# Pi-Star-Lab/RESCO

Measured on AMD Instinct MI355X. Metric: env-steps/sec, higher is better.
Workload: dtype f32; 1 GPU; ingolstadt21 x 4096 lock-step envs per GPU (BASELINE config 3), fixed demand from the map's rou.xml, on-device seeded random policy, Krauss sigma 0.5 + speedFactor dev 0.1; tls_expiry=1, map=ingolstadt21, envs_per_gpu=4096, pipes=2, ticks_per_env_step=10, block_threads=512, lds_bytes_per_env=40896, parallelism=env-batch split x1, no collective on the data path

## Files before the change

include/resco_sim.h:

```cpp
#ifndef RESCO_SIM_H
#define RESCO_SIM_H
#include <stdint.h>

#ifdef __cplusplus
extern "C" {
#endif

#define RS_OK 0
#define RS_EINVAL (-1)
#define RS_EHIP (-2)
#define RS_ENOMEM (-3)
#define RS_ELIMIT (-4)

typedef struct rs_scenario {
    int32_t n_lanes, n_links, n_edges, n_routes, n_trips, n_signals, n_obs, n_vtypes;
    int32_t n_foes, n_route_steps, n_tls_states, n_tls_dur, n_tls_yellow;
    int32_t n_fix_states, n_fix_dur, n_mv_in, n_mv_out, n_pr_out;
    int32_t horizon, capacity, step_length, yellow_length, kmax;
    const float *lane_len, *lane_vmax;
    const int32_t *lane_edge, *lane_left, *lane_right, *lane_link_start, *lane_link_cnt, *lane_obs, *lane_internal;
    const int32_t *link_to_lane, *link_dest_lane, *link_to_edge, *link_tls, *link_tls_pos, *link_minor, *link_cont;
    const int32_t *link_foe_start, *link_foe_cnt;
    const float *link_via_len;
    const int32_t *link_via1, *link_via2, *link_from_lane, *foe_link;
// ... 203 lines not shown
int rs_mplight_dqn_grad(rs_mplight_dqn_handle p, const rs_mplight_ring *ring, const int32_t *idx, int32_t batch, float *loss_out, void *stream);
int rs_mplight_dqn_step(rs_mplight_dqn_handle p, void *stream);
int rs_mplight_dqn_update(rs_mplight_dqn_handle p, const rs_mplight_ring *ring, int32_t batch, uint32_t seed, int32_t n_updates, float *loss_out,
                          void *stream);
int64_t rs_mplight_dqn_steps(rs_mplight_dqn_handle p);
void rs_mplight_dqn_destroy(rs_mplight_dqn_handle p);

typedef struct rs_train {
    int32_t kind;
    int32_t n_envs;
    rs_policy_handle policy;
    void *learner;
    void *obs;
    int16_t *act;
    float *rew;
    uint8_t *done;
    float *ret;
    float *loss_out;
    int64_t t0;
    double eps_start, eps_end;
    int32_t capacity, head, count, done_step;
    int32_t batch, updates_per_step, target_update, decay_steps;
    uint32_t policy_seed, learner_seed;
} rs_train;
int rs_idqn_pack_weights(rs_policy_handle p, const rs_dqn_tensors *params, void *stream);
int rs_dqn_sync_target(rs_dqn_handle p, void *stream);
int rs_mplight_dqn_sync_target(rs_mplight_dqn_handle p, void *stream);
int rs_group_train(const rs_handle *handles, int32_t n_handles, const rs_train *train, int32_t n_steps);

typedef struct rs_ppo_train {
    rs_policy_handle policy;
    rs_ppo_handle learner;
    rs_rollout seg;
    uint8_t *done;
    float *last_value;
    float *adv, *ret;
    void *gae_scratch;
    int32_t *perm;
    float *loss_out;
    int64_t t0;
    int64_t update0;
    int32_t slot0, done_step;
    int32_t epochs, minibatch;
    float gamma, lambda;
    uint32_t policy_seed, learner_seed;
} rs_ppo_train;
int rs_ppo_perm(int32_t n, int32_t epochs, uint32_t seed, uint32_t update_key, int32_t *perm , void *stream);
int rs_ippo_pack_weights(rs_policy_handle p, const rs_ppo_tensors *params, void *stream);
int rs_group_ppo_train(const rs_handle *handles, int32_t n_handles, const rs_ppo_train *tr, int32_t n_steps);

typedef struct rs_fma2c_desc {
    int32_t K, M, S, n_obs, full;
    float norm_wave, clip_wave, norm_wait, clip_wait;
    const int32_t *n_a, *n_s, *n_w, *n_f;
    const int32_t *gather_off, *gather_idx;
    const float *gather_scale;
    const int32_t *fp_off, *fp_src, *mgr_off, *mgr_src;
} rs_fma2c_desc;
int rs_fma2c_create(int32_t device_id, const rs_fma2c_desc *desc, const float *weights, int32_t max_envs, rs_policy_handle *out);
int rs_fma2c_act(rs_policy_handle p, const float *lane_agg, int32_t n_envs, int32_t env_base, uint32_t seed, uint32_t step_key,
                 const void *dyn, int32_t *actions, float *pi_out, float *value_out, float *rows_out, void *stream);
int rs_fma2c_value(rs_policy_handle p, const float *lane_agg, int32_t n_envs, int32_t env_base, float *value_out, void *stream);
int rs_fma2c_reset(rs_policy_handle p, int32_t env_base, int32_t n_envs, int32_t clear_fingerprints, void *stream);
int rs_fma2c_set_device_weights(rs_policy_handle p, const float *weights);
int rs_fma2c_buffer(rs_policy_handle p, int32_t which, void **dev_ptr);
void rs_fma2c_destroy(rs_policy_handle p);

typedef struct rs_fma2c_learn_config {
    double gamma, lr, alpha, eps, max_grad_norm, value_coef, entropy_coef, reward_norm, reward_clip;
    int64_t workspace_bytes;
} rs_fma2c_learn_config;
typedef struct rs_fma2c_learn *rs_fma2c_learn_handle;
int rs_fma2c_learn_create(rs_policy_handle policy, const rs_fma2c_learn_config *config, int32_t n_envs, int32_t t_max, rs_fma2c_learn_handle *out);
int rs_fma2c_learn_grad(rs_fma2c_learn_handle l, const float *rows, const int32_t *acts, const float *rewards, const float *values,
                        const int32_t *dones, const float *R_boot, int32_t T, float *loss_out, void *stream);
int rs_fma2c_learn_step(rs_fma2c_learn_handle l, void *stream);
int rs_fma2c_learn_update(rs_fma2c_learn_handle l, const float *rows, const int32_t *acts, const float *rewards, const float *values,
                          const int32_t *dones, const float *R_boot, int32_t T, float *loss_out, const float *states_fw, void *stream);
int rs_fma2c_learn_reset(rs_fma2c_learn_handle l, void *stream);
int rs_fma2c_learn_buffer(rs_fma2c_learn_handle l, int32_t which, void **dev_ptr);
void rs_fma2c_learn_destroy(rs_fma2c_learn_handle l);

int rs_info(rs_handle h, int32_t *n_envs, int32_t *block_threads, int32_t *lds_bytes, int32_t *max_lanes_per_signal);

#ifdef __cplusplus
}
#endif
#endif
```

resco_amd/build.py:

```python
import os
import subprocess

HERE = os.path.dirname(os.path.abspath(__file__))
ROOT = os.path.dirname(HERE)
SRC = os.path.join(HERE, 'csrc', 'resco_sim.hip')
LIB = os.path.join(HERE, 'csrc', 'libresco_sim.so')
HIPCC = os.environ.get('HIPCC', '/opt/rocm/bin/hipcc')
FLAGS = ['--offload-arch=gfx950', '-O3', '-std=c++17', '-ffp-contract=off', '-fno-honor-nans', '-mllvm', '-disable-machine-licm', '-fPIC', '-shared',
         '-I' + os.path.join(ROOT, 'include'), '-I' + os.path.join(HERE, 'csrc')]
_DEPS = [SRC] + [os.path.join(HERE, 'csrc', f) for f in ('resco_host.h', 'resco_step.h', 'resco_tables.h', 'resco_policy.h', 'resco_frap.h', 'resco_fma2c.h', 'resco_fma2c_train.h', 'resco_ppo.h', 'resco_train.h', 'resco_ppo_train.h', 'resco_dqn_train.h', 'resco_frap_train.h', 'resco_group_train.h', 'resco_ppo_loop.h')] + \
        [os.path.join(ROOT, 'include', f) for f in ('resco_sim.h', 'resco_model.h')]


def build_library(force=False, verbose=False):
    force = force or os.environ.get('GRAFT_FORCE_BUILD') == '1'
    if not force and os.path.exists(LIB) and all(os.path.getmtime(LIB) >= os.path.getmtime(d) for d in _DEPS):
        return LIB
    cmd = [HIPCC] + FLAGS + [SRC, '-o', LIB]
    if verbose:
        print(' '.join(cmd))
    subprocess.check_call(cmd)
    return LIB


CHECK_LIB = os.path.join(HERE, 'csrc', 'libresco_sim_check.so')


def build_check_library(force=False):
    force = force or os.environ.get('GRAFT_FORCE_BUILD') == '1'
    if not force and os.path.exists(CHECK_LIB) and all(os.path.getmtime(CHECK_LIB) >= os.path.getmtime(d) for d in _DEPS):
        return CHECK_LIB
    subprocess.check_call([HIPCC] + FLAGS + ['-DRS_DEVICE_ASSERT', '-DRS_ONE_CAP=256', SRC, '-o', CHECK_LIB])
    return CHECK_LIB


FIELDLOADS_LIB = os.path.join(HERE, 'csrc', 'libresco_sim_fieldloads.so')


def build_fieldloads_library(force=False):
    if not force and os.path.exists(FIELDLOADS_LIB) and all(os.path.getmtime(FIELDLOADS_LIB) >= os.path.getmtime(d) for d in _DEPS):
        return FIELDLOADS_LIB
    subprocess.check_call([HIPCC] + FLAGS + ['-DRS_FIELD_LOADS', '-DRS_ONE_CAP=256', SRC, '-o', FIELDLOADS_LIB])
    return FIELDLOADS_LIB


if __name__ == '__main__':
    print(build_library(force=True, verbose=True))
```

resco_amd/csrc/resco_host.h:

```cpp
#pragma once
#include "resco_step.h"

RS_DEV void rs_reset_env(const KTab &T, const State &G, const KParams &P, int env, int first, unsigned stride) {
    const int C = T.capacity, S = T.n_signals;
    const size_t eo = (size_t)env * C;
    for (int s = first; s < C; s += stride) {
        G.lane()[eo + s] = LANE_NONE; G.trip()[eo + s] = TRIP_NONE; G.owner()[eo + s] = OWNER_NONE;
        G.rwait()[eo + s] = 0; G.swait()[eo + s] = 0; G.cursor()[eo + s] = 0; G.depart()[eo + s] = 0; G.wtot()[eo + s] = 0;
        G.pos()[eo + s] = 0.0f; G.speed()[eo + s] = 0.0f; G.accel()[eo + s] = 0.0f; G.tloss()[eo + s] = 0.0f; G.sf()[eo + s] = 1.0f;
        G.coop(0)[eo + s] = COOP_NONE; G.coop(1)[eo + s] = COOP_NONE; G.cooplead(0)[eo + s] = COOP_NONE; G.cooplead(1)[eo + s] = COOP_NONE;
    }
    for (int s = first; s < S; s += stride) {
        int ph, left;
        if (P.fixed_program) { ph = T.cold.fix_init_phase[s]; left = T.cold.fix_init_left[s]; }
        else { ph = T.cold.tls_init_phase[s]; left = T.cold.tls_dur[T.cold.tls_dur_off[s] + ph]; }
        G.tls[(env * S + s) * TLS_W + 0] = ph; G.tls[(env * S + s) * TLS_W + 1] = left; G.tls[(env * S + s) * TLS_W + 2] = 0; G.tls[(env * S + s) * TLS_W + 3] = 0;
    }
    for (int d = first; d < T.n_dep; d += stride) G.dep_next[(size_t)env * T.n_dep + d] = T.cold.dep_first[d];
    for (int i = first; i < (C + 31) / 32; i += stride) G.mail[(size_t)env * ((C + 31) / 32) + i] = 0u;
    for (int i = first; i < 4; i += stride) G.env[env * 4 + i] = 0;
    for (int i = first; i < ST_N; i += stride) G.stats[(size_t)env * ST_N + i] = 0;
    if (G.trip_log)
        for (int i = first; i < T.n_trips * 4; i += stride) G.trip_log[(size_t)env * T.n_trips * 4 + i] = 0;
}
// ... 57 lines not shown
    X(VEH_POS, G.pos(), F32, 2, n, c, 1, 1)                 X(VEH_SPEED, G.speed(), F32, 2, n, c, 1, 1)                               \
    X(VEH_ACCEL, G.accel(), F32, 2, n, c, 1, 1)             X(VEH_TLOSS, G.tloss(), F32, 2, n, c, 1, 1)                               \
    X(VEH_LANE, G.lane(), U16, 2, n, c, 1, 1)               X(VEH_TRIP, G.trip(), U16, 2, n, c, 1, 1)                                 \
    X(VEH_CURSOR, G.cursor(), U16, 2, n, c, 1, 1)           X(VEH_SWAIT, G.swait(), U16, 2, n, c, 1, 1)                               \
    X(VEH_RWAIT, G.rwait(), U16, 2, n, c, 1, 1)             X(VEH_DEPART, G.depart(), U16, 2, n, c, 1, 1)                             \
    X(VEH_OWNER, G.owner(), U8, 2, n, c, 1, 1)              X(STATS, G.stats, I64, 2, n, ST_N, 1, 1)                                  \
    X(DRQ_NORM_F16, O.drq_f16(), F16, 4, n, s, lmax, 5)     X(VEH_SF, G.sf(), F32, 2, n, c, 1, 1)                                     \
    X(VEH_WTOT, G.wtot(), U16, 2, n, c, 1, 1)               X(TRIP_LOG, G.trip_log, I32, 3, n, n_trips, 4, 1)                         \
    X(DEP_NEXT, G.dep_next, U16, 2, n, n_dep, 1, 1)                                                                                   \
    X(VEH_COOP, G.coop(0), U32, 2, n, c, 1, 1)              X(VEH_COOPLEAD, G.cooplead(0), U32, 2, n, c, 1, 1)                        \
    X(ARRIVALS, O.arrivals(), I32, 2, n, s, 1, 1)           X(DEPARTURES, O.departures(), I32, 2, n, s, 1, 1)                         \
    X(MPLIGHT_FULL, O.mplight_full(), F32, 3, n, s, 49, 1)  X(LANE_ARRIVALS, O.lane_arr(), I32, 2, n, o, 1, 1)                        \
    X(VEH_COOP_ODD, G.coop(1), U32, 2, n, c, 1, 1)          X(VEH_COOPLEAD_ODD, G.cooplead(1), U32, 2, n, c, 1, 1)                    \
    X(VEH_MAIL, G.mail, U32, 2, n, (c + 31) / 32, 1, 1)
#define RS_BUF_BIT(id, ptr, dt, nd, a, b, c_, d) | (1ull << RS_BUF_##id)
static_assert((0ull RS_BUF_TABLE(RS_BUF_BIT)) == (1ull << RS_BUF_COUNT) - 1, "RS_BUF_TABLE must describe every buffer id below RS_BUF_COUNT");
#undef RS_BUF_BIT
#define RS_BUF_ONE(id, ptr, dt, nd, a, b, c_, d) + 1
static_assert((0 RS_BUF_TABLE(RS_BUF_ONE)) == RS_BUF_COUNT, "RS_BUF_TABLE must describe every buffer id once");
#undef RS_BUF_ONE
static inline void rs_fill_bufs(Buf *bufs, const State &G, const Out &O, int32_t *actions, const BufDims &D) {
    const int64_t n = D.n, c = D.c, s = D.s, o = D.o, lmax = D.lmax, n_dep = D.n_dep, n_trips = D.n_trips;
#define RS_BUF_SET(id, ptr_, dt, nd, a, b, c_, d)                                                                  \
    { Buf &B = bufs[RS_BUF_##id];                                                                                  \
      B.ptr = (void *)(ptr_); B.dtype = RS_##dt; B.ndim = nd;                                                      \
      B.shape[0] = (a); B.shape[1] = (b); B.shape[2] = (c_); B.shape[3] = (d);                                     \
      B.bytes = (size_t)(B.shape[0] * B.shape[1] * B.shape[2] * B.shape[3]) * kDtypeSize[RS_##dt]; }
    RS_BUF_TABLE(RS_BUF_SET)
#undef RS_BUF_SET
}
static inline void rs_buf_describe(const Buf &B, void **ptr, int64_t shape[4], int32_t *ndim, int32_t *dtype) {
    if (ptr) *ptr = B.ptr;
    if (shape) for (int i = 0; i < 4; ++i) shape[i] = B.shape[i];
    if (ndim) *ndim = B.ndim;
    if (dtype) *dtype = B.dtype;
}
static inline void rs_info_describe(int n_envs_, int block_, size_t lds_, int lmax_, int32_t *n_envs, int32_t *block_threads, int32_t *lds_bytes,
                                    int32_t *max_lanes_per_signal) {
    if (n_envs) *n_envs = n_envs_;
    if (block_threads) *block_threads = block_;
    if (lds_bytes) *lds_bytes = (int32_t)lds_;
    if (max_lanes_per_signal) *max_lanes_per_signal = lmax_;
}

static inline const char *rs_pack_tables(PackedTables &PT, const rs_scenario *sc) {
    PackedTables probe;
    if (!probe.build(sc)) { PT.err = probe.err; return PT.err.c_str(); }
    if (!PT.build(sc, pick_cell_len(sc, probe.n_arr, probe.n_dep, probe.tls_maxl))) return PT.err.c_str();
    return nullptr;
}
#define RS_KTAB_TABLES(X, K, PT, sc)                                                                                                  \
    X(K.lanes_, LaneRec, PT.lanes.data(), PT.lanes.size()) X(K.links_, LinkRec, PT.links.data(), PT.links.size())                     \
    X(K.foes_, FoeRec, PT.foes.data(), PT.foes.size()) X(K.rsteps_, RStep, PT.rsteps.data(), PT.rsteps.size())                        \
    X(K.routes_, RouteRec, PT.routes.data(), PT.routes.size()) X(K.next_link_, uint16_t, PT.next_link.data(), PT.next_link.size())    \
    X(K.trip_route_, uint16_t, PT.trip_route.data(), PT.trip_route.size()) X(K.trip_vtype_, uint8_t, PT.trip_vtype.data(), PT.trip_vtype.size()) \
    X(K.route_cont_, float, PT.route_cont.data(), PT.route_cont.size()) X(K.notbest_, uint16_t, PT.notbest.data(), PT.notbest.size()) \
    X(K.cold.trip_depart, int32_t, sc->trip_depart, sc->n_trips) X(K.cold.trip_next, uint16_t, PT.trip_next.data(), PT.trip_next.size()) \
    X(K.cold.dep_lane, uint16_t, PT.dep_lane.data(), PT.dep_lane.size()) X(K.cold.dep_info, DepInfo, PT.dep_info.data(), PT.dep_info.size()) \
    X(K.cold.dep_first, uint16_t, PT.dep_first.data(), PT.dep_first.size())                                                           \
    X(K.cold.vtype_params, float, sc->vtype_params, sc->n_vtypes * VT_COLS)                                                           \
    X(K.cold.tls8, uint8_t, PT.tls8.data(), PT.tls8.size()) X(K.cold.fix8, uint8_t, PT.fix8.data(), PT.fix8.size())                   \
    X(K.cold.tls_nphase, int32_t, sc->tls_nphase, sc->n_signals) X(K.cold.tls_ngreen, int32_t, sc->tls_ngreen, sc->n_signals)         \
    X(K.cold.tls_nlinks, int32_t, sc->tls_nlinks, sc->n_signals) X(K.cold.tls_state_off, int32_t, PT.tls_off_p.data(), sc->n_signals) \
    X(K.cold.tls_dur_off, int32_t, sc->tls_dur_off, sc->n_signals) X(K.cold.tls_yel_off, int32_t, sc->tls_yel_off, sc->n_signals)     \
    X(K.cold.tls_dur, int32_t, sc->tls_dur, sc->n_tls_dur) X(K.cold.tls_yellow, int32_t, sc->tls_yellow, sc->n_tls_yellow)            \
    X(K.cold.tls_init_phase, int32_t, sc->tls_init_phase, sc->n_signals)                                                              \
    X(K.cold.fix_nphase, int32_t, sc->fix_nphase, sc->n_signals) X(K.cold.fix_state_off, int32_t, PT.fix_off_p.data(), sc->n_signals) \
    X(K.cold.fix_dur_off, int32_t, sc->fix_dur_off, sc->n_signals) X(K.cold.fix_dur, int32_t, sc->fix_dur, sc->n_fix_dur)             \
    X(K.cold.fix_init_phase, int32_t, sc->fix_init_phase, sc->n_signals) X(K.cold.fix_init_left, int32_t, sc->fix_init_left, sc->n_signals) \
    X(K.cold.lane_obs, int16_t, PT.lane_obs16.data(), PT.lane_obs16.size()) X(K.cold.obs_sig, int32_t, PT.obs_sig.data(), PT.obs_sig.size()) \
    X(K.cold.sig_obs_start, int32_t, sc->sig_obs_start, sc->n_signals + 1)                                                            \
    X(K.cold.mv_in_start, int32_t, sc->mv_in_start, sc->n_signals * 12 + 1) X(K.cold.mv_in_idx, int32_t, sc->mv_in_idx, sc->n_mv_in)  \
    X(K.cold.mv_out_start, int32_t, sc->mv_out_start, sc->n_signals * 12 + 1) X(K.cold.mv_out_idx, int32_t, sc->mv_out_idx, sc->n_mv_out) \
    X(K.cold.pr_out_start, int32_t, sc->pr_out_start, sc->n_signals + 1) X(K.cold.pr_out_idx, int32_t, sc->pr_out_idx, sc->n_pr_out)  \
    X(K.cold.trips_cum, int32_t, sc->trips_cum, sc->horizon + 2)
static inline int rs_step_ratio(const rs_params *p) { return p->step_ratio > 1 ? p->step_ratio : 1; }
static inline void rs_ktab_scalars(KTab &K, const PackedTables &PT, const rs_scenario *sc, int ratio) {
    K.maxlen = PT.maxlen; K.occ_unit = PT.occ_unit;
    K.n_trips = sc->n_trips; K.tls_maxl = PT.tls_maxl; K.kmax = sc->kmax;
    K.n_lanes = sc->n_lanes; K.n_cells = PT.n_cells; K.n_signals = sc->n_signals; K.n_obs = sc->n_obs; K.n_vtypes = sc->n_vtypes;
    K.horizon = sc->horizon; K.capacity = sc->capacity; K.step_length = sc->step_length; K.yellow_length = sc->yellow_length * ratio; K.lmax = PT.lmax;
    K.n_arr = PT.n_arr; K.n_dep = PT.n_dep;
}
static inline KParams rs_kparams(const rs_params *p, int32_t env_base, int32_t n_envs) {
    KParams P{};
    P.seed = p->seed; P.env_base = env_base; P.max_distance = p->max_distance; P.sigma = p->sigma;
    P.speed_dev = p->speed_dev; P.fixed_program = p->fixed_program; P.tls_expiry = p->tls_hold == 0; P.n_envs = n_envs;
    return P;
}
```

resco_amd/csrc/resco_sim.hip:

```cpp
#include <hip/hip_runtime.h>
#include <hip/hip_fp16.h>
#include <stdint.h>
#include <stdio.h>
#include <stdlib.h>
#include <string.h>
#include <math.h>
#include <initializer_list>
#include <mutex>
#include <new>
#include <string>
#include <vector>

#include "resco_sim.h"

#define RS_DEV __device__ __forceinline__
#define RS_HD __host__ __device__
#define RS_MEM __device__ __forceinline__
#define RS_G(p) (p)
#define RS_CARVE __host__ __device__ __forceinline__
__device__ __forceinline__ void rs_atomic_min(int32_t *p, int32_t v) { atomicMin(p, v); }
__device__ __forceinline__ void rs_atomic_min(uint32_t *p, uint32_t v) { atomicMin(p, v); }
__device__ __forceinline__ void rs_atomic_max(int32_t *p, int32_t v) { atomicMax(p, v); }
__device__ __forceinline__ void rs_atomic_add(int32_t *p, int32_t v) { atomicAdd(p, v); }
__device__ __forceinline__ int32_t rs_atomic_fetch_add(int32_t *p, int32_t v) { return atomicAdd(p, v); }
__device__ __forceinline__ int32_t rs_wave_ticket(int32_t *p) {
    const unsigned long long m = __ballot(1);
    const int below = (int)__builtin_amdgcn_mbcnt_hi((uint32_t)(m >> 32), __builtin_amdgcn_mbcnt_lo((uint32_t)m, 0u));
    int32_t base = 0;
    if (below == 0) base = atomicAdd(p, (int32_t)__popcll(m));
    return __builtin_amdgcn_readlane(base, __ffsll((long long)m) - 1) + below;
}
__device__ __forceinline__ void rs_wave_add(int32_t *p, int32_t v) {
    for (int m = 32; m > 0; m >>= 1) v += __shfl_xor(v, m);
    if ((threadIdx.x & 63) == 0 && v) atomicAdd(p, v);
}
__device__ __forceinline__ void rs_wave_max(int32_t *p, int32_t v) {
    for (int m = 32; m > 0; m >>= 1) { const int32_t o = __shfl_xor(v, m); v = o > v ? o : v; }
    if ((threadIdx.x & 63) == 0) atomicMax(p, v);
}
__device__ __forceinline__ void rs_atomic_or(uint32_t *p, uint32_t v) { atomicOr(p, v); }
__device__ __forceinline__ uint32_t rs_atomic_fetch_or(uint32_t *p, uint32_t v) { return atomicOr(p, v); }
__device__ __forceinline__ int rs_atomic_inc(int32_t *p) { return atomicAdd(p, 1); }
__device__ __forceinline__ void rs_atomic_and(uint32_t *p, uint32_t v) { atomicAnd(p, v); }
__device__ __forceinline__ uint32_t rs_atomic_cas(uint32_t *p, uint32_t cmp, uint32_t v) { return atomicCAS(p, cmp, v); }
__device__ __forceinline__ int rs_ffsll(unsigned long long x) { return __ffsll(x); }
__device__ __forceinline__ int rs_clzll(unsigned long long x) { return __clzll((long long)x); }
__device__ __forceinline__ int rs_ffs(uint32_t x) { return __ffs((int)x); }
__device__ __forceinline__ int rs_popc(uint32_t x) { return __popc(x); }
__device__ __forceinline__ float rs_int_as_float(int x) { return __int_as_float(x); }
__device__ __forceinline__ int rs_float_as_int(float x) { return __float_as_int(x); }
__device__ __forceinline__ uint16_t rs_f2h(float x) { return __half_as_ushort(__float2half(x)); }

#ifndef RS_IEEE_DIV
__device__ __forceinline__ float rs_div_unscaled(float a, float b) {
    const float r0 = __builtin_amdgcn_rcpf(b);
    const float r1 = __builtin_fmaf(__builtin_fmaf(-b, r0, 1.0f), r0, r0);
    const float q0 = a * r1;
    const float q1 = __builtin_fmaf(__builtin_fmaf(-b, q0, a), r1, q0);
    return __builtin_fmaf(__builtin_fmaf(-b, q1, a), r1, q1);
}
#define RS_DIV(a, b) rs_div_unscaled((a), (b))
#endif
#define RS_OPAQUE_S(x) asm volatile("" : "+s"(x));
#ifndef RS_NARROW_NODE
#define RS_KEEP4(a, b, c, d) asm volatile("" : "+v"(a), "+v"(b), "+v"(c), "+v"(d));
#define RS_KEEP2(a, b) asm volatile("" : "+v"(a), "+v"(b));
#endif
extern __shared__ __attribute__((aligned(16))) char rs_smem[];
#define RS_SMEM rs_smem

#ifdef RS_STUDY_SECTIONS
__device__ unsigned long long *g_sec_prof;
#define RS_SEC_BEGIN unsigned long long sec_t = wall_clock64();
#define RS_SEC(id) { const unsigned long long sec_1 = wall_clock64(); if (g_sec_prof && (threadIdx.x & 63) == 0 && (blockIdx.x & 15) == 0) atomicAdd(&g_sec_prof[id], (sec_1 - sec_t) + (1ull << 40)); sec_t = wall_clock64(); }
#endif
#ifdef RS_DEVICE_ASSERT
#define RS_ASSERT(c) if (!(c)) rs_atomic_add(&L.sc[SC_STATS + ST_INVARIANT], 1);
#endif
#include "resco_host.h"
#include "resco_policy.h"
#include "resco_frap.h"
#include "resco_fma2c.h"
#include "resco_ppo.h"
#include "resco_ppo_train.h"
#include "resco_dqn_train.h"
#include "resco_frap_train.h"
#include "resco_group_train.h"
#include "resco_ppo_loop.h"
#include "resco_fma2c_train.h"

struct StepArgs { KTab T; State G; Out O; Lds L; };
typedef const __attribute__((address_space(4))) StepArgs *StepArgsPtr;

template <bool PROF> struct DevExec {
    int B;
    int wave;
    unsigned long long *prof;
    unsigned long long t0;
    template <class F> __device__ __forceinline__ void phase(int id, F f) {
        int w = wave;
        uint32_t ones = ~0u;
        asm volatile("" : "+s"(w), "+s"(ones));
        int tid = (w << 6) | (int)__builtin_amdgcn_mbcnt_hi(ones, __builtin_amdgcn_mbcnt_lo(ones, 0u));
        asm volatile("" : "+v"(tid));
        f(tid);
        __syncthreads();
        if (PROF && prof) {
            const unsigned long long t1 = wall_clock64();
            if (tid == 0) atomicAdd(&prof[id], t1 - t0);
            t0 = t1;
        }
    }
    __device__ __forceinline__ int wave_of(int) const { return wave; }
    __device__ __forceinline__ int next_chunk(int32_t *ctr, int, int, int) const {
        int c = 0;
        if (__builtin_amdgcn_mbcnt_hi(~0u, __builtin_amdgcn_mbcnt_lo(~0u, 0u)) == 0) c = atomicAdd(ctr, 1);
        return __builtin_amdgcn_readfirstlane(c);
    }
    __device__ __forceinline__ unsigned long long role_begin() const { return (PROF && prof) ? wall_clock64() : 0ull; }
    __device__ __forceinline__ void role_end(int id, unsigned long long start) const {
#ifdef RS_STUDY_SECTIONS
        return;
#endif
        if (PROF && prof && (threadIdx.x & 63) == 0 && (blockIdx.x & 15) == 0) atomicAdd(&prof[id], (wall_clock64() - start) + (1ull << 40));
    }
};
template <int CAP, bool PROF> __device__ __forceinline__ void rs_step_kernel_body(StepArgsPtr Ac, const KParams &P, const int32_t *__restrict__ actions) {
    if ((int)blockIdx.x >= P.n_envs) return;
    const StepArgs *A = (const StepArgs *)Ac;
#ifdef RS_STUDY_SECTIONS
    if (threadIdx.x == 0) g_sec_prof = P.prof;
#endif
    DevExec<PROF> ex{(int)blockDim.x, __builtin_amdgcn_readfirstlane((int)threadIdx.x >> 6), PROF ? P.prof : nullptr, (PROF && P.prof) ? wall_clock64() : 0ull};
    rs_step_body<CAP>(ex, A->L, A->T, A->G, A->O, P, actions, (int)blockIdx.x);
}
template <int CAP>
__global__ void __launch_bounds__(1024, 8)
rs_step_kernel_v64(StepArgsPtr Ac, KParams P, const int32_t *__restrict__ actions) { rs_step_kernel_body<CAP, false>(Ac, P, actions); }
template <int CAP>
__global__ void __launch_bounds__(768, 6)
rs_step_kernel_v80(StepArgsPtr Ac, KParams P, const int32_t *__restrict__ actions) { rs_step_kernel_body<CAP, false>(Ac, P, actions); }
template <int CAP>
__global__ void __launch_bounds__(512, 4)
rs_step_kernel_v128(StepArgsPtr Ac, KParams P, const int32_t *__restrict__ actions) { rs_step_kernel_body<CAP, false>(Ac, P, actions); }
__global__ void __launch_bounds__(768, 6)
rs_step_kernel_prof(StepArgsPtr Ac, KParams P, const int32_t *__restrict__ actions) { rs_step_kernel_body<0, true>(Ac, P, actions); }

__global__ void rs_reset_kernel(KTab T, State G, KParams P) { rs_reset_env(T, G, P, (int)blockIdx.x, (int)threadIdx.x, blockDim.x); }
__global__ void rs_reinit_kernel(KTab T, State G, KParams P) { rs_reinit_env(T, G, P, (int)blockIdx.x, (int)threadIdx.x, blockDim.x); }
__global__ void rs_act_random_kernel(KTab T, KParams P, uint32_t step_key, int32_t *actions) {
    const int i = blockIdx.x * blockDim.x + threadIdx.x;
    if (i < P.n_envs * T.n_signals) actions[i] = rs_random_action(T, P, step_key, i);
}
__global__ void rs_act_maxwave_kernel(KTab T, KParams P, const int32_t *pairs, int n_pairs, const int32_t *valid, const int32_t *order,
                                      int use_pressure, const int32_t *mplight, const int32_t *wave, int32_t *actions) {
    const int i = blockIdx.x * blockDim.x + threadIdx.x;
    if (i < P.n_envs * T.n_signals) actions[i] = rs_maxwave_action(T, pairs, n_pairs, valid, order, use_pressure, mplight, wave, i);
}

enum RegBudget { V64 = 0, V128 = 1, V80 = 2 };
struct rs_sim {
    int device = 0;
    int n_envs = 0, env_base = 0, block = 256;
    int ratio = 1;
    size_t lds = 0;
    KTab K{};
    StepArgs *args = nullptr;
    RegBudget budget = V64;
    State G{};
    Out O{};
    KParams P{};
    uint32_t out_mask = OUT_ALL;
    int32_t *actions = nullptr;
    int32_t *pairs = nullptr, *valid = nullptr, *order = nullptr;
    unsigned long long *prof = nullptr;
    int n_pairs = 0;
    hipStream_t stream = nullptr;
    bool blocking = false;
    int32_t *pair = nullptr;
    hipStream_t last = nullptr;
    std::vector<void *> allocs;
    Buf bufs[RS_BUF_COUNT]{};
    bool timing = false;
    std::vector<std::pair<hipEvent_t, hipEvent_t>> events;
    size_t ev_used = 0;
    std::string err;
};

static thread_local std::string g_create_err;

#define HIPCHK(h, call)                                                                            \
    do {                                                                                           \
        hipError_t e_ = (call);                                                                    \
        if (e_ != hipSuccess) {                                                                    \
            (h)->err = std::string(#call) + ": " + hipGetErrorString(e_);                          \
            (void)hipGetLastError();     \
            return RS_EHIP;                                                                        \
        }                                                                                          \
    } while (0)

template <typename Tp>
static int dev_alloc(rs_sim *h, Tp **p, size_t count, bool zero = true) {
    void *d = nullptr;
    size_t bytes = (count ? count : 1) * sizeof(Tp);
    hipError_t e = hipMalloc(&d, bytes);
    if (e != hipSuccess) { h->err = std::string("hipMalloc: ") + hipGetErrorString(e); return RS_ENOMEM; }
    if (zero) (void)hipMemset(d, 0, bytes);
    h->allocs.push_back(d);
    *p = (Tp *)d;
    return RS_OK;
}
template <typename Tp>
static int dev_upload(rs_sim *h, const Tp **dst, const Tp *src, size_t count) {
    Tp *d = nullptr;
    int rc = dev_alloc(h, &d, count, false);
    if (rc) return rc;
    if (count) HIPCHK(h, hipMemcpy(d, src, count * sizeof(Tp), hipMemcpyHostToDevice));
    *dst = d;
    return RS_OK;
}

typedef void (*step_kernel_fn)(StepArgsPtr, KParams, const int32_t *);
static const int kStepCaps[] = {0, 128, 256, 512, 768, 896, 1024};
#define RS_PICK(cap_) (regs == V128 ? rs_step_kernel_v128<cap_> : (regs == V80 ? rs_step_kernel_v80<cap_> : rs_step_kernel_v64<cap_>))
static step_kernel_fn step_kernel_for(int regs, int capacity) {
#ifdef RS_ONE_CAP
    (void)capacity;
    return regs == V64 ? rs_step_kernel_v64<RS_ONE_CAP> : rs_step_kernel_v80<RS_ONE_CAP>;
#else
    switch (capacity) {
        case 128: return RS_PICK(128);
        case 256: return RS_PICK(256);
        case 512: return RS_PICK(512);
        case 768: return RS_PICK(768);
        case 896: return RS_PICK(896);
        case 1024: return RS_PICK(1024);
        default: return RS_PICK(0);
    }
#endif
}

static hipError_t wait_idle(rs_sim *h) {
    hipError_t e = hipStreamSynchronize(h->stream);
    if (e == hipSuccess && h->last && h->last != h->stream) e = hipStreamSynchronize(h->last);
    return e;
}

extern "C" int32_t rs_default_block(int32_t capacity, int32_t n_envs_on_device, int32_t device_id) {
    const int C = capacity;
    if (C < 64 || n_envs_on_device <= 0) return 0;
    const int base = C >= 768 ? 8 : ((C / 2) + 63) / 64;
    int waves = base;
    if (C < 768) {
        int cus = 256;
        hipDeviceProp_t prop;
        if (hipGetDeviceProperties(&prop, device_id) == hipSuccess && prop.multiProcessorCount > 0) cus = prop.multiProcessorCount;
        else (void)hipGetLastError();
        const long budget = (long)cus * 4 * 7;
        const int fit = (int)(budget / n_envs_on_device), most = C / 64 + 1;
        waves = fit < most ? fit : most;
        if (waves < base) waves = base;
    }
    return -(20000 + 64 * waves);
}

static bool decode_block(int block_threads, size_t lds, RegBudget *budget, int *threads) {
    int t = block_threads;
    RegBudget b = V64;
    if (t <= -20000) {
        t = -t - 20000;
        b = (t == 512 && lds <= RS_LDS_4WG_LIMIT) ? V64 : V80;
    } else if (t < 0) { b = V128; t = -t; if (t >= 10000) { b = V80; t -= 10000; } }
    *budget = b; *threads = t;
    return t % 64 == 0 && t >= 64 && t <= (b == V128 ? 512 : (b == V80 ? 768 : 1024));
}

extern "C" int rs_create(const rs_scenario *sc, const rs_params *p, int32_t n_envs, int32_t env_base, int32_t device_id,
                         int32_t block_threads, rs_handle *out) {
    if (!sc || !p || !out || n_envs <= 0) { g_create_err = "rs_create: bad argument"; return RS_EINVAL; }
    rs_sim *h = new (std::nothrow) rs_sim();
    if (!h) return RS_ENOMEM;
    auto fail = [&](int rc) { g_create_err = h->err; (void)hipGetLastError(); rs_destroy(h); return rc; };
    (void)hipGetLastError();
    h->device = device_id; h->n_envs = n_envs; h->env_base = env_base;
    int ndev = 0;
    if (hipGetDeviceCount(&ndev) != hipSuccess || ndev <= 0) { h->err = "no HIP device visible (this library has no CPU fallback)"; return fail(RS_EHIP); }
    if (hipSetDevice(device_id) != hipSuccess) { h->err = "hipSetDevice failed"; return fail(RS_EHIP); }
    if (sc->step_length <= 0 || sc->yellow_length < 0 || sc->yellow_length >= sc->step_length) {
        h->err = "need 0 <= yellow_length < step_length"; return fail(RS_EINVAL);
    }
    const int C = sc->capacity;
    if (C < 64 || (C % 64) || C > 1984) { h->err = "capacity must be a multiple of 64 in [64, 1984]"; return fail(RS_ELIMIT); }
    if (sc->kmax < 1 || sc->kmax > 16) { h->err = "kmax (lanes per edge) must be in [1, 16]"; return fail(RS_ELIMIT); }
    PackedTables PT;
    if (const char *msg = rs_pack_tables(PT, sc)) { h->err = msg; return fail(RS_ELIMIT); }
    int rc;
#define UP(dst, type, src, count) if ((rc = dev_upload<type>(h, &dst, src, (size_t)(count)))) return fail(rc);
    RS_KTAB_TABLES(UP, h->K, PT, sc)
#undef UP
    h->ratio = rs_step_ratio(p);
    rs_ktab_scalars(h->K, PT, sc, h->ratio);
    const int lmax = PT.lmax;
    h->P = rs_kparams(p, env_base, n_envs);
    const size_t N = (size_t)n_envs, NC = N * C, S = (size_t)sc->n_signals;
    State &G = h->G;
    Out &O = h->O;
    {
        char *slab = nullptr, *outb = nullptr;
        G.nc = NC;
        O.n = n_envs; O.o = sc->n_obs; O.s = sc->n_signals; O.lm = lmax;
        if ((rc = dev_alloc(h, &slab, State::bytes(NC))) || (rc = dev_alloc(h, &outb, O.bytes())) ||
            (rc = dev_alloc(h, &G.env, N * 4)) || (rc = dev_alloc(h, &G.tls, N * S * TLS_W)) || (rc = dev_alloc(h, &G.stats, N * ST_N)) ||
            (rc = dev_alloc(h, &G.dep_next, N * (size_t)h->K.n_dep)) || (rc = dev_alloc(h, &G.mail, N * (size_t)((C + 31) / 32))) ||
            (rc = dev_alloc(h, &h->actions, N * S)))
            return fail(rc);
        G.base = slab; O.base = outb;
    }
    G.trip_log = nullptr;
    if (p->trip_log && (rc = dev_alloc(h, &G.trip_log, N * (size_t)sc->n_trips * 4))) return fail(rc);
    rs_fill_bufs(h->bufs, G, O, h->actions, BufDims{n_envs, C, sc->n_signals, sc->n_obs, lmax, h->K.n_dep, p->trip_log ? sc->n_trips : 0});

    h->lds = lds_carve(nullptr, C, h->K.n_cells, h->K.n_arr, h->K.n_dep, sc->n_obs, sc->n_signals, sc->n_vtypes, h->K.tls_maxl);
    if (const char *pad = getenv("RESCO_STUDY_LDS_PAD")) h->lds += (size_t)atoi(pad);
    if (h->lds > 160 * 1024) { h->err = "scenario needs more than 160 KiB of LDS per environment"; return fail(RS_ELIMIT); }
    if (block_threads == 0) block_threads = rs_default_block(C, n_envs, device_id);
    if (!decode_block(block_threads, h->lds, &h->budget, &block_threads)) {
        h->err = "block_threads must be a multiple of 64 in [64, 1024] ([64, 768] for the 80-VGPR build, [64, 512] for the 128-VGPR build)";
        return fail(RS_EINVAL);
    }
    h->block = block_threads;
    {
        static std::mutex mu;
        static size_t max_lds[64] = {0};
        std::lock_guard<std::mutex> lock(mu);
        size_t &cur = max_lds[device_id & 63];
        if (h->lds > cur) {
            for (int v = V64; v <= V80; ++v)
                for (int cp : kStepCaps)
                    if (hipFuncSetAttribute((const void *)step_kernel_for(v, cp), hipFuncAttributeMaxDynamicSharedMemorySize, (int)h->lds) != hipSuccess) {
                        h->err = "hipFuncSetAttribute(MaxDynamicSharedMemorySize) failed"; return fail(RS_EHIP);
                    }
            if (hipFuncSetAttribute((const void *)rs_step_kernel_prof, hipFuncAttributeMaxDynamicSharedMemorySize, (int)h->lds) != hipSuccess) {
                h->err = "hipFuncSetAttribute(MaxDynamicSharedMemorySize) failed"; return fail(RS_EHIP);
            }
            cur = h->lds;
        }
    }
    {
        StepArgs sa{h->K, h->G, h->O, Lds{}};
        lds_carve(&sa.L, C, h->K.n_cells, h->K.n_arr, h->K.n_dep, sc->n_obs, sc->n_signals, sc->n_vtypes, h->K.tls_maxl);
        if (!lds_fix_matches(sa.L, C)) { h->err = "the layout of the working memory does not match the kernel's literals (lds_carve / LdsFix)"; return fail(RS_EINVAL); }
        sa.L.cell_inv = PT.cell_inv;
        if ((rc = dev_alloc(h, &h->args, 1, false))) return fail(rc);
        if (hipMemcpy(h->args, &sa, sizeof(sa), hipMemcpyHostToDevice) != hipSuccess) { h->err = "hipMemcpy(StepArgs) failed"; return fail(RS_EHIP); }
    }
    {
        hipDeviceProp_t prop;
        std::vector<uint32_t> mask;
        if (getenv("RESCO_PLAIN_STREAMS") == nullptr && hipGetDeviceProperties(&prop, device_id) == hipSuccess)
            mask.assign((size_t)(prop.multiProcessorCount + 31) / 32, 0xFFFFFFFFu);
        if (mask.empty() || hipExtStreamCreateWithCUMask(&h->stream, (uint32_t)mask.size(), mask.data()) != hipSuccess) {
            (void)hipGetLastError();
            if (hipStreamCreateWithFlags(&h->stream, hipStreamNonBlocking) != hipSuccess) { h->err = "hipStreamCreate failed"; return fail(RS_EHIP); }
        } else h->blocking = true;
    }
    *out = h;
    int r2 = rs_reset(h, nullptr);
    if (r2) { g_create_err = h->err; *out = nullptr; rs_destroy(h); return r2; }
    return RS_OK;
}

extern "C" void rs_destroy(rs_handle h) {
    if (!h) return;
    (void)hipSetDevice(h->device);
    if (h->stream) { (void)wait_idle(h); (void)hipStreamDestroy(h->stream); }
    for (auto &e : h->events) { (void)hipEventDestroy(e.first); (void)hipEventDestroy(e.second); }
    for (void *p : h->allocs) (void)hipFree(p);
    delete h;
}

extern "C" const char *rs_last_error(rs_handle h) { return h ? h->err.c_str() : g_create_err.c_str(); }

static int launch_step(rs_sim *h, hipStream_t st, int n_ticks, int do_fsm, int do_observe = 1) {
    KParams P = h->P;
    P.n_ticks = n_ticks; P.do_fsm = do_fsm; P.do_observe = do_observe; P.out_mask = h->out_mask; P.prof = h->prof;
    hipEvent_t e0 = nullptr, e1 = nullptr;
    if (h->timing) {
        if (h->ev_used == h->events.size()) {
            hipEvent_t a, b;
            HIPCHK(h, hipEventCreate(&a));
            HIPCHK(h, hipEventCreate(&b));
            h->events.emplace_back(a, b);
        }
        e0 = h->events[h->ev_used].first; e1 = h->events[h->ev_used].second;
        h->ev_used += 1;
        HIPCHK(h, hipEventRecord(e0, st));
    }
    const step_kernel_fn fn = (h->prof && h->block <= 768) ? (step_kernel_fn)rs_step_kernel_prof : step_kernel_for(h->budget, h->K.capacity);
    hipLaunchKernelGGL(fn, dim3(h->n_envs), dim3(h->block), h->lds, st, (StepArgsPtr)h->args, P, (const int32_t *)h->actions);
    HIPCHK(h, hipGetLastError());
    if (h->timing) HIPCHK(h, hipEventRecord(e1, st));
    return RS_OK;
}

static int enter(rs_sim *h, void *stream, hipStream_t *st) {
    if (!h) return RS_EINVAL;
    HIPCHK(h, hipSetDevice(h->device));
    *st = stream ? (hipStream_t)stream : h->stream;
    h->last = *st;
    return RS_OK;
}

static int launch_reset(rs_sim *h, void *stream, void (*kernel)(KTab, State, KParams)) {
    hipStream_t st;
    int rc = enter(h, stream, &st);
    if (rc) return rc;
    hipLaunchKernelGGL(kernel, dim3(h->n_envs), dim3(256), 0, st, h->K, h->G, h->P);
    HIPCHK(h, hipGetLastError());
    bool tm = h->timing;
    h->timing = false;
    rc = launch_step(h, st, 0, 0);
    h->timing = tm;
    return rc;
}
extern "C" int rs_reset(rs_handle h, void *stream) { return launch_reset(h, stream, rs_reset_kernel); }
extern "C" int rs_reinit_signals(rs_handle h, void *stream) { return launch_reset(h, stream, rs_reinit_kernel); }

extern "C" int rs_step(rs_handle h, const int32_t *actions, int32_t actions_on_device, void *stream) {
    hipStream_t st;
    if (int rc = enter(h, stream, &st)) return rc;
    if (actions) {
        size_t bytes = (size_t)h->n_envs * h->K.n_signals * sizeof(int32_t);
        HIPCHK(h, hipMemcpyAsync(h->actions, actions, bytes, actions_on_device ? hipMemcpyDeviceToDevice : hipMemcpyHostToDevice, st));
        if (!actions_on_device) HIPCHK(h, hipStreamSynchronize(st));
    }
    return launch_step(h, st, h->K.step_length * h->ratio, 1);
}

extern "C" int rs_ticks(rs_handle h, int32_t n_ticks, void *stream) {
    hipStream_t st;
    if (n_ticks < 0) return RS_EINVAL;
    if (int rc = enter(h, stream, &st)) return rc;
    return launch_step(h, st, n_ticks, 0);
}

extern "C" int rs_step_sim(rs_handle h, int32_t n_ticks, void *stream) {
    hipStream_t st;
    if (n_ticks < 0) return RS_EINVAL;
    if (int rc = enter(h, stream, &st)) return rc;
    return launch_step(h, st, n_ticks, 0, 0);
}

extern "C" int rs_set_outputs(rs_handle h, uint64_t buffer_mask) {
    if (!h) return RS_EINVAL;
    h->out_mask = rs_out_mask(buffer_mask);
    return RS_OK;
}

extern "C" int rs_sync(rs_handle h) {
    if (!h) return RS_EINVAL;
    HIPCHK(h, hipSetDevice(h->device));
    HIPCHK(h, wait_idle(h));
    return RS_OK;
}

static void launch_random(rs_sim *h, hipStream_t st, uint32_t step_key) {
    const int total = h->n_envs * h->K.n_signals;
    hipLaunchKernelGGL(rs_act_random_kernel, dim3((total + 255) / 256), dim3(256), 0, st, h->K, h->P, step_key, h->actions);
}
static void launch_maxwave(rs_sim *h, hipStream_t st, int use_pressure) {
    const int total = h->n_envs * h->K.n_signals;
    hipLaunchKernelGGL(rs_act_maxwave_kernel, dim3((total + 255) / 256), dim3(256), 0, st, h->K, h->P, (const int32_t *)h->pairs,
                       h->n_pairs, (const int32_t *)h->valid, (const int32_t *)h->order, use_pressure, (const int32_t *)h->O.mplight(),
                       (const int32_t *)h->O.wave(), h->actions);
}

extern "C" int rs_act_random(rs_handle h, uint32_t step_key, void *stream) {
    hipStream_t st;
    if (int rc = enter(h, stream, &st)) return rc;
    launch_random(h, st, step_key);
    HIPCHK(h, hipGetLastError());
// ... 45 lines not shown
    if (!h) return RS_EINVAL;
    return rs_read_buffer(h, RS_BUF_STATS, host_out, (int64_t)h->n_envs * ST_N * 8);
}

struct Snapshot { std::vector<void *> ptrs; uint32_t seed = 0; };
static const int kSnapBufs[] = {RS_BUF_LANE_AGG, RS_BUF_DRQ_NORM, RS_BUF_PHASE, RS_BUF_MPLIGHT, RS_BUF_WAVE, RS_BUF_WAIT,
                                RS_BUF_WAIT_NORM, RS_BUF_PRESSURE, RS_BUF_QUEUE_SUM, RS_BUF_QUEUE_MAX, RS_BUF_DRQ_NORM_F16,
                                RS_BUF_ENV, RS_BUF_TLS, RS_BUF_VEH_POS, RS_BUF_VEH_SPEED, RS_BUF_VEH_ACCEL, RS_BUF_VEH_TLOSS,
                                RS_BUF_VEH_LANE, RS_BUF_VEH_TRIP, RS_BUF_VEH_CURSOR, RS_BUF_VEH_SWAIT, RS_BUF_VEH_RWAIT,
                                RS_BUF_VEH_DEPART, RS_BUF_VEH_OWNER, RS_BUF_VEH_SF, RS_BUF_VEH_WTOT, RS_BUF_TRIP_LOG, RS_BUF_STATS,
                                RS_BUF_DEP_NEXT, RS_BUF_VEH_COOP, RS_BUF_VEH_COOPLEAD, RS_BUF_ARRIVALS, RS_BUF_DEPARTURES, RS_BUF_MPLIGHT_FULL,
                                RS_BUF_LANE_ARRIVALS, RS_BUF_VEH_COOP_ODD, RS_BUF_VEH_COOPLEAD_ODD, RS_BUF_VEH_MAIL};
extern "C" int rs_snapshot(rs_handle h, void **snap) {
    if (!h || !snap) return RS_EINVAL;
    HIPCHK(h, hipSetDevice(h->device));
    HIPCHK(h, wait_idle(h));
    Snapshot *S = new Snapshot();
    S->seed = h->P.seed;
    for (int b : kSnapBufs) {
        void *d = nullptr;
        if (h->bufs[b].bytes == 0) { S->ptrs.push_back(nullptr); continue; }
        if (hipMalloc(&d, h->bufs[b].bytes) != hipSuccess) { h->err = "rs_snapshot: hipMalloc failed"; rs_snapshot_free(h, S); return RS_ENOMEM; }
        S->ptrs.push_back(d);
        HIPCHK(h, hipMemcpy(d, h->bufs[b].ptr, h->bufs[b].bytes, hipMemcpyDeviceToDevice));
    }
    *snap = S;
    return RS_OK;
}
extern "C" int rs_restore(rs_handle h, const void *snap) {
    if (!h || !snap) return RS_EINVAL;
    HIPCHK(h, hipSetDevice(h->device));
    HIPCHK(h, wait_idle(h));
    const Snapshot *S = (const Snapshot *)snap;
    size_t i = 0;
    for (int b : kSnapBufs) { if (h->bufs[b].bytes) HIPCHK(h, hipMemcpy(h->bufs[b].ptr, S->ptrs[i], h->bufs[b].bytes, hipMemcpyDeviceToDevice)); ++i; }
    h->P.seed = S->seed;
    return RS_OK;
}
extern "C" void rs_snapshot_free(rs_handle h, void *snap) {
    if (!snap) return;
    Snapshot *S = (Snapshot *)snap;
    for (void *p : S->ptrs) (void)hipFree(p);
    delete S;
}

extern "C" int rs_timing(rs_handle h, int32_t enable) {
    if (!h) return RS_EINVAL;
    h->timing = enable != 0;
    return RS_OK;
}
extern "C" int rs_timing_read(rs_handle h, float *total_ms, int32_t *launches) {
    if (!h) return RS_EINVAL;
    HIPCHK(h, hipSetDevice(h->device));
    HIPCHK(h, hipDeviceSynchronize());
    float tot = 0.0f;
    for (size_t i = 0; i < h->ev_used; ++i) {
        float ms = 0.0f;
        HIPCHK(h, hipEventElapsedTime(&ms, h->events[i].first, h->events[i].second));
        tot += ms;
    }
    if (total_ms) *total_ms = tot;
    if (launches) *launches = (int32_t)h->ev_used;
    h->ev_used = 0;
    return RS_OK;
}

extern "C" int rs_phase_profile(rs_handle h, int32_t enable, uint64_t *host_out16) {
    if (!h) return RS_EINVAL;
    HIPCHK(h, hipSetDevice(h->device));
    HIPCHK(h, hipDeviceSynchronize());
    if (h->prof && host_out16) HIPCHK(h, hipMemcpy(host_out16, h->prof, 16 * 8, hipMemcpyDeviceToHost));
    if (enable && !h->prof) { int rc = dev_alloc(h, &h->prof, 16); if (rc) return rc; }
    if (h->prof) HIPCHK(h, hipMemset(h->prof, 0, 16 * 8));
    if (!enable) h->prof = nullptr;
    return RS_OK;
}

extern "C" int rs_set_seed(rs_handle h, uint32_t seed) {
    if (!h) return RS_EINVAL;
    h->P.seed = seed;
    return RS_OK;
}

extern "C" int rs_info(rs_handle h, int32_t *n_envs, int32_t *block_threads, int32_t *lds_bytes, int32_t *max_lanes_per_signal) {
    if (!h) return RS_EINVAL;
    rs_info_describe(h->n_envs, h->block, h->lds, h->K.lmax, n_envs, block_threads, lds_bytes, max_lanes_per_signal);
    return RS_OK;
}


enum { POLICY_IDQN = 0, POLICY_MPLIGHT = 1, POLICY_FMA2C = 2 };
struct rs_policy {
    int device = 0;
    int kind = POLICY_IDQN;
    PolicyTab W{};
    int amax = 0;
    bool own_w1 = true, own_w2 = true, own_w3 = true, own_b3 = true;
    FrapTab F{};
    Fma2cTab A{};
    int fm_lds = 0;
    const float *fm_own_w = nullptr;
    std::vector<void *> allocs;
};

static int policy_devices(rs_policy_handle *out, int *ndev) {
    if (!out) return RS_EINVAL;
    *out = nullptr;
    if (hipGetDeviceCount(ndev) != hipSuccess || *ndev <= 0) { g_create_err = "no HIP device visible (this library has no CPU fallback)"; return RS_EHIP; }
    return RS_OK;
}
static int policy_new(int device_id, int kind, rs_policy **p) {
    if (hipSetDevice(device_id) != hipSuccess) { g_create_err = "hipSetDevice failed"; return RS_EHIP; }
    *p = new (std::nothrow) rs_policy();
    if (!*p) return RS_ENOMEM;
    (*p)->device = device_id; (*p)->kind = kind;
    return RS_OK;
}
static void policy_destroy(rs_policy *p) {
    if (!p) return;
    (void)hipSetDevice(p->device);
    (void)hipDeviceSynchronize();
    for (void *d : p->allocs) (void)hipFree(d);
    delete p;
}
extern "C" void rs_idqn_destroy(rs_policy_handle p) { policy_destroy(p); }
extern "C" void rs_mplight_destroy(rs_policy_handle p) { policy_destroy(p); }

template <class T> static int pol_upload(rs_policy *p, const T **dst, const void *src, size_t count) {
    void *d = nullptr;
    if (hipMalloc(&d, count * sizeof(T) + 2048) != hipSuccess) return RS_ENOMEM;
    p->allocs.push_back(d);
    if (hipMemcpy(d, src, count * sizeof(T), hipMemcpyHostToDevice) != hipSuccess) return RS_EHIP;
    *dst = (const T *)d;
    return RS_OK;
}

extern "C" int rs_idqn_create(int32_t device_id, int32_t n_signals, int32_t lmax, const int32_t *n_actions, const float *conv_w,
                              const float *conv_b, const uint16_t *w1, const float *b1, const uint16_t *w2, const float *b2,
                              const uint16_t *w3, const float *b3, rs_policy_handle *out) {
    int ndev = 0;
    if (int rc = policy_devices(out, &ndev)) return rc;
    if (device_id < 0 || device_id >= ndev || n_signals <= 0 || lmax < 2 || lmax > 17 || !n_actions || !conv_w || !conv_b || !w1 || !b1 || !w2 || !b2 || !w3 || !b3) {
        g_create_err = "rs_idqn_create: bad argument (1 <= signals, 2 <= lmax <= 17)"; return RS_EINVAL;
    }
    for (int s = 0; s < n_signals; ++s)
        if (n_actions[s] < 1 || n_actions[s] > POL_QMAX) { g_create_err = "rs_idqn_create: 1..8 actions per signal"; return RS_ELIMIT; }
    rs_policy *p = nullptr;
    int rc = policy_new(device_id, POLICY_IDQN, &p);
    if (rc) return rc;
    const size_t S = (size_t)n_signals, hp = (size_t)(lmax / 2);
    p->W.S = n_signals; p->W.lmax = lmax; p->W.hp = (int32_t)hp;
    for (int s = 0; s < n_signals; ++s) p->amax = n_actions[s] > p->amax ? n_actions[s] : p->amax;
    if ((rc = pol_upload<float>(p, &p->W.conv_w, conv_w, S * 64 * 4)) || (rc = pol_upload<float>(p, &p->W.conv_b, conv_b, S * 64)) ||
        (rc = pol_upload<h4_t>(p, &p->W.w1, w1, S * 64 * hp * 2 * 64)) || (rc = pol_upload<float>(p, &p->W.b1, b1, S * 64)) ||
        (rc = pol_upload<h4_t>(p, &p->W.w2, w2, S * 8 * 2 * 64)) || (rc = pol_upload<float>(p, &p->W.b2, b2, S * 64)) ||
        (rc = pol_upload<h4_t>(p, &p->W.w3, w3, S * 8 * 64)) || (rc = pol_upload<float>(p, &p->W.b3, b3, S * 32)) ||
        (rc = pol_upload<int32_t>(p, &p->W.n_actions, n_actions, S)) ||
        (rc = pol_upload<int32_t>(p, &p->W.hp_sig, std::vector<int32_t>(S, (int32_t)hp).data(), S))) {
        g_create_err = "rs_idqn_create: device allocation / upload failed";
        rs_idqn_destroy(p);
        return rc;
    }
    *out = p;
    return RS_OK;
}

// ... 1189 lines not shown
```

resco_amd/csrc/resco_step.h:

```cpp
#pragma once
#include "resco_tables.h"

struct State {
    char *base;
    size_t nc;
    int32_t *trip_log;
    int32_t *env;
    int32_t *tls;
    long long *stats;
    uint16_t *dep_next;
    uint32_t *mail;
    RS_HD float *pos() const { return (float *)base; }
    RS_HD float *speed() const { return RS_G((float *)(base + 4 * nc)); }
    RS_HD float *accel() const { return RS_G((float *)(base + 8 * nc)); }
    RS_HD float *tloss() const { return RS_G((float *)(base + 12 * nc)); }
    RS_HD float *sf() const { return RS_G((float *)(base + 16 * nc)); }
    RS_HD uint32_t *coop(int par) const { return RS_G((uint32_t *)(base + (par ? 43 : 20) * nc)); }
    RS_HD uint32_t *cooplead(int par) const { return RS_G((uint32_t *)(base + (par ? 47 : 24) * nc)); }
    RS_HD uint16_t *lane() const { return RS_G((uint16_t *)(base + 28 * nc)); }
    RS_HD uint16_t *trip() const { return RS_G((uint16_t *)(base + 30 * nc)); }
    RS_HD uint16_t *cursor() const { return RS_G((uint16_t *)(base + 32 * nc)); }
    RS_HD uint16_t *swait() const { return RS_G((uint16_t *)(base + 34 * nc)); }
    RS_HD uint16_t *rwait() const { return RS_G((uint16_t *)(base + 36 * nc)); }
    RS_HD uint16_t *depart() const { return RS_G((uint16_t *)(base + 38 * nc)); }
    RS_HD uint16_t *wtot() const { return RS_G((uint16_t *)(base + 40 * nc)); }
    RS_HD uint8_t *owner() const { return RS_G((uint8_t *)(base + 42 * nc)); }
    static size_t bytes(size_t nc_) { return 51 * nc_; }
};

struct Out {
    char *base;
    int32_t n, o, s, lm;
    RS_HD size_t a5() const { return (size_t)n * o * 5 * 4; }
    RS_HD size_t ns() const { return (size_t)n * s * 4; }
    RS_HD float *lane_agg() const { return (float *)base; }
    RS_HD float *drq_norm() const { return RS_G((float *)(base + a5())); }
    RS_HD float *wait() const { return RS_G((float *)(base + 2 * a5())); }
    RS_HD float *wait_norm() const { return RS_G((float *)(base + 2 * a5() + ns())); }
    RS_HD int32_t *phase() const { return RS_G((int32_t *)(base + 2 * a5() + 2 * ns())); }
    RS_HD int32_t *pressure() const { return RS_G((int32_t *)(base + 2 * a5() + 3 * ns())); }
    RS_HD int32_t *queue_sum() const { return RS_G((int32_t *)(base + 2 * a5() + 4 * ns())); }
    RS_HD int32_t *queue_max() const { return RS_G((int32_t *)(base + 2 * a5() + 5 * ns())); }
    RS_HD int32_t *mplight() const { return RS_G((int32_t *)(base + 2 * a5() + 6 * ns())); }
    RS_HD int32_t *wave() const { return RS_G((int32_t *)(base + 2 * a5() + 19 * ns())); }
    RS_HD int32_t *arrivals() const { return RS_G((int32_t *)(base + 2 * a5() + 31 * ns())); }
    RS_HD int32_t *departures() const { return RS_G((int32_t *)(base + 2 * a5() + 32 * ns())); }
    RS_HD float *mplight_full() const { return RS_G((float *)(base + 2 * a5() + 33 * ns())); }
    RS_HD int32_t *lane_arr() const { return RS_G((int32_t *)(base + 2 * a5() + 82 * ns())); }
    RS_HD uint16_t *drq_f16() const { return RS_G((uint16_t *)(base + 2 * a5() + 82 * ns() + a5() / 5)); }
    RS_HD size_t bytes() const { return 2 * a5() + 82 * ns() + a5() / 5 + (size_t)n * s * lm * 5 * 2 + 64; }
};

RS_DEV uint32_t rs_rotl32(uint32_t x, int r) { return (x << r) | (x >> (32 - r)); }
RS_DEV uint32_t d_hash(uint32_t seed, uint32_t env, uint32_t trip, uint32_t tick, uint32_t stream) {
    uint32_t h = seed;
    const uint32_t w[4] = {env, trip, tick, stream};
#pragma unroll
    for (int i = 0; i < 4; ++i) {
        uint32_t k = w[i];
        k *= 0xcc9e2d51u; k = rs_rotl32(k, 15); k *= 0x1b873593u;
        h ^= k; h = rs_rotl32(h, 13); h = h * 5u + 0xe6546b64u;
    }
    h ^= 16u;
    h ^= h >> 16; h *= 0x85ebca6bu; h ^= h >> 13; h *= 0xc2b2ae35u; h ^= h >> 16;
    return h;
}
RS_DEV float d_u01(uint32_t h) { return (float)(h >> 8) * (1.0f / 16777216.0f); }

#ifndef RS_DIV
#define RS_DIV(a, b) ((a) / (b))
#endif
RS_DEV float d_brake_gap(float v, float b) {
    const int steps = (int)RS_DIV(v, b);
    const float fs = (float)steps;
    return fs * v - b * fs * (fs + 1.0f) * 0.5f;
}
RS_DEV float d_stop_speed(float gap, float b, float tau) {
    const float g = gap - 0.001f;
    if (g < 0.0f) return 0.0f;
    const float q = 1.0f + 4.0f * ((RS_DIV(2.0f * g, b) - tau) + tau * tau);
    const float n = floorf(0.5f - (tau + sqrtf(q) * -0.5f));
    const float h = 0.5f * n * (n - 1.0f) * b + n * b * tau;
    const float r = RS_DIV(g - h, n + tau);
    return n * b + r;
}
RS_DEV float d_free_speed(float dist, float target, float b) {
    if (dist < target) return target;
    const float t2 = b + 2.0f * target;
    float y = RS_DIV((sqrtf(t2 * t2 + 8.0f * b * dist) - b) * 0.5f - target, b);
    if (y < 0.0f) y = 0.0f;
    const float yf = floorf(y);
    const float exact = (yf * yf + yf) * 0.5f * b + yf * target + (y > yf ? target : 0.0f);
    float rest = dist - exact;
    if (rest < 0.0f) rest = 0.0f;
    return RS_DIV(rest, yf + 1.0f) + yf * b + target;
}
RS_DEV float d_follow_speed(float gap, float vl, float b, float bl, float tau) {
    const float bm = b > bl ? b : bl;
    return d_stop_speed(gap + d_brake_gap(vl, bm), b, tau);
}
RS_DEV int speed_factor_q(const KParams &P, int env, int trip, const float *vt) {
    float f = vt[VT_SF_MEAN];
    if (P.speed_dev) {
        float s = 0.0f;
#pragma unroll
        for (uint32_t i = 0; i < 4; ++i) s += d_u01(d_hash(P.seed, (uint32_t)env, (uint32_t)trip, 0xFFFFFFFFu, i));
        const float z = (s - 2.0f) * 1.7320508f;
        f = vt[VT_SF_MEAN] + vt[VT_SF_DEV] * z;
    }
    if (f < 0.2f) f = 0.2f;
// ... 109 lines not shown
        if (6 * ab > grid_bytes) {
            p = (uint32_t)(align16((size_t)C * 16) + align16((size_t)C * 8));
            if (6 * ab > align16((size_t)C * 4)) { p = (uint32_t)o; o += 6 * ab; }
        }
        if (L) {
            L->agg_q.off = p; L->agg_a.off = p + (uint32_t)ab; L->agg_w.off = p + (uint32_t)(2 * ab);
            L->agg_m.off = p + (uint32_t)(3 * ab); L->agg_s.off = p + (uint32_t)(4 * ab); L->agg_n.off = p + (uint32_t)(5 * ab);
        }
    }
#undef CARVE
    return o;
}

template <class Tp, uint32_t OFF> struct CPtr {
    RS_MEM Tp &operator[](int i) const { return ((Tp *)(RS_SMEM + OFF))[i]; }
    RS_MEM operator Tp *() const { return (Tp *)(RS_SMEM + OFF); }
};
template <int C> struct LdsFix {
    static constexpr uint32_t a16(uint32_t x) { return (x + 15u) & ~15u; }
#ifdef RS_LIST_CAP
    static constexpr uint32_t kcap = RS_LIST_CAP;
#else
    static constexpr uint32_t kcap = ((C / 4 + 63) / 64) * 64;
#endif
    static constexpr uint32_t o_node = 0, o_aux = o_node + a16(C * 16), o_vnx = o_aux + a16(C * 8), o_sc = o_vnx + a16(C * 4),
                              o_alive = o_sc + a16((SC_STATS + ST_N) * 4), o_alive0 = o_alive + a16(((C + 31) / 32) * 4),
                              o_ls_h = o_alive0 + a16(((C + 31) / 32) * 4), o_ls_lc = o_ls_h + a16(kcap * 2), o_ls_mh = o_ls_lc + a16(kcap * 2),
                              o_grid = o_ls_mh + a16(kcap * 2);
    CPtr<Node, o_node> node;
    CPtr<Aux, o_aux> aux;
    CPtr<float, o_vnx> vnx;
    CPtr<int32_t, o_sc> sc;
    CPtr<uint32_t, o_alive> alive;
    CPtr<uint32_t, o_alive0> alive0;
    CPtr<uint16_t, o_ls_h> ls_h;
    CPtr<uint16_t, o_ls_lc> ls_lc;
    CPtr<uint16_t, o_ls_mh> ls_mh;
    CPtr<uint16_t, o_grid> grid;
    static constexpr uint32_t lcap = kcap;
    const LPtr<float> &vtp;
    const uint32_t &gstride;
    const LPtr<int32_t> &arr;
    const LPtr<uint16_t> &dep, &dep_t;
    const LPtr<uint32_t> &insm, &mailw;
    const LPtr<int32_t> &agg_q, &agg_a, &agg_w, &agg_m, &agg_n;
    const LPtr<uint32_t> &agg_s;
    const LPtr<int32_t> &sig_arr, &sig_dep, &phase, &left, &nextp;
    const LPtr<uint8_t> &tstate;
    const float &cell_inv;
    RS_MEM explicit LdsFix(const Lds &T)
        : vtp(T.vtp), gstride(T.gstride), arr(T.arr), dep(T.dep), dep_t(T.dep_t), insm(T.insm), mailw(T.mailw), agg_q(T.agg_q), agg_a(T.agg_a), agg_w(T.agg_w),
          agg_m(T.agg_m), agg_n(T.agg_n), agg_s(T.agg_s), sig_arr(T.sig_arr), sig_dep(T.sig_dep), phase(T.phase), left(T.left), nextp(T.nextp),
          tstate(T.tstate), cell_inv(T.cell_inv) {}
    static RS_HD bool matches(const Lds &T) {
        return T.node.off == o_node && T.aux.off == o_aux && T.vnx.off == o_vnx && T.sc.off == o_sc && T.alive.off == o_alive && T.alive0.off == o_alive0 &&
               T.ls_h.off == o_ls_h && T.ls_lc.off == o_ls_lc && T.ls_mh.off == o_ls_mh && T.grid.off == o_grid && T.lcap == kcap;
    }
};
RS_CARVE bool lds_fix_matches(const Lds &T, int C) {
    switch (C) {
        case 128: return LdsFix<128>::matches(T);
        case 256: return LdsFix<256>::matches(T);
        case 512: return LdsFix<512>::matches(T);
        case 768: return LdsFix<768>::matches(T);
        case 896: return LdsFix<896>::matches(T);
        case 1024: return LdsFix<1024>::matches(T);
        default: return true;
    }
}

RS_CARVE float pick_cell_len(const rs_scenario *sc, int n_arr, int n_dep, int tls_maxl) {
    const float choices[] = CELL_CHOICES;
    const int n = (int)(sizeof(choices) / sizeof(choices[0]));
    const size_t limits[2] = {RS_LDS_4WG_LIMIT, RS_LDS_3WG_LIMIT};
    for (int k = 0; k < 2; ++k)
        for (int i = 0; i < n; ++i)
            if (PackedTables::cell_len_ok(sc, choices[i]) &&
                lds_carve(nullptr, sc->capacity, PackedTables::count_cells(sc, choices[i]), n_arr, n_dep, sc->n_obs, sc->n_signals, sc->n_vtypes, tls_maxl) <= limits[k])
                return choices[i];
    for (int i = 0; i < n; ++i) if (PackedTables::cell_len_ok(sc, choices[i])) return choices[i];
    return choices[0];
}

#ifdef RS_EMU_DEBUG
#define RS_CHAIN_GUARD if (++rs_dbg_chain > 50000000L) { printf("endless chain walk\n"); fflush(stdout); abort(); }
#else
#define RS_CHAIN_GUARD
#endif
#ifndef RS_ASSERT
#define RS_ASSERT(c)
#endif
#ifndef RS_SEC
#define RS_SEC_BEGIN
#define RS_SEC(id) {}
#endif
template <class LT> RS_DEV int lane_cells(const LT &L, const LaneRec &LR) { return (int)(LR.len * L.cell_inv) + 1; }
template <class LT> RS_DEV int cell_of(const LT &L, float pos, int ncell) { const int c = (int)(pos * L.cell_inv); return c < ncell ? c : ncell - 1; }

struct Grid { uint16_t *c; uint32_t tag; };
RS_DEV unsigned long long grid_tag4(const Grid &g) { return g.tag ? 0x8000800080008000ull : 0ull; }
RS_DEV int cell_head(const Grid &g, int c) {
    const uint32_t v = g.c[c];
    return ((v ^ g.tag) & CELL_TAG) ? (int)NIL : (int)(v & NIL);
}
RS_DEV uint16_t grid_push(const Grid &g, int c, int s, bool mover) {
    uint32_t *w = (uint32_t *)g.c + (c >> 1);
    const int sh = (c & 1) * 16;
    const uint32_t flag = (mover ? CELL_MOVER : 0u) | g.tag;
    uint32_t old = *w, assumed, cell;
    do {
        assumed = old;
        cell = (assumed >> sh) & 0xFFFFu;
        if ((cell ^ g.tag) & CELL_TAG) cell = NIL;
        const uint32_t keep = cell & CELL_MOVER;
        uint32_t cnt = (cell >> CELL_CNT_SHIFT) & CELL_CNT_MAX;
        if (cnt < CELL_CNT_MAX) cnt += 1u;
        old = rs_atomic_cas(w, assumed, (assumed & ~(0xFFFFu << sh)) | (((uint32_t)s | (cnt << CELL_CNT_SHIFT) | keep | flag) << sh));
    } while (old != assumed);
    return (uint16_t)(cell & NIL);
}
RS_DEV unsigned long long quad_load(const Grid &g, int b) { return *(const unsigned long long *)(g.c + b) ^ grid_tag4(g); }
RS_DEV unsigned long long quad_occ(const Grid &g, int b) {
    const unsigned long long w = quad_load(g, b);
    const unsigned long long x = (w & 0x07FF07FF07FF07FFull) ^ 0x07FF07FF07FF07FFull;
    return (x + 0x07FF07FF07FF07FFull) & 0x0800080008000800ull & ~(w >> 4);
}
RS_DEV int cells_count(const Grid &g, int c0, int nc) {
    const int c1 = c0 + nc - 1;
    int n = 0;
    for (int b = c0 & ~3; b <= c1; b += 4) {
        const unsigned long long w = quad_load(g, b);
        unsigned long long m = (w >> CELL_CNT_SHIFT) & 0x0007000700070007ull;
        m &= ~(((w >> 15) & 0x0001000100010001ull) * 7ull);
        const int lo = c0 - b, hi = c1 - b;
        if (lo > 0) m &= ~0ull << (16 * lo);
        if (hi < 3) m &= ~0ull >> (16 * (3 - hi));
        n += (int)((m * 0x0001000100010001ull) >> 48);
    }
    return n;
}
RS_DEV int scan_up(const Grid &g, int c0, int c1) {
    for (int b = c0 & ~3; b <= c1; b += 4) {
        unsigned long long m = quad_occ(g, b);
        const int lo = c0 - b, hi = c1 - b;
        if (lo > 0) m &= ~0ull << (16 * lo);
        if (hi < 3) m &= ~0ull >> (16 * (3 - hi));
        if (m) return b + ((rs_ffsll(m) - 1) >> 4);
    }
    return -1;
}
RS_DEV int scan_down(const Grid &g, int c0, int c1) {
    for (int b = c1 & ~3; b + 3 >= c0; b -= 4) {
        unsigned long long m = quad_occ(g, b);
        const int lo = c0 - b, hi = c1 - b;
        if (lo > 0) m &= ~0ull << (16 * lo);
        if (hi < 3) m &= ~0ull >> (16 * (3 - hi));
        if (m) return b + ((63 - rs_clzll(m)) >> 4);
        if (b == 0) break;
    }
    return -1;
}
RS_DEV bool cells_have_mover(const Grid &g, int c0, int nc) {
    const int c1 = c0 + nc - 1;
    for (int b = c0 & ~3; b <= c1; b += 4) {
        const unsigned long long w = quad_load(g, b);
        unsigned long long m = w & 0x4000400040004000ull & ~(w >> 1);
// ... 31 lines not shown
};
#define RS_CHAIN_STEP(f, s, COND)                                                                          \
    {                                                                                                      \
        RS_CHAIN_GUARD                                                                                     \
        const Node nd_ = node_load(L, s);                                                                  \
        const unsigned long long key = order_key(nd_.pos, nd_.trip);                                       \
        const bool take_ = (COND);                                                                         \
        (f).slot = take_ ? (s) : (f).slot; (f).key = take_ ? key : (f).key;                                \
        (f).speed_bits = take_ ? (uint32_t)rs_float_as_int(nd_.speed) : (f).speed_bits;                    \
        (f).vtw = take_ ? (uint32_t)nd_.vt : (f).vtw;                                                      \
        s = nd_.nxt;                                                                                       \
    }
template <class LT> RS_DEV Found chain_rearmost(const LT &L, int head) {
    Found f{(int)NIL, ~0ull, 0u, 0u};
    for (int s = head & NIL; s != NIL;) RS_CHAIN_STEP(f, s, key < f.key)
    return f;
}
template <class LT> RS_DEV Found chain_frontmost(const LT &L, int head) {
    Found f{(int)NIL, 0ull, 0u, 0u};
    for (int s = head & NIL; s != NIL;) RS_CHAIN_STEP(f, s, key > f.key)
    return f;
}
template <class LT> RS_DEV Found rearmost_within(const LT &L, const Grid &grid, int cell0, int ncell, float win) {
    Found f{(int)NIL, ~0ull, 0u, 0u};
    if (win < 0.0f) return f;
    const int c = scan_up(grid, cell0, cell0 + cell_of(L, win, ncell));
    if (c < 0) return f;
    f = chain_rearmost(L, cell_head(grid, c));
    if (f.slot != NIL && f.pos() > win) f.slot = NIL;
    return f;
}
template <class LT> RS_DEV Found leader_found(const LT &L, const Grid &grid, int cell0, int ncell, float pos, int k, int self, float win) {
    const int c = cell_of(L, pos, ncell);
    const unsigned long long mykey = order_key(pos, k);
    Found f{(int)NIL, ~0ull, 0u, 0u};
    const uint32_t cw = grid.c[cell0 + c];
    int s = ((cw ^ grid.tag) & CELL_TAG) ? (int)NIL : (int)(cw & NIL);
    if (s == self && ((cw >> CELL_CNT_SHIFT) & CELL_CNT_MAX) == 1u) s = NIL;
    while (s != NIL) {
        RS_ASSERT(s != self || order_key(L.node[s].pos, L.node[s].trip) == mykey)
        RS_CHAIN_STEP(f, s, (key > mykey) & (key < f.key))
    }
    if (f.slot == NIL && c + 1 < ncell) {
        const int cc = scan_up(grid, cell0 + c + 1, cell0 + cell_of(L, pos + win, ncell));
        if (cc >= 0) f = chain_rearmost(L, cell_head(grid, cc));
    }
    if (f.slot != NIL && f.pos() - pos > win) f.slot = NIL;
    return f;
}
template <class LT> RS_DEV int leader_within(const LT &L, const Grid &grid, int cell0, int ncell, float pos, int k, int self, float win) {
    return leader_found(L, grid, cell0, ncell, pos, k, self, win).slot;
}
template <class LT> RS_DEV int follower_within(const LT &L, const Grid &grid, int cell0, int ncell, float pos, int k, int self, float win) {
    const int c = cell_of(L, pos, ncell);
    const unsigned long long mykey = order_key(pos, k);
    Found f{(int)NIL, 0ull, 0u, 0u};
    for (int s = cell_head(grid, cell0 + c); s != NIL;) {
        RS_ASSERT(s != self || order_key(L.node[s].pos, L.node[s].trip) == mykey)
        RS_CHAIN_STEP(f, s, (key < mykey) & (key > f.key))
    }
    if (f.slot == NIL && c > 0) {
        const float lo = pos - win;
        const int cc = scan_down(grid, cell0 + (lo > 0.0f ? cell_of(L, lo, ncell) : 0), cell0 + c - 1);
        if (cc >= 0) f = chain_frontmost(L, cell_head(grid, cc));
    }
    if (f.slot != NIL && pos - f.pos() > win) f.slot = NIL;
    (void)self;
    return f.slot;
}
template <class LT> RS_DEV int at_or_behind_within(const LT &L, const Grid &grid, int cell0, int ncell, float back, float win) {
    if (back < 0.0f) return NIL;
    const int c = cell_of(L, back, ncell);
    Found f{(int)NIL, 0ull, 0u, 0u};
    for (int s = cell_head(grid, cell0 + c); s != NIL;) RS_CHAIN_STEP(f, s, !(nd_.pos > back) & (key > f.key))
    if (f.slot == NIL && c > 0) {
        const float lo = back - win;
        const int cc = scan_down(grid, cell0 + (lo > 0.0f ? cell_of(L, lo, ncell) : 0), cell0 + c - 1);
        if (cc >= 0) f = chain_frontmost(L, cell_head(grid, cc));
    }
    if (f.slot != NIL && back - f.pos() > win) f.slot = NIL;
    return f.slot;
}

template <class LT> RS_DEV int tls_state(const KTab &T, const LT &L, int tls, int pos) {
    if (tls == 0xFF) return TLS_G;
    return L.tstate[tls * T.tls_maxl + pos];
}
RS_DEV uint16_t cache_link(const KTab &T, const LaneRec &LR, int lane, int rq, int trip) {
    if (LR.link_cnt == 0) return NLINK_NONE;
    if (LR.flags & LF_INTERNAL) { const int l = LR.link_start; return (uint16_t)(l | (T.links()[l].arr_idx >= 0 ? NLINK_ARR : 0)); }
    return T.next_link()[((size_t)rq * T.kmax + (lane - (int)LR.edge_lane0)) * 2 + (trip & 1)];
}
template <class LT> RS_DEV bool foe_blocked(const KTab &T, const LT &L, const Grid &grid, const LinkRec &K) {
    for (int i = K.foe_start; i < K.foe_start + K.foe_cnt; ++i) {
        const FoeRec F = rec_load16(T.foes(), i);
        if (F.tls != 0xFF && tls_state(T, L, F.tls, F.tls_pos) == TLS_R) continue;
        if (F.arr_idx >= 0 && L.arr[F.arr_idx] < RM_FOE_GAP_Q) return true;
        if (F.via1_cell0 != 0xFFFF && cells_have_mover(grid, F.via1_cell0, F.via1_nc)) return true;
        if (F.via2_cell0 != 0xFFFF && cells_have_mover(grid, F.via2_cell0, F.via2_nc)) return true;
    }
    return false;
}
template <class LT> RS_DEV void tls_refresh(const KTab &T, const LT &L, const KParams &P, int s, int ph) {
    const int w = T.tls_maxl >> 2;
    const uint32_t *src = (const uint32_t *)((P.fixed_program ? T.cold.fix8 + T.cold.fix_state_off[s] : T.cold.tls8 + T.cold.tls_state_off[s]) + ph * T.tls_maxl);
    uint32_t *dst = (uint32_t *)((uint8_t *)L.tstate + s * T.tls_maxl);
    uint32_t v[8];
#pragma unroll
    for (int i = 0; i < 8; ++i) v[i] = src[i < w ? i : 0];
#pragma unroll
    for (int i = 0; i < 8; ++i) if (i < w) dst[i] = v[i];
#pragma unroll 1
    for (int i = 8; i < w; ++i) dst[i] = src[i];
}
template <class LT> RS_DEV void set_phase(const KTab &T, const LT &L, const KParams &P, int s, int ph) {
    if (ph < 0 || ph >= T.cold.tls_nphase[s]) return;
    L.phase[s] = ph;
    L.left[s] = P.tls_expiry ? T.cold.tls_dur[T.cold.tls_dur_off[s] + ph] : RM_TLS_HOLD_TICKS;
    tls_refresh(T, L, P, s, ph);
}
template <class LT> RS_DEV void tls_begin_of_tick(const KTab &T, const LT &L, const KParams &P, int s, int tick) {
    if (P.do_fsm && !P.fixed_program && tick == T.yellow_length) set_phase(T, L, P, s, L.nextp[s]);
    int left = L.left[s];
    if (left == 0) {
        const int32_t *dur = P.fixed_program ? T.cold.fix_dur + T.cold.fix_dur_off[s] : T.cold.tls_dur + T.cold.tls_dur_off[s];
        const int Pn = P.fixed_program ? T.cold.fix_nphase[s] : T.cold.tls_nphase[s];
        const int ph = (L.phase[s] + 1) % Pn;
        left = dur[ph];
        L.phase[s] = ph;
        tls_refresh(T, L, P, s, ph);
    }
    L.left[s] = left - 1;
}
struct ContRow { float c[4]; const float *cn; };
RS_DEV ContRow cont_row(const KTab &T, int rq) {
    ContRow R;
    R.cn = T.route_cont() + (size_t)rq * T.kmax;
    for (int j = 0; j < 4; ++j) R.c[j] = j < T.kmax ? R.cn[j] : 0.0f;
    return R;
}
RS_DEV float cont_of(const ContRow &R, int j) {
    return j == 0 ? R.c[0] : (j == 1 ? R.c[1] : (j == 2 ? R.c[2] : (j == 3 ? R.c[3] : R.cn[j])));
}
#define OCC_NONE (Grid{(uint16_t *)0, 0u})
#define OCC_FULL (Grid{(uint16_t *)1, 0u})
RS_DEV bool cont_notbest(float c) { return rs_float_as_int(c) < 0; }
RS_DEV float cont_len(float c) { return rs_int_as_float(rs_float_as_int(c) & 0x7FFFFFFF); }
RS_DEV int strategic_dir(const ContRow &R, int kk, int n, float x, float v, int extra, float &rem, const Grid &grid, int cell0, int nc, float occ_unit) {
    const float mine = cont_of(R, kk);
    rem = cont_len(mine) - x;
#ifdef RS_EMU_CHECK_MAIL
    { float best = 0.0f; for (int j = 0; j < n; ++j) { const float c = cont_len(cont_of(R, j)); if (c > best) best = c; }
      for (int j = 0; j < n; ++j) RS_ASSERT(cont_notbest(cont_of(R, j)) == !(cont_len(cont_of(R, j)) >= best - RM_CONT_EPS)) }
#endif
    if (!cont_notbest(mine)) return 0;
    int dl = 1000, dr = 1000;
    for (int j = kk + 1; j < n; ++j) if (!cont_notbest(cont_of(R, j))) { dl = j - kk; break; }
    for (int j = kk - 1; j >= 0; --j) if (!cont_notbest(cont_of(R, j))) { dr = kk - j; break; }
    const int dir = (dr <= dl) ? -1 : +1;
    if (grid.c == (uint16_t *)1) return dir;
    const int off = (dr <= dl ? dr : dl) + extra;
    const float la = (v > RM_LOOK_MIN_SPEED ? v : RM_LOOK_MIN_SPEED) * RM_LOOK_TIME + RM_LOOK_BASE;
    int cnt = 0;
    if (grid.c != (uint16_t *)0) cnt = cells_count(grid, cell0 + ((dr <= dl) ? -dr : dl) * nc, nc);
    if (rem - (float)cnt * occ_unit >= la * (float)off) return 0;
    return dir;
}
RS_DEV uint32_t link_reg_word(const KTab &T, int nlk) { return ((const uint32_t *)&T.links()[nlk & 0x7FFF])[2]; }
template <class LT> RS_DEV void register_approach_w(const KTab &T, const LT &L, uint32_t kw, float v, float pos, float lane_len, int vt) {
    const int st = tls_state(T, L, (int)((kw >> 16) & 0xFFu), (int)(kw >> 24));
    if (st == TLS_R) return;
    const float dist = lane_len - pos;
    if (st == TLS_Y && dist >= d_brake_gap(v, L.vtp[vt * VT_COLS + VT_DECEL])) return;
    const float ta = RS_DIV(dist, v > 1.0f ? v : 1.0f);
    const int q = ta * 10.0f >= 65000.0f ? 65000 : (int)(ta * 10.0f);
    rs_atomic_min(&L.arr[(int16_t)(kw & 0xFFFFu)], q);
}
template <class LT> RS_DEV void register_approach(const KTab &T, const LT &L, int nlk, float v, float pos, float lane_len, int vt) {
    if (!(nlk & NLINK_ARR)) return;
    if (v <= RM_HALT_SPEED) return;
    register_approach_w(T, L, link_reg_word(T, nlk), v, pos, lane_len, vt);
}
template <class LT> RS_DEV void follow_neighbour(const KTab &T, const LT &L, uint32_t key, bool clamp_gap, const LaneRec &LR, int lane, float x, float v,
                             float b, float tau, float mingap, float &vsafe) {
    const int X = (int)(key & 0xFFFFu), kx = (int)(key >> 16);
    if ((int)L.node[X].trip != kx) return;
    const int lx = L.aux[X].lane;
    if (lx == (int)LANE_NONE || (LR.flags & LF_INTERNAL)) return;
    const int l0 = LR.edge_lane0, n = LR.flags >> 2;
    if (lx < l0 || lx >= l0 + n) return;
    const float *vo = L.vtp + L.node[X].vt * VT_COLS;
    const float px = L.node[X].pos, backx = px - vo[VT_LENGTH];
    if (clamp_gap ? !(px >= x) : !(backx >= x)) return;
    float g = backx - x - mingap;
    if (clamp_gap && g < 0.0f) g = 0.0f;
    float vs = d_follow_speed(g, L.node[X].speed, b, vo[VT_DECEL], tau);
    float vc = v - b; if (vc < 0.0f) vc = 0.0f;
    if (vs < vc) vs = vc;
    if (vs < vsafe) vsafe = vs;
    (void)lane;
}

template <class LT> RS_DEV void mail_flag_set(const LT &L, int s, int par) { rs_atomic_or((uint32_t *)((Node *)L.node + s) + 3, SFQ_MAIL(par) << 16); }
template <class LT> RS_DEV void mail_flag_clear(const LT &L, int s, int par) { rs_atomic_and((uint32_t *)((Node *)L.node + s) + 3, ~(SFQ_MAIL(par) << 16)); }
template <class LT, class LP> RS_DEV void list_push(const LT &L, const LP &list, int counter, int s);
template <class LT> RS_DEV void flag_mover(const LT &L, int s, int t, int lct = 0) {
    uint32_t *w = (uint32_t *)((Node *)L.node + s) + 3;
    const uint32_t bit = (uint32_t)fl_mh(t) << 8;
    if (!(rs_atomic_fetch_or(w, bit | ((uint32_t)lct << 8)) & bit)) list_push(L, L.ls_mh, SC_NMH + (t & 1), s);
}
template <class LT, class LP> RS_DEV void list_push(const LT &L, const LP &list, int counter, int s) {
    const int i = rs_wave_ticket(&L.sc[counter]);
    if (i < (int)L.lcap) list[i] = (uint16_t)s;
}
RS_DEV float plan_vfree(const float *vt, float v, float lane_vmax, float sf) {
    float vfree = v + vt[VT_ACCEL];
    const float vl = lane_vmax * sf;
    if (vl < vfree) vfree = vl;
    if (vt[VT_MAXSPEED] < vfree) vfree = vt[VT_MAXSPEED];
    return vfree;
}
RS_DEV float plan_look(const float *vt, float vfree) { return d_brake_gap(vfree, vt[VT_DECEL]) + vfree * vt[VT_TAU] + vt[VT_MINGAP] + 1.0f; }
RS_DEV bool looks_beyond(const float *vt, float v, float x, float lane_len, float lane_vmax, float sf) {
    return lane_len - x < plan_look(vt, plan_vfree(vt, v, lane_vmax, sf));
}
RS_DEV bool may_change_lanes_row(const ContRow &R, const LaneRec &LR, int lane, int k, float x, float v, int t) {
    const int n = LR.flags >> 2;
    if ((LR.flags & LF_INTERNAL) || n < 2) return false;
    const int kk = lane - (int)LR.edge_lane0;
    float rem;
    if (strategic_dir(R, kk, n, x, v, 0, rem, OCC_FULL, 0, 0, 0.0f) != 0) return true;
    if ((((uint32_t)t >> 1) + (uint32_t)k) & 3u) return false;
    const int tk = kk + ((t & 1) ? -1 : +1);
    return tk >= 0 && tk < n && strategic_dir(R, tk, n, x, v, RM_SG_EXTRA_LANES, rem, OCC_NONE, 0, 0, 0.0f) == 0;
}
RS_DEV bool may_change_lanes(const KTab &T, int rq, uint32_t nb, const LaneRec &LR, int lane, int k, float x, float v, int t) {
    const int n = LR.flags >> 2;
    if ((LR.flags & LF_INTERNAL) || n < 2) return false;
    const int kk = lane - (int)LR.edge_lane0;
    bool r;
    if ((nb >> kk) & 1u) r = true;
    else if ((((uint32_t)t >> 1) + (uint32_t)k) & 3u) r = false;
    else {
        const int tk = kk + ((t & 1) ? -1 : +1);
        if (tk < 0 || tk >= n) r = false;
        else if (!((nb >> tk) & 1u)) r = true;
        else { float rem; r = strategic_dir(cont_row(T, rq), tk, n, x, v, RM_SG_EXTRA_LANES, rem, OCC_NONE, 0, 0, 0.0f) == 0; }
    }
#ifdef RS_EMU_CHECK_MAIL
    RS_ASSERT(r == may_change_lanes_row(cont_row(T, rq), LR, lane, k, x, v, t))
#endif
    return r;
}
template <class LT> RS_DEV int classify(const KTab &T, const LT &L, int s, const float *vt, float v, float x, const LaneRec &LR, int lane, int rq, uint32_t nb, int k, float sf, int t) {
    int fl = 0;
    if (looks_beyond(vt, v, x, LR.len, LR.vmax, sf)) { fl |= FL_H; list_push(L, L.ls_h, SC_NH, s); }
    if (may_change_lanes(T, rq, nb, LR, lane, k, x, v, t)) { fl |= FL_LC; list_push(L, L.ls_lc, SC_NLC, s); }
    return fl;
}

template <bool LONG, class LT> RS_DEV void phase_plan(const KTab &T, const LT &L, const Grid &grid, const State &G, size_t eo, const KParams &P, int genv, int t, int s) {
    RS_SEC_BEGIN
    const Aux ax = L.aux[s];
    const int lane = ax.lane;
    if (lane == (int)LANE_NONE) return;
    const Node me = L.node[s];
    const int k = me.trip;
    const float *vt = L.vtp + me.vt * VT_COLS;
    const float a = vt[VT_ACCEL], b = vt[VT_DECEL], tau = vt[VT_TAU], mingap = vt[VT_MINGAP];
    const float v = me.speed, x = me.pos;
    const float sf = sf_of(me.sfq);
    const LaneRec LR0 = rec_load16(T.lanes(), lane);
    LaneRec LR = LR0;
    float vsafe = RM_BIGF;
    float tgap = 0.0f, tvl = 0.0f, tbl = b;
    bool have = false;
    if (LONG) RS_SEC(7)
    const float vfree = plan_vfree(vt, v, LR.vmax, sf);
    const float look = plan_look(vt, vfree);
    const Found ld = leader_found(L, grid, LR.cell0, lane_cells(L, LR), x, k, s, look + T.maxlen);
    const int lead = ld.slot;
    if (LONG) RS_SEC(8)
    bool found = false;
    if (lead != NIL) {
        const float *vo = L.vtp + ld.vt() * VT_COLS;
        tgap = ld.pos() - vo[VT_LENGTH] - x - mingap;
        tvl = ld.speed(); tbl = vo[VT_DECEL];
        have = true; found = true;
    }
    if (me.sfq & SFQ_MAIL((t + 1) & 1)) {
        const int q = (t + 1) & 1;
        const uint32_t c1 = G.coop(q)[eo + s], c2 = G.cooplead(q)[eo + s];
        if (c1 != COOP_NONE) { G.coop(q)[eo + s] = COOP_NONE; follow_neighbour(T, L, c1, false, LR, lane, x, v, b, tau, mingap, vsafe); }
        if (c2 != COOP_NONE) { G.cooplead(q)[eo + s] = COOP_NONE; follow_neighbour(T, L, c2, true, LR, lane, x, v, b, tau, mingap, vsafe); }
        mail_flag_clear(L, s, q);
    }
#ifdef RS_EMU_CHECK_MAIL
    else { RS_ASSERT(G.coop((t + 1) & 1)[eo + s] == COOP_NONE && G.cooplead((t + 1) & 1)[eo + s] == COOP_NONE) }
#endif
    if (LONG) RS_SEC(9)
    float seen = LR.len - x;
    RS_ASSERT(LONG || found || !(seen < look))
    if (LONG && !found && seen < look) {
        int rq = ax.rq;
        int link = (int)(ax.nlink & 0x7FFF);
        int cur_lane = lane;
        const float bgv = d_brake_gap(v, b);
        for (int hop = 0; hop < RM_MAX_HOPS; ++hop) {
            const bool cur_int = (LR.flags & LF_INTERNAL) != 0;
            if (hop > 0) link = (int)(cache_link(T, LR, cur_lane, rq, k) & 0x7FFF);
            bool stop_here = false;
            LinkRec K;
            if (link == NLINK_NONE) {
                if (!cur_int && T.rsteps()[rq].next_edge == 0xFFFF) break;
                stop_here = true;
            } else {
                K = link_load(T.links(), link);
                const int st = tls_state(T, L, K.tls, K.tls_pos);
                if (K.tls != 0xFF && (st == TLS_R || st == TLS_Y) && seen >= bgv) stop_here = true;
                if (!stop_here && !(K.flags & KF_CONT) && ((K.flags & KF_MINOR) || (K.tls != 0xFF && st == TLS_g))) {
                    if (seen > RM_VIS_DIST) stop_here = true;
                    else if (K.foe_cnt > 0 && foe_blocked(T, L, grid, K)) stop_here = true;
                }
            }
            if (stop_here) {
                const float g = seen - RM_STOP_OFFSET;
                tgap = g > 0.0f ? g : 0.0f; tvl = 0.0f; tbl = b;
                have = true;
                break;
            }
            LR = K.dest;
            cur_lane = K.to_lane;
            {
                const float vnl = LR.vmax * sf;
                if (vnl < vfree) {
                    const float vs = d_free_speed(seen, vnl, b);
                    if (vs < vsafe) vsafe = vs;
                }
            }
            const Found od = rearmost_within(L, grid, LR.cell0, lane_cells(L, LR), look - seen + T.maxlen);
            if (od.slot != NIL) {
                const float *vo = L.vtp + od.vt() * VT_COLS;
                tgap = seen + od.pos() - vo[VT_LENGTH] - mingap;
                tvl = od.speed(); tbl = vo[VT_DECEL];
                have = true;
                break;
            }
            if (!cur_int) rq += 1;
            seen += LR.len;
            if (!(seen < look)) break;
        }
    }
    if (LONG) RS_SEC(10)
    if (have) {
        const float vs = d_follow_speed(tgap, tvl, b, tbl, tau);
        if (vs < vsafe) vsafe = vs;
    }
    float vmin_n = v - b; if (vmin_n < 0.0f) vmin_n = 0.0f;
    float vmin_e = v - vt[VT_EMERGENCY]; if (vmin_e < 0.0f) vmin_e = 0.0f;
    const float lo = vsafe > vmin_e ? vsafe : vmin_e;
    const float vmin = vmin_n < lo ? vmin_n : lo;
    float vmax = vfree < vsafe ? vfree : vsafe;
    if (vmax < vmin) vmax = vmin;
    const float sigma = P.sigma >= 0.0f ? P.sigma : vt[VT_SIGMA];
    float vd = vmax;
    if (sigma > 0.0f) {
        const float r = d_u01(d_hash(P.seed, (uint32_t)genv, (uint32_t)k, (uint32_t)t, 0u));
        if (vd < a) vd -= sigma * vd * r; else vd -= sigma * a * r;
        if (vd < 0.0f) vd = 0.0f;
    }
    const float vnext = vd > vmin ? vd : vmin;
    L.vnx[s] = vnext;
#ifdef RS_EMU_DEBUG
    if (s == rs_dbg_slot && (t == rs_dbg_t || rs_dbg_t < 0))
        printf("plan t %d slot %d lane %d x %.3f v %.3f lead %d have %d tgap %.3f tvl %.3f vsafe %.3f vfree %.3f vnext %.3f nlink %x\n", t, s, lane, x, v, lead,
               (int)have, tgap, tvl, vsafe, vfree, vnext, ax.nlink);
#endif
    if (LONG) RS_SEC(3)
    if (x + vnext > LR0.len) flag_mover(L, s, t);
    if (LONG) RS_SEC(15)
    (void)LR;
}

template <bool LONG, class LT> RS_DEV void phase_move(const KTab &T, const LT &L, const Grid &gnew, const State &G, const KParams &P, int env, size_t eo,
                       int t, bool last_tick, bool more, int s, int &active, int &halted, int &top) {
    const Aux ax = L.aux[s];
    const Node me = L.node[s];
    const int k = me.trip;
    int lane = ax.lane;
#ifdef RS_EMU_DEBUG
    {
        static int moved_at[65536];
        if (moved_at[s] == t + 1) { printf("slot %d moved twice in tick %d: fl %x lane %d trip %d\n", s, t, me.fl, lane, k); fflush(stdout); abort(); }
        moved_at[s] = t + 1;
    }
#endif
#ifdef RS_FIELD_LOADS
    LaneRec LR = rec_load16(T.lanes(), lane);
#endif
    uint32_t nb = T.notbest()[ax.rq];
    uint32_t kw = 0;
    if (more && (ax.nlink & NLINK_ARR)) kw = link_reg_word(T, ax.nlink);
    const float sfv = sf_of(me.sfq);
    float tl = G.tloss()[eo + s];
#ifndef RS_FIELD_LOADS
    LaneRec LR = rec_load16(T.lanes(), lane);
#endif
    const int sw = ax.swait;
    int swn = sw;
    const float vn = L.vnx[s];
    int rq = ax.rq;
    uint16_t nlink = ax.nlink;
    int link = (int)(nlink & 0x7FFF);
    bool relink = false;
    int side = 0;
    RS_ASSERT(LONG || (!(me.fl & (LCT_LEFT | LCT_RIGHT | LCT_SWAP_LEFT | LCT_SWAP_RIGHT)) && !(me.pos + vn > LR.len)))
    if (LONG && (me.fl & (LCT_LEFT | LCT_RIGHT | LCT_SWAP_LEFT | LCT_SWAP_RIGHT))) {
        if ((me.fl & (LCT_LEFT | LCT_RIGHT)) && !(me.pos + vn > LR.len)) side = (me.fl & LCT_LEFT) ? +1 : -1;
        else if (me.fl & (LCT_SWAP_LEFT | LCT_SWAP_RIGHT)) side = (me.fl & LCT_SWAP_LEFT) ? +1 : -1;
    }
    if (LONG && side) {
        lane += side;
        LR = rec_load16(T.lanes(), lane);
        nlink = cache_link(T, LR, lane, rq, k);
        link = (int)(nlink & 0x7FFF);
        relink = true;
    }
    const float vref = LR.vmax * sfv;
    if (last_tick && (P.out_mask & OUT_VEH_ACCEL)) G.accel()[eo + s] = vn - me.speed;
    if (vn <= RM_HALT_SPEED) {
        if (sw < 65535) swn = sw + 1;
        halted += 1;
        if (G.trip_log) { const int wt = G.wtot()[eo + s]; if (wt < 65535) G.wtot()[eo + s] = (uint16_t)(wt + 1); }
    } else swn = 0;
    if (vref > 0.0f && vn < vref) { tl += RS_DIV(vref - vn, vref); G.tloss()[eo + s] = tl; }
    float x = me.pos + vn;
    bool arrived = false;
    if (LONG) for (int it = 0; it < 16; ++it) {
        if (!(x > LR.len)) break;
        const bool li = (LR.flags & LF_INTERNAL) != 0;
        if (link == NLINK_NONE) {
            if (!li && T.rsteps()[rq].next_edge == 0xFFFF) arrived = true; else x = LR.len;
            break;
        }
        x -= LR.len;
        if (!li) rq += 1;
        {
            const LinkRec Km = link_load(T.links(), link);
            lane = Km.to_lane;
            LR = Km.dest;
        }
        nlink = cache_link(T, LR, lane, rq, k);
        link = (int)(nlink & 0x7FFF);
        relink = true;
    }
    if (LONG && arrived) {
        Aux na = ax; na.lane = LANE_NONE; na.swait = 0;
        L.aux[s] = na;
        L.node[s].trip = TRIP_NONE; L.node[s].fl = (uint8_t)(me.fl & fl_mh(t));
        rs_atomic_and(&L.alive[s >> 5], ~(1u << (s & 31)));
        {
            const int ow = G.owner()[eo + s];
            if (ow != (int)OWNER_NONE) rs_atomic_add(&L.sig_dep[ow], 1);
        }
        G.owner()[eo + s] = OWNER_NONE; G.rwait()[eo + s] = 0;
        rs_atomic_add(&L.sc[SC_NACT], -1);
        rs_atomic_add(&L.sc[SC_STATS + ST_ARRIVED], 1);
        rs_atomic_add(&L.sc[SC_STATS + ST_DURATION], t + 1 - (int)G.depart()[eo + s]);
        rs_atomic_add(&L.sc[SC_STATS + ST_TLOSS], (int)(tl * 1024.0f + 0.5f));
        if (G.trip_log) {
            int32_t *r = G.trip_log + ((size_t)env * T.n_trips + k) * 4;
            r[0] = (int)G.depart()[eo + s]; r[1] = t + 1; r[2] = (int)(tl * 1024.0f + 0.5f); r[3] = (int)G.wtot()[eo + s];
        }
        return;
    }
    active += 1;
    if (s + 1 > top) top = s + 1;
    Aux na = ax;
    na.lane = (uint16_t)lane; na.rq = (uint16_t)rq; na.swait = (uint16_t)swn;
    if (LONG && relink) na.nlink = nlink;
    L.aux[s] = na;
    Node nn = me;
    nn.pos = x; nn.speed = vn; nn.fl = (uint8_t)(me.fl & fl_mh(t));
    nn.nxt = grid_push(gnew, LR.cell0 + cell_of(L, x, lane_cells(L, LR)), s, vn > RM_HALT_SPEED);
    if (more) {
        if (LONG && relink) { nb = T.notbest()[rq]; if (na.nlink & NLINK_ARR) kw = link_reg_word(T, na.nlink); }
        nn.fl |= classify(T, L, s, L.vtp + me.vt * VT_COLS, vn, x, LR, lane, rq, nb, k, sfv, t + 1);
        L.node[s] = nn;
        if ((na.nlink & NLINK_ARR) && vn > RM_HALT_SPEED) register_approach_w(T, L, kw, vn, x, LR.len, me.vt);
    } else L.node[s] = nn;
    (void)P;
}

template <class LT> RS_DEV int overlapping(const LT &L, const Grid &grid, int cell0, int ncell, float pos, int k, int self, float len_self) {
    const int lead = leader_within(L, grid, cell0, ncell, pos, k, self, RM_NB_WINDOW);
    if (lead != NIL && L.node[lead].pos - L.vtp[L.node[lead].vt * VT_COLS + VT_LENGTH] - pos < 0.0f) return lead;
    const int foll = follower_within(L, grid, cell0, ncell, pos, k, self, RM_NB_WINDOW);
    if (foll != NIL && pos - len_self - L.node[foll].pos < 0.0f) return foll;
    return NIL;
}

template <class LT> RS_DEV int phase_lc_decide(const KTab &T, const LT &L, const Grid &grid, const State &G, size_t eo, int t, int s, const Aux &ax, const Node &me) {
    const int lane = ax.lane;
#ifdef RS_FIELD_LOADS
    const LaneRec LR = rec_load16(T.lanes(), lane);
    const ContRow R = cont_row(T, ax.rq);
#else
    const ContRow R = cont_row(T, ax.rq);
    const LaneRec LR = rec_load16(T.lanes(), lane);
#endif
    const int my_wait = (int)ax.swait;
    const int n = LR.flags >> 2;
    if ((LR.flags & LF_INTERNAL) || n < 2) return 0;
    const int dir_allowed = (t & 1) ? -1 : +1;
    const int l0 = LR.edge_lane0, kk = lane - l0;
    const int k = me.trip;
    const float *vt = L.vtp + me.vt * VT_COLS;
    const float x = me.pos, v = me.speed;
    const int nc = lane_cells(L, LR);
    int want = 0, dir = dir_allowed;
    float rem;
    const int sdir = strategic_dir(R, kk, n, x, v, 0, rem, grid, LR.cell0, nc, T.occ_unit);
    if (sdir != 0) { dir = sdir; want = 2; }
    int code = 0;
    const int tk = kk + dir;
    if (tk >= 0 && tk < n) {
        const int tcell0 = (int)LR.cell0 + dir * nc;
        int lead_t = NIL, foll_t = NIL;
        bool have_t = false;
        if (!want && !((((uint32_t)t >> 1) + (uint32_t)k) & 3u)) {
            float rem_t;
            if (strategic_dir(R, tk, n, x, v, RM_SG_EXTRA_LANES, rem_t, grid, tcell0, nc, T.occ_unit) == 0) {
                const int lead_c = leader_within(L, grid, LR.cell0, nc, x, k, s, RM_NB_WINDOW);
                if (lead_c != NIL) {
                    lead_t = leader_within(L, grid, tcell0, nc, x, k, s, RM_NB_WINDOW);
                    have_t = true;
                    const float gcur = L.node[lead_c].pos - L.vtp[L.node[lead_c].vt * VT_COLS + VT_LENGTH] - x;
                    float gtgt = RM_BIGF;
                    if (lead_t != NIL) gtgt = L.node[lead_t].pos - L.vtp[L.node[lead_t].vt * VT_COLS + VT_LENGTH] - x;
                    if (gcur < v * 3.0f + 15.0f && gtgt > gcur + RM_SG_ADVANTAGE) want = 1;
                }
            }
        }
        if (want) {
            if (!have_t) lead_t = leader_within(L, grid, tcell0, nc, x, k, s, RM_NB_WINDOW);
            foll_t = follower_within(L, grid, tcell0, nc, x, k, s, RM_NB_WINDOW);
            const bool urgent = want == 2 && rem <= RM_URGENT_DIST;
            bool safe = true;
            if (lead_t != NIL) {
                const Node ld = L.node[lead_t];
                const float *vo = L.vtp + ld.vt * VT_COLS;
                const float gap = ld.pos - vo[VT_LENGTH] - x - (urgent ? 0.0f : vt[VT_MINGAP]);
                const float dec = urgent ? vt[VT_EMERGENCY] : vt[VT_DECEL];
                float vb = v - dec; if (vb < 0.0f) vb = 0.0f;
                if (gap < 0.0f || vb > d_follow_speed(gap, ld.speed, vt[VT_DECEL], vo[VT_DECEL], vt[VT_TAU])) safe = false;
            }
            if (safe && foll_t != NIL) {
                const Node fd = L.node[foll_t];
                const float *vo = L.vtp + fd.vt * VT_COLS;
                const float gap = x - vt[VT_LENGTH] - fd.pos - (urgent ? 0.0f : vo[VT_MINGAP]);
                const float dec = urgent ? vo[VT_EMERGENCY] : vo[VT_DECEL];
                float vb = fd.speed - dec; if (vb < 0.0f) vb = 0.0f;
                if (gap < 0.0f || vb > d_follow_speed(gap, v, vo[VT_DECEL], vt[VT_DECEL], vo[VT_TAU])) safe = false;
            }
            if (safe) {
                if (dir == dir_allowed) code = dir > 0 ? LCT_LEFT : LCT_RIGHT;
            } else if (want == 2) {
                if (lead_t != NIL) { G.cooplead(t & 1)[eo + s] = ((uint32_t)L.node[lead_t].trip << 16) | (uint32_t)lead_t; mail_flag_set(L, s, t & 1); }
                const int R = at_or_behind_within(L, grid, tcell0, nc, x - vt[VT_LENGTH], RM_COOP_RANGE);
                if (R != NIL) { rs_atomic_min(&G.coop(t & 1)[eo + R], ((uint32_t)k << 16) | (uint32_t)s); mail_flag_set(L, R, t & 1); }
            }
        }
    }
    if (sdir != 0 && (t % RM_SWAP_EVERY) == 0 && v <= RM_HALT_SPEED && rem <= RM_URGENT_DIST &&
        my_wait >= RM_SWAP_WAIT) {
        const int b = overlapping(L, grid, (int)LR.cell0 + sdir * nc, nc, x, k, s, vt[VT_LENGTH]);
        if (b != NIL) {
            const Node nb = L.node[b];
            float rem_b;
            if (nb.speed <= RM_HALT_SPEED && (int)L.aux[b].swait >= RM_SWAP_WAIT &&
                strategic_dir(cont_row(T, L.aux[b].rq), kk + sdir, n, nb.pos, nb.speed, 0, rem_b, grid, (int)LR.cell0 + sdir * nc, nc, T.occ_unit) == -sdir && rem_b <= RM_URGENT_DIST &&
                overlapping(L, grid, LR.cell0, nc, nb.pos, nb.trip, b, L.vtp[nb.vt * VT_COLS + VT_LENGTH]) == s)
                code |= sdir > 0 ? LCT_SWAP_LEFT : LCT_SWAP_RIGHT;
        }
    }
        return code;
}

template <class LT> RS_DEV bool phase_insert_decide(const KTab &T, const LT &L, const Grid &grid, int t, int d) {
    if ((int)L.dep_t[d] > t) return false;
    const int k = L.dep[d];
    const DepInfo LR = rec_load8(T.cold.dep_info, d);
    const float *vt = L.vtp + T.trip_vtype()[k] * VT_COLS;
    const float mypos = vt[VT_LENGTH] < LR.len ? vt[VT_LENGTH] : LR.len;
    const int nc = (int)(LR.len * L.cell_inv) + 1;
    const int c1 = LR.cell0 + cell_of(L, mypos + vt[VT_MINGAP] + T.maxlen, nc);
    for (int c = scan_up(grid, LR.cell0, c1); c >= 0; c = (c < c1 ? scan_up(grid, c + 1, c1) : -1))
        for (int o = cell_head(grid, c); o != NIL;) { RS_CHAIN_GUARD
            const Node od = L.node[o];
            const float back = (od.pos + L.vnx[o]) - L.vtp[od.vt * VT_COLS + VT_LENGTH];
            if (back - mypos - vt[VT_MINGAP] < 0.0f) return false;
            o = od.nxt;
        }
    return true;
}

template <class LT> RS_DEV int nth_free_slot(const LT &L, int C, int r) {
#pragma unroll 1
    for (int w = 0; w < (C + 31) / 32; ++w) {
        uint32_t fr = ~L.alive0[w];
        if (w == (C - 1) / 32 && (C & 31)) fr &= (1u << (C & 31)) - 1u;
        const int c = rs_popc(fr);
        if (r >= c) { r -= c; continue; }
#pragma unroll 1
        for (int j = 0; j < r; ++j) fr &= fr - 1u;
        return w * 32 + rs_ffs(fr) - 1;
    }
    return -1;
}

template <class LT> RS_DEV void lc_decide_and_flag(const KTab &T, const LT &L, const Grid &grid, const State &G, size_t eo, int t, int s) {
    const Aux ax = L.aux[s];
    if (ax.lane == LANE_NONE) return;
    const int code = phase_lc_decide(T, L, grid, G, eo, t, s, ax, L.node[s]);
    if (code) flag_mover(L, s, t, code);
}
struct ExecInline {};

template <int CAP, class Exec, class LT>
RS_DEV void rs_step_body_on(Exec &ex, const LT &L, const KTab &T, const State &G, const Out &O, const KParams &P,
                            const int32_t *actions, int env) {
    const int B = ex.B;
    const int C = CAP ? CAP : T.capacity, S = T.n_signals, NO = T.n_obs;
    const int genv = P.env_base + env;
    const size_t eo = (size_t)env * C;
    const int n_ticks = P.n_ticks;

    uint16_t *const grid0 = L.grid;

    ex.phase(0, [&](int tid) {
        if (tid < SC_STATS + ST_N) L.sc[tid] = tid < 4 ? G.env[env * 4 + tid] : 0;
        for (int i = tid; i < T.n_vtypes * VT_COLS; i += B) L.vtp[i] = T.cold.vtype_params[i];
        for (int i = tid; i < (int)(L.gstride >> 1); i += B) ((uint32_t *)grid0)[i] = 0x07FF07FFu;
        for (int i = tid; i < T.n_arr; i += B) L.arr[i] = ARR_NONE;
        for (int i = tid; i < (C + 31) / 32; i += B) { L.alive[i] = 0u; L.mailw[i] = 0u; }
        for (int i = tid; i < (T.n_dep + 31) / 32; i += B) L.insm[i] = 0u;
        for (int i = tid; i < T.n_dep; i += B) {
            const int k = G.dep_next[(size_t)env * T.n_dep + i];
            L.dep[i] = (uint16_t)k;
            L.dep_t[i] = k == (int)TRIP_NONE ? (uint16_t)0xFFFF : (uint16_t)T.cold.trip_depart[k];
        }
        for (int i = tid; i < S; i += B) {
            const int ph = G.tls[(env * S + i) * TLS_W + 0];
            L.phase[i] = ph;
            L.left[i] = G.tls[(env * S + i) * TLS_W + 1];
            L.nextp[i] = G.tls[(env * S + i) * TLS_W + 2];
            L.sig_arr[i] = 0; L.sig_dep[i] = G.tls[(env * S + i) * TLS_W + 3];
            tls_refresh(T, L, P, i, ph);
        }
    });
    ex.phase(1, [&](int tid) {
        const int hw0 = L.sc[SC_HW];
        for (int s = tid; s < C; s += B) {
            uint16_t ln = LANE_NONE, tr = TRIP_NONE;
            if (s < hw0) { ln = G.lane()[eo + s]; tr = G.trip()[eo + s]; }
            Aux ax; ax.lane = ln; ax.rq = 0; ax.nlink = NLINK_NONE; ax.swait = 0;
            if (ln == LANE_NONE) { L.aux[s] = ax; L.node[s].trip = TRIP_NONE; continue; }
            const float sp = G.speed()[eo + s], x = G.pos()[eo + s];
            const int rq = (int)T.routes()[T.trip_route()[tr]].start + (int)G.cursor()[eo + s];
            const LaneRec LR0 = rec_load16(T.lanes(), ln);
            ax.rq = (uint16_t)rq;
            ax.nlink = cache_link(T, LR0, ln, rq, tr);
            ax.swait = G.swait()[eo + s];
            L.aux[s] = ax;
            Node nn; nn.pos = x; nn.speed = sp; nn.trip = tr; nn.vt = T.trip_vtype()[tr];
            nn.fl = 0; nn.sfq = (uint16_t)speed_factor_q(P, genv, tr, L.vtp + nn.vt * VT_COLS);
            if ((G.mail[(size_t)env * ((C + 31) / 32) + (s >> 5)] >> (s & 31)) & 1u) nn.sfq |= (uint16_t)SFQ_MAIL((L.sc[SC_T] + 1) & 1);
            nn.nxt = grid_push(Grid{grid0, 0u}, LR0.cell0 + cell_of(L, x, lane_cells(L, LR0)), s, sp > RM_HALT_SPEED);
            if (n_ticks > 0) nn.fl = (uint8_t)classify(T, L, s, L.vtp + nn.vt * VT_COLS, sp, x, LR0, ln, rq, T.notbest()[rq], tr, sf_of(nn.sfq), L.sc[SC_T]);
            L.node[s] = nn;
            rs_atomic_or(&L.alive[s >> 5], 1u << (s & 31));
        }
        for (int s = B - 1 - tid; s < S; s += B) {
            if (P.do_fsm && !P.fixed_program) {
                const int a = actions[env * S + s], cur = L.phase[s], Gn = T.cold.tls_ngreen[s];
                if (a < 0 || a >= T.cold.tls_nphase[s]) L.nextp[s] = cur;
                else {
                    L.nextp[s] = a;
                    if (cur != a && cur < Gn && a < Gn) {
                        const int y = T.cold.tls_yellow[T.cold.tls_yel_off[s] + cur * Gn + a];
                        if (y >= 0) set_phase(T, L, P, s, y);
                    }
                }
            }
            if (n_ticks > 0) tls_begin_of_tick(T, L, P, s, 0);
        }
    });
    if (n_ticks > 0) ex.phase(2, [&](int tid) {
        const int hw = L.sc[SC_HW];
        for (int s = tid; s < hw; s += B) {
            const Aux ax = L.aux[s];
            if (ax.lane == LANE_NONE) continue;
            const Node me = L.node[s];
            register_approach(T, L, ax.nlink, me.speed, me.pos, T.lanes()[ax.lane].len, me.vt);
        }
    });

    int cur = 0;
    for (int tick = 0; tick < n_ticks; ++tick) {
        const int t = L.sc[SC_T], hw = L.sc[cur ? SC_HWNEW : SC_HW];
        const Grid gold{grid0, cur ? CELL_TAG : 0u}, gnew{grid0, cur ? 0u : CELL_TAG};
        const bool more = tick + 1 < n_ticks;
        const int lcap = (int)L.lcap;
        const int nwv = B >> 6;
        ex.phase(4, [&](int tid) {
            const int wv = ex.wave_of(tid), ln = tid & 63;
            const int nh = L.sc[SC_NH], nlc = L.sc[SC_NLC];
            const unsigned long long r0 = ex.role_begin();
            int role = 0;
            if (nh > lcap || nlc > lcap) {
                for (int pass = 0; pass < 2; ++pass)
                    for (int w = tid; w < hw; w += B) {
                        if (pass && !(L.node[w].fl & FL_LC)) continue;
                        if (pass) lc_decide_and_flag(T, L, gold, G, eo, t, w);
                        else phase_plan<true>(T, L, gold, G, eo, P, genv, t, w);
                    }
            } else {
                const int hch = (nh + RS_H_CHUNK - 1) / RS_H_CHUNK, lch = (nlc + RS_LIST_CHUNK - 1) / RS_LIST_CHUNK;
                const int total = hch + lch + ((hw + 63) >> 6);
                for (int it = 0;; ++it) {
                    const int c = ex.next_chunk(&L.sc[SC_CHUNK_P], wv, it, nwv);
                    if (c >= total) break;
                    if (c < hch) {
                        role = 1;
                        const int w = c * RS_H_CHUNK + ln;
                        if (ln < RS_H_CHUNK && w < nh) phase_plan<true>(T, L, gold, G, eo, P, genv, t, L.ls_h[w]);
                    } else if (c < hch + lch) {
                        role = 2;
                        const int w = (c - hch) * RS_LIST_CHUNK + ln;
                        if (ln < RS_LIST_CHUNK && w < nlc) lc_decide_and_flag(T, L, gold, G, eo, t, L.ls_lc[w]);
                    } else {
                        const int w = (c - hch - lch) * 64 + ln;
                        if (w < hw && !(L.node[w].fl & FL_H)) phase_plan<false>(T, L, gold, G, eo, P, genv, t, w);
                    }
                }
            }
            ex.role_end(role == 1 ? 7 : (role == 2 ? 8 : 9), r0);
            for (int i = tid; i < (T.n_dep + 31) / 32; i += B) L.insm[i] = 0u;
        });
        ex.phase(5, [&](int tid) {
            for (int i = tid; i < T.n_arr; i += B) L.arr[i] = ARR_NONE;
            for (int i = tid; i < (C + 31) / 32; i += B) L.alive0[i] = L.alive[i];
            int Bs = B;
            RS_OPAQUE_S(Bs)
            for (int i = tid; i < (int)(L.gstride >> 2); i += Bs) {
                unsigned long long *q = (unsigned long long *)grid0 + i;
                const unsigned long long w = *q;
                const unsigned long long st = ((w ^ grid_tag4(gold)) >> 15) & 0x0001000100010001ull;
                if (st) { const unsigned long long m = st * 0xFFFFull; *q = (w & ~m) | ((0x07FF07FF07FF07FFull | grid_tag4(gold)) & m); }
            }
            for (int d = B - 1 - tid; d < T.n_dep; d += B)
                if (phase_insert_decide(T, L, gold, t, d)) rs_atomic_or(&L.insm[d >> 5], 1u << (d & 31));
            if (more)
                for (int sg = B - 1 - tid; sg < S; sg += B) tls_begin_of_tick(T, L, P, sg, tick + 1);
            if (tid == 0) {
                L.sc[SC_T] = t + 1; L.sc[SC_STATS + ST_TICKS] += 1;
                L.sc[cur ? SC_HW : SC_HWNEW] = 0;
                L.sc[SC_ROOM] = C - L.sc[SC_NACT];
                L.sc[SC_NH] = 0; L.sc[SC_NLC] = 0;
                L.sc[SC_NMH + ((t + 1) & 1)] = 0;
                L.sc[SC_CHUNK_P] = 0; L.sc[SC_CHUNK_M] = 0;
            }
        });
        ex.phase(6, [&](int tid) {
            int active = 0, halted = 0, top = 0;
            const int wv = ex.wave_of(tid), ln = tid & 63;
            const int nmh = L.sc[SC_NMH + (t & 1)];
            int ich = 0;
            for (int i = 0; i < (T.n_dep + 31) / 32; ++i) if (L.insm[i]) ich = 1;
            const bool all = nmh > lcap;
            const int mch = all ? 0 : (nmh + RS_LIST_CHUNK - 1) / RS_LIST_CHUNK;
            const int total = mch + ich + ((hw + 63) >> 6);
            const unsigned long long r0 = ex.role_begin();
            bool list = false;
            for (int it = 0;; ++it) {
                const int c = ex.next_chunk(&L.sc[SC_CHUNK_M], wv, it, nwv);
                if (c >= total) break;
                if (c < mch) {
                    list = true;
                    const int w = c * RS_LIST_CHUNK + ln;
                    if (ln < RS_LIST_CHUNK && w < nmh) phase_move<true>(T, L, gnew, G, P, env, eo, t, !more, more, L.ls_mh[w], active, halted, top);
                } else if (c < mch + ich) {
                    for (int d = 63 - ln; d < T.n_dep; d += 64) {
                        if (!(L.insm[d >> 5] & (1u << (d & 31)))) continue;
                        int rank = rs_popc(L.insm[d >> 5] & ((1u << (d & 31)) - 1u));
                        for (int w = 0; w < (d >> 5); ++w) rank += rs_popc(L.insm[w]);
                        if (rank >= L.sc[SC_ROOM]) { rs_atomic_add(&L.sc[SC_STATS + ST_CAP_BLOCKED], 1); continue; }
                        const int s = nth_free_slot(L, C, rank);
                        if (s < 0) continue;
                        const int k = L.dep[d];
                        const int v = T.trip_vtype()[k];
                        const float *vt = L.vtp + v * VT_COLS;
                        const RouteRec RR = rec_load16(T.routes(), T.trip_route()[k]);
                        const LaneRec LRd = rec_load16(T.lanes(), RR.depart_lane);
                        const int sfq = speed_factor_q(P, genv, k, vt);
                        const float sfn = sf_of(sfq);
                        Node nn; nn.pos = vt[VT_LENGTH] < RR.depart_len ? vt[VT_LENGTH] : RR.depart_len;
                        nn.speed = 0.0f; nn.trip = (uint16_t)k; nn.vt = (uint8_t)v; nn.fl = 0; nn.sfq = (uint16_t)sfq;
                        nn.nxt = grid_push(gnew, LRd.cell0 + cell_of(L, nn.pos, lane_cells(L, LRd)), s, false);
                        if (more) nn.fl = (uint8_t)classify(T, L, s, vt, 0.0f, nn.pos, LRd, RR.depart_lane, (int)RR.start, T.notbest()[RR.start], k, sfn, t + 1);
                        L.node[s] = nn;
                        Aux na; na.lane = RR.depart_lane; na.rq = (uint16_t)RR.start; na.swait = 0;
                        na.nlink = cache_link(T, LRd, RR.depart_lane, (int)RR.start, k);
                        L.aux[s] = na;
                        G.sf()[eo + s] = sfn; G.tloss()[eo + s] = 0.0f; G.cooplead(0)[eo + s] = COOP_NONE; G.cooplead(1)[eo + s] = COOP_NONE; G.coop(0)[eo + s] = COOP_NONE; G.coop(1)[eo + s] = COOP_NONE;
                        G.rwait()[eo + s] = 0; G.owner()[eo + s] = OWNER_NONE; G.depart()[eo + s] = (uint16_t)(t + 1); G.accel()[eo + s] = 0.0f; G.wtot()[eo + s] = 0;
                        {
                            const int k2 = T.cold.trip_next[k];
                            L.dep[d] = (uint16_t)k2;
                            L.dep_t[d] = k2 == (int)TRIP_NONE ? (uint16_t)0xFFFF : (uint16_t)T.cold.trip_depart[k2];
                        }
                        rs_atomic_or(&L.alive[s >> 5], 1u << (s & 31));
                        rs_atomic_add(&L.sc[SC_NACT], 1);
                        rs_atomic_add(&L.sc[SC_NINS], 1);
                        rs_atomic_add(&L.sc[SC_STATS + ST_INSERTED], 1);
                        rs_atomic_add(&L.sc[SC_STATS + ST_DEPDELAY], t - T.cold.trip_depart[k]);
                        if (s + 1 > top) top = s + 1;
                    }
                } else {
                    const int w = (c - mch - ich) * 64 + ln;
                    if (w < hw && (L.alive0[w >> 5] & (1u << (w & 31)))) {
                        if (all) phase_move<true>(T, L, gnew, G, P, env, eo, t, !more, more, w, active, halted, top);
                        else if (!(L.node[w].fl & fl_mh(t))) phase_move<false>(T, L, gnew, G, P, env, eo, t, !more, more, w, active, halted, top);
                    }
                }
            }
            ex.role_end(list ? 10 : 3, r0);
            rs_wave_add(&L.sc[SC_STATS + ST_ACTIVE_TICKS], active);
            rs_wave_add(&L.sc[SC_STATS + ST_WAITING], halted);
            rs_wave_max(&L.sc[cur ? SC_HW : SC_HWNEW], top);
            ex.role_end(15, r0);
        });
        cur ^= 1;
    }
    const int hw_end = L.sc[cur ? SC_HWNEW : SC_HW];

    const bool obs = P.do_observe != 0;
    if (obs) ex.phase(11, [&](int tid) {
        for (int i = tid; i < NO; i += B) { L.agg_q[i] = 0; L.agg_a[i] = 0; L.agg_w[i] = 0; L.agg_m[i] = 0; L.agg_s[i] = 0; L.agg_n[i] = 0; }
    });
    ex.phase(12, [&](int tid) {
        const int hw0 = G.env[env * 4 + 2];
        const int top = hw_end > hw0 ? hw_end : hw0;
        int hi = 0;
        for (int s = tid; s < top; s += B) {
            const int lane = L.aux[s].lane;
            G.lane()[eo + s] = (uint16_t)lane; G.trip()[eo + s] = L.node[s].trip;
            if (lane == (int)LANE_NONE) continue;
            hi = s + 1;
            if (L.node[s].sfq & SFQ_MAIL((L.sc[SC_T] + 1) & 1)) rs_atomic_or(&L.mailw[s >> 5], 1u << (s & 31));
            const int rq = L.aux[s].rq;
            G.pos()[eo + s] = L.node[s].pos; G.speed()[eo + s] = L.node[s].speed; G.swait()[eo + s] = L.aux[s].swait;
            G.cursor()[eo + s] = (uint16_t)(rq - (int)T.routes()[T.trip_route()[L.node[s].trip]].start);
            if (!obs) continue;
            const int prev_owner = G.owner()[eo + s];
            const LaneRec LR = T.lanes()[lane];
            const int oi = T.cold.lane_obs[lane];
            bool detect = false;
            if (oi >= 0) {
                const float d = (LR.len - L.node[s].pos) + T.rsteps()[rq].tlsdist;
                detect = d <= P.max_distance;
            }
            if (!detect) {
                if (prev_owner != (int)OWNER_NONE) rs_atomic_add(&L.sig_dep[prev_owner], 1);
                G.owner()[eo + s] = OWNER_NONE; G.rwait()[eo + s] = 0;
                continue;
            }
            const int sig = T.cold.obs_sig[oi];
            int rw = G.rwait()[eo + s];
            if (prev_owner != sig) {
                rw = 0;
                rs_atomic_add(&L.sig_arr[sig], 1);
                rs_atomic_add(&L.agg_n[oi], 1);
                if (prev_owner != (int)OWNER_NONE) rs_atomic_add(&L.sig_dep[prev_owner], 1);
            }
            if (rw > 0) { rw += T.step_length; if (rw > 65535) rw = 65535; }
            else { const int sw = L.aux[s].swait; if (sw > 0) rw = sw; }
            G.rwait()[eo + s] = (uint16_t)rw;
            G.owner()[eo + s] = (uint8_t)sig;
            if (rw > 0) { rs_atomic_add(&L.agg_q[oi], 1); rs_atomic_add(&L.agg_w[oi], rw); rs_atomic_max(&L.agg_m[oi], rw); }
            else rs_atomic_add(&L.agg_a[oi], 1);
            rs_atomic_add((int32_t *)&L.agg_s[oi], (int32_t)(uint32_t)(L.node[s].speed * 65536.0f + 0.5f));
        }
        if (hi) rs_atomic_max(&L.sc[SC_HWOUT], hi);
    });
    ex.phase(13, [&](int tid) {
        const uint32_t om = obs ? P.out_mask : 0u;
        if (om & (OUT_LANE_AGG | OUT_DRQ_NORM)) for (int i = tid; i < NO * 5; i += B) {
            const int oi = i / 5, c = i - oi * 5;
            const int sg = T.cold.obs_sig[oi];
            const float sp = (float)L.agg_s[oi] * (1.0f / 65536.0f);
            float raw, nrm;
            if (c == 0) { raw = (float)L.agg_q[oi]; nrm = (oi - T.cold.sig_obs_start[sg]) == L.phase[sg] ? 1.0f : 0.0f; }
            else if (c == 1) { raw = (float)L.agg_a[oi]; nrm = raw / 28.0f; }
            else if (c == 2) { raw = (float)L.agg_w[oi]; nrm = raw / 28.0f; }
            else if (c == 3) { raw = (float)L.agg_m[oi]; nrm = (float)L.agg_q[oi] / 28.0f; }
            else { raw = sp; nrm = sp / 20.0f / 28.0f; }
            if (om & OUT_LANE_AGG) O.lane_agg()[(size_t)env * NO * 5 + i] = raw;
            if (om & OUT_DRQ_NORM) O.drq_norm()[(size_t)env * NO * 5 + i] = nrm;
        }
        if (om & OUT_LANE_ARR) for (int i = tid; i < NO; i += B) O.lane_arr()[(size_t)env * NO + i] = L.agg_n[i];
        if (om & OUT_DRQ_F16) for (int i = tid; i < S * T.lmax * 5; i += B) {
            const int sg = i / (T.lmax * 5), r = i - sg * T.lmax * 5;
            const int l = r / 5, c = r - l * 5;
            const int o0 = T.cold.sig_obs_start[sg];
            float nrm = 0.0f;
            if (l < T.cold.sig_obs_start[sg + 1] - o0) {
                const int oi = o0 + l;
                if (c == 0) nrm = l == L.phase[sg] ? 1.0f : 0.0f;
                else if (c == 1) nrm = (float)L.agg_a[oi] / 28.0f;
                else if (c == 2) nrm = (float)L.agg_w[oi] / 28.0f;
                else if (c == 3) nrm = (float)L.agg_q[oi] / 28.0f;
                else nrm = (float)L.agg_s[oi] * (1.0f / 65536.0f) / 20.0f / 28.0f;
            }
            O.drq_f16()[(size_t)env * S * T.lmax * 5 + i] = rs_f2h(nrm);
        }
        if (om & (OUT_MPLIGHT | OUT_WAVE | OUT_MPLIGHT_FULL)) for (int i = tid; i < S * 12; i += B) {
            const int sg = i / 12, m = i - sg * 12;
            int q = 0, wv = 0, tw = 0, ap = 0;
            float last_speed = 0.0f;
            for (int j = T.cold.mv_in_start[i]; j < T.cold.mv_in_start[i + 1]; ++j) {
                const int oi = T.cold.mv_in_idx[j];
                q += L.agg_q[oi]; wv += L.agg_q[oi] + L.agg_a[oi]; tw += L.agg_w[oi]; ap += L.agg_a[oi];
                last_speed = (float)L.agg_s[oi] * (1.0f / 65536.0f);
            }
            for (int j = T.cold.mv_out_start[i]; j < T.cold.mv_out_start[i + 1]; ++j) q -= L.agg_q[T.cold.mv_out_idx[j]];
            const size_t so = (size_t)env * S + sg;
            if (om & OUT_MPLIGHT) O.mplight()[so * 13 + 1 + m] = q;
            if (om & OUT_WAVE) O.wave()[so * 12 + m] = wv;
            if (om & OUT_MPLIGHT_FULL) {
                float *mf = O.mplight_full() + so * 49 + 1 + m * 4;
                mf[0] = (float)q; mf[1] = (float)tw / 28.0f; mf[2] = last_speed; mf[3] = (float)ap / 28.0f;
            }
        }
        for (int sg = tid; sg < S; sg += B) {
            const int ph = L.phase[sg];
            if (obs) {
                const int o0 = T.cold.sig_obs_start[sg], o1 = T.cold.sig_obs_start[sg + 1];
                int tw = 0, tq = 0, mq = 0;
                for (int oi = o0; oi < o1; ++oi) { tw += L.agg_w[oi]; const int qq = L.agg_q[oi]; tq += qq; if (qq > mq) mq = qq; }
                const size_t so = (size_t)env * S + sg;
                O.phase()[so] = ph; O.queue_sum()[so] = tq; O.queue_max()[so] = mq;
                O.wait()[so] = -(float)tw;
                const float wn = -(float)tw / 224.0f;
                O.wait_norm()[so] = wn < -4.0f ? -4.0f : (wn > 4.0f ? 4.0f : wn);
                int pr = tq;
                for (int i = T.cold.pr_out_start[sg]; i < T.cold.pr_out_start[sg + 1]; ++i) pr -= L.agg_q[T.cold.pr_out_idx[i]];
                O.pressure()[so] = -pr;
                if (om & OUT_MPLIGHT) O.mplight()[so * 13] = ph;
                if (om & OUT_MPLIGHT_FULL) O.mplight_full()[so * 49] = (float)ph;
                O.arrivals()[so] = L.sig_arr[sg]; O.departures()[so] = L.sig_dep[sg];
            }
            G.tls[(env * S + sg) * TLS_W + 0] = ph;
            G.tls[(env * S + sg) * TLS_W + 1] = L.left[sg];
            G.tls[(env * S + sg) * TLS_W + 2] = L.nextp[sg];
            G.tls[(env * S + sg) * TLS_W + 3] = obs ? 0 : L.sig_dep[sg];
        }
        for (int i = tid; i < T.n_dep; i += B) G.dep_next[(size_t)env * T.n_dep + i] = L.dep[i];
        for (int i = tid; i < (C + 31) / 32; i += B) G.mail[(size_t)env * ((C + 31) / 32) + i] = L.mailw[i];
    });
    ex.phase(14, [&](int tid) {
        if (tid == 0) {
            G.env[env * 4 + 0] = L.sc[SC_T]; G.env[env * 4 + 1] = L.sc[SC_NINS]; G.env[env * 4 + 3] = L.sc[SC_NACT];
            G.env[env * 4 + 2] = L.sc[SC_HWOUT];
        }
        if (tid < ST_N) {
            long long *st = G.stats + (size_t)env * ST_N;
            if (tid == ST_ACTIVE) st[tid] = L.sc[SC_NACT];
            else if (tid == ST_PENDING) {
                const int t = L.sc[SC_T];
                const int hz = t - 1 <= T.horizon ? t - 1 : T.horizon;
                st[tid] = (t >= 1 ? T.cold.trips_cum[hz] : 0) - L.sc[SC_NINS];
            } else st[tid] += L.sc[SC_STATS + tid];
        }
    });
}

template <int CAP, class Exec>
RS_DEV void rs_step_body(Exec &ex, const Lds &L, const KTab &T, const State &G, const Out &O, const KParams &P,
                         const int32_t *actions, int env) {
    if constexpr (CAP != 0) {
        const LdsFix<CAP> Lf(L);
        rs_step_body_on<CAP>(ex, Lf, T, G, O, P, actions, env);
    } else rs_step_body_on<CAP>(ex, L, T, G, O, P, actions, env);
}
```

resco_amd/csrc/resco_tables.h:

```cpp
#pragma once
#include <stdint.h>
#include <string.h>
#include <string>
#include <vector>

#include "resco_model.h"
#include "resco_sim.h"

enum { VT_LENGTH, VT_MINGAP, VT_ACCEL, VT_DECEL, VT_TAU, VT_SIGMA, VT_MAXSPEED, VT_SF_MEAN, VT_SF_DEV, VT_EMERGENCY, VT_COLS };
enum { TLS_R = 0, TLS_Y = 1, TLS_g = 2, TLS_G = 3 };
enum { ST_INSERTED, ST_ARRIVED, ST_DURATION, ST_DEPDELAY, ST_WAITING, ST_TLOSS, ST_ACTIVE, ST_PENDING, ST_ACTIVE_TICKS, ST_TICKS, ST_CAP_BLOCKED, ST_INVARIANT, ST_N };

#define LANE_NONE 0xFFFFu
#define OWNER_NONE 0xFFu
#define NIL 0x7FF
#define CELL_CNT_SHIFT 11
#define CELL_CNT_MAX 7u
#define CELL_MOVER 0x4000u
#define CELL_TAG 0x8000u
#define ARR_NONE 65535
#define COOP_NONE 0xFFFFFFFFu
#define TRIP_NONE 0xFFFFu

#ifdef CELL_LEN
// ... 6 lines not shown

struct __attribute__((aligned(16))) LaneRec {
    float len, vmax;
    uint16_t link_start;
    uint8_t link_cnt;
    uint8_t flags;
    uint16_t cell0;
    uint16_t edge_lane0;
};
struct __attribute__((aligned(16))) LinkRec {
    uint16_t to_lane, to_edge, foe_start, via2;
    int16_t arr_idx;
    uint8_t tls, tls_pos;
    uint8_t foe_cnt, flags;
    uint8_t dest_k, pad;
    LaneRec dest;
};
struct __attribute__((aligned(16))) FoeRec {
    int16_t arr_idx;
    uint8_t tls, tls_pos;
    uint16_t via1_cell0, via2_cell0;
    uint8_t via1_nc, via2_nc, pad[6];
};
struct __attribute__((aligned(8))) RStep {
    uint16_t edge, next_edge;
    float tlsdist;
};
struct __attribute__((aligned(16))) RouteRec {
    uint32_t start;
    uint16_t depart_lane;
    int16_t dep_idx;
    uint16_t depart_cell0;
    uint16_t pad;
    float depart_len;
};
#define LF_INTERNAL 1u
#define KF_MINOR 1u
#define KF_CONT 2u
#define NLINK_NONE 0x7FFF
#define NLINK_ARR 0x8000

struct __attribute__((aligned(8))) DepInfo { float len; uint16_t cell0, lane; };
struct KCold {
    const int32_t *trip_depart;
    const uint16_t *trip_next;
    const uint16_t *dep_lane;
    const struct DepInfo *dep_info;
    const uint16_t *dep_first;
    const float *vtype_params;
    const uint8_t *tls8, *fix8;
    const int32_t *tls_nphase, *tls_ngreen, *tls_nlinks, *tls_state_off, *tls_dur_off, *tls_yel_off, *tls_dur, *tls_yellow, *tls_init_phase;
    const int32_t *fix_nphase, *fix_state_off, *fix_dur_off, *fix_dur, *fix_init_phase, *fix_init_left;
    const int16_t *lane_obs;
    const int32_t *obs_sig, *sig_obs_start, *mv_in_start, *mv_in_idx, *mv_out_start, *mv_out_idx, *pr_out_start, *pr_out_idx;
    const int32_t *trips_cum;
};
#ifndef RS_G
#define RS_G(p) (p)
#endif
#ifndef RS_MEM
#define RS_MEM inline
#endif
#ifndef RS_KEEP4
#define RS_KEEP4(a, b, c, d)
#endif
#ifndef RS_KEEP2
#define RS_KEEP2(a, b)
#endif
static_assert(sizeof(LaneRec) == 16 && alignof(LaneRec) == 16, "LaneRec: one 16-byte load");
static_assert(sizeof(FoeRec) == 16 && alignof(FoeRec) == 16, "FoeRec: one 16-byte load");
static_assert(sizeof(RouteRec) == 16 && alignof(RouteRec) == 16, "RouteRec: one 16-byte load");
static_assert(sizeof(LinkRec) == 32 && alignof(LinkRec) == 16, "LinkRec: two 16-byte loads");
static_assert(sizeof(RStep) == 8 && alignof(RStep) == 8, "RStep: one 8-byte load");
static_assert(sizeof(DepInfo) == 8 && alignof(DepInfo) == 8, "DepInfo: one 8-byte load");
#ifdef RS_FIELD_LOADS
#define rec_load16(tab, i) ((tab)[i])
#define rec_load8(tab, i) ((tab)[i])
#define link_load(tab, i) ((tab)[i])
#else
struct alignas(16) RecRaw16 { uint32_t a, b, c, d; };
template <class R, class I> RS_MEM R rec_load16(const R *tab, I i) {
    static_assert(sizeof(R) == 16 && alignof(R) == 16, "rec_load16: a 16-byte record");
    RecRaw16 r;
    __builtin_memcpy(&r, &tab[i], 16);
    RS_KEEP4(r.a, r.b, r.c, r.d)
    R out;
    __builtin_memcpy(&out, &r, 16);
    return out;
}
template <class R, class I> RS_MEM R rec_load8(const R *tab, I i) {
    static_assert(sizeof(R) == 8 && alignof(R) == 8, "rec_load8: an 8-byte record");
    struct alignas(8) Raw { uint32_t a, b; } r;
    __builtin_memcpy(&r, &tab[i], 8);
    RS_KEEP2(r.a, r.b)
    R out;
    __builtin_memcpy(&out, &r, 8);
    return out;
}
template <class I> RS_MEM LinkRec link_load(const LinkRec *tab, I i) {
    RecRaw16 r[2];
    __builtin_memcpy(r, &tab[i], 32);
    RS_KEEP4(r[0].a, r[0].b, r[0].c, r[0].d)
    RS_KEEP4(r[1].a, r[1].b, r[1].c, r[1].d)
    LinkRec out;
    __builtin_memcpy(&out, r, 32);
    return out;
}
#endif

struct KTab {
    const LaneRec *lanes_;
    const LinkRec *links_;
    const FoeRec *foes_;
    const RStep *rsteps_;
    const float *route_cont_;
    const uint16_t *next_link_;
    const uint16_t *notbest_;
    const RouteRec *routes_;
    const uint16_t *trip_route_;
    const uint8_t *trip_vtype_;
    KCold cold;
    float maxlen;
    float occ_unit;
    int32_t n_trips, tls_maxl, kmax;
    int32_t n_lanes, n_cells, n_signals, n_obs, n_vtypes, horizon, capacity, step_length, yellow_length, lmax, n_arr, n_dep;
    RS_MEM const LaneRec *lanes() const { return RS_G(lanes_); }
    RS_MEM const LinkRec *links() const { return RS_G(links_); }
    RS_MEM const FoeRec *foes() const { return RS_G(foes_); }
    RS_MEM const RStep *rsteps() const { return RS_G(rsteps_); }
    RS_MEM const float *route_cont() const { return RS_G(route_cont_); }
    RS_MEM const uint16_t *next_link() const { return RS_G(next_link_); }
    RS_MEM const uint16_t *notbest() const { return RS_G(notbest_); }
    RS_MEM const RouteRec *routes() const { return RS_G(routes_); }
    RS_MEM const uint16_t *trip_route() const { return RS_G(trip_route_); }
    RS_MEM const uint8_t *trip_vtype() const { return RS_G(trip_vtype_); }
};

struct KParams {
    uint32_t seed;
    int32_t env_base;
    float max_distance, sigma;
    int32_t speed_dev, fixed_program;
    int32_t tls_expiry;
    int32_t n_ticks;
    int32_t do_fsm;
    int32_t do_observe;
    uint32_t out_mask;
    int32_t n_envs;
    unsigned long long *prof;
};

#define OUT_LANE_AGG 1u
#define OUT_DRQ_NORM 2u
#define OUT_DRQ_F16 4u
#define OUT_LANE_ARR 8u
#define OUT_MPLIGHT 16u
#define OUT_WAVE 32u
#define OUT_MPLIGHT_FULL 64u
#define OUT_VEH_ACCEL 128u
#define OUT_ALL 255u
#define TLS_W 4

struct PackedTables {
    std::vector<LaneRec> lanes;
    std::vector<LinkRec> links;
    std::vector<FoeRec> foes;
    std::vector<RStep> rsteps;
    std::vector<RouteRec> routes;
    std::vector<uint16_t> next_link, trip_route, trip_next, dep_lane, dep_first, notbest;
    std::vector<uint8_t> trip_vtype, tls8, fix8;
    std::vector<DepInfo> dep_info;
    std::vector<int32_t> tls_off_p, fix_off_p;
    std::vector<int16_t> lane_obs16;
    std::vector<int32_t> obs_sig;
    std::vector<float> route_cont;
    int n_cells = 0, n_arr = 1, n_dep = 1, kmax = 1, lmax = 1, tls_maxl = 1;
    float maxlen = 0.0f, occ_unit = 0.0f;
    float cell_len = 30.0f, cell_inv = 1.0f / 30.0f;
    std::string err;

    static void choose(const rs_scenario *sc, int q, int ln, int out[2]) {
        out[0] = out[1] = -1;
        const int ne = sc->route_edge[q + 1];
        const float *cn = sc->route_cont + (size_t)(q + 1) * sc->kmax;
// ... 196 lines not shown
```

resco_amd/sim.py:

```python
import ctypes as C
import os

import numpy as np

from ._abi import ParamsStruct, PPOTrainStruct, RolloutStruct, TrainStruct, pack_scenario

_HERE = os.path.dirname(os.path.abspath(__file__))
LIB_PATH = os.environ.get('RESCO_SIM_LIB') or os.path.join(_HERE, 'csrc', 'libresco_sim.so')

BUFFERS = ['lane_agg', 'drq_norm', 'phase', 'mplight', 'wave', 'wait', 'wait_norm', 'pressure', 'queue_sum',
           'queue_max', 'actions', 'env', 'tls', 'veh_pos', 'veh_speed', 'veh_accel', 'veh_tloss', 'veh_lane',
           'veh_trip', 'veh_cursor', 'veh_swait', 'veh_rwait', 'veh_depart', 'veh_owner', 'stats', 'drq_norm_f16',
           'veh_sf', 'veh_wtot', 'trip_log', 'dep_next', 'veh_coop', 'veh_cooplead', 'arrivals', 'departures',
           'mplight_full', 'lane_arrivals', 'veh_coop_odd', 'veh_cooplead_odd', 'veh_mail']
BUF_ID = {n: i for i, n in enumerate(BUFFERS)}
OUTPUT_GROUPS = ('lane_agg', 'drq_norm', 'drq_norm_f16', 'lane_arrivals', 'mplight', 'wave', 'mplight_full', 'veh_accel')
_NP_DTYPES = [np.float32, np.int32, np.uint16, np.uint8, np.float16, np.int64, np.uint32]
_TYPESTR = ['<f4', '<i4', '<u2', '|u1', '<f2', '<i8', '<u4']
STAT_KEYS = ['inserted', 'arrived', 'sum_duration', 'sum_depart_delay', 'sum_waiting', 'sum_time_loss_q10',
             'active', 'pending', 'active_ticks', 'ticks', 'cap_blocked', 'invariant']
TRIP_NONE = 0xFFFF

ABI_SYMBOLS = ['rs_create', 'rs_destroy', 'rs_last_error', 'rs_reset', 'rs_step', 'rs_sync', 'rs_reinit_signals', 'rs_ticks', 'rs_step_sim', 'rs_set_outputs', 'rs_act_random',
               'rs_act_maxwave', 'rs_get_buffer', 'rs_read_buffer', 'rs_stats', 'rs_snapshot', 'rs_restore',
               'rs_snapshot_free', 'rs_timing', 'rs_timing_read', 'rs_set_seed', 'rs_phase_profile', 'rs_info',
               'rs_idqn_create', 'rs_idqn_act', 'rs_idqn_set_device_weights', 'rs_idqn_set_lanes', 'rs_idqn_destroy', 'rs_group_step',
               'rs_default_block', 'rs_mplight_create', 'rs_mplight_act', 'rs_mplight_set_device_weights', 'rs_mplight_destroy',
               'rs_ippo_act', 'rs_group_rollout', 'rs_ppo_gae',
               'rs_ppo_create', 'rs_ppo_grad', 'rs_ppo_step', 'rs_ppo_fit', 'rs_ppo_steps', 'rs_ppo_destroy',
               'rs_dqn_create', 'rs_dqn_sample', 'rs_dqn_grad', 'rs_dqn_step', 'rs_dqn_update', 'rs_dqn_steps', 'rs_dqn_destroy',
               'rs_mplight_dqn_create', 'rs_mplight_dqn_sample', 'rs_mplight_dqn_grad', 'rs_mplight_dqn_step', 'rs_mplight_dqn_update',
               'rs_mplight_dqn_steps', 'rs_mplight_dqn_destroy',
               'rs_idqn_pack_weights', 'rs_dqn_sync_target', 'rs_mplight_dqn_sync_target', 'rs_group_train',
               'rs_ppo_perm', 'rs_ippo_pack_weights', 'rs_group_ppo_train']

FMA2C_SYMBOLS = ['rs_fma2c_create', 'rs_fma2c_act', 'rs_fma2c_value', 'rs_fma2c_reset', 'rs_fma2c_set_device_weights', 'rs_fma2c_buffer',
                 'rs_fma2c_destroy', 'rs_fma2c_learn_create', 'rs_fma2c_learn_grad', 'rs_fma2c_learn_step', 'rs_fma2c_learn_update',
                 'rs_fma2c_learn_reset', 'rs_fma2c_learn_buffer', 'rs_fma2c_learn_destroy']

_lib = None


def bind(L):
    vp, i32, u32, f32 = C.c_void_p, C.c_int32, C.c_uint32, C.c_float
    L.rs_create.argtypes = [vp, vp, i32, i32, i32, i32, C.POINTER(vp)]
    L.rs_destroy.argtypes = [vp]
    L.rs_destroy.restype = None
    L.rs_last_error.argtypes = [vp]
    L.rs_last_error.restype = C.c_char_p
    L.rs_reset.argtypes = [vp, vp]
    L.rs_step.argtypes = [vp, vp, i32, vp]
    L.rs_sync.argtypes = [vp]
    L.rs_ticks.argtypes = [vp, i32, vp]
    L.rs_step_sim.argtypes = [vp, i32, vp]
    L.rs_set_outputs.argtypes = [vp, C.c_uint64]
    L.rs_reinit_signals.argtypes = [vp, vp]
    L.rs_act_random.argtypes = [vp, C.c_uint32, vp]
    L.rs_act_maxwave.argtypes = [vp, vp, i32, vp, vp, i32, vp]
    L.rs_get_buffer.argtypes = [vp, i32, C.POINTER(vp), C.POINTER(C.c_int64), C.POINTER(i32), C.POINTER(i32)]
    L.rs_read_buffer.argtypes = [vp, i32, vp, C.c_int64]
    L.rs_stats.argtypes = [vp, vp]
    L.rs_snapshot.argtypes = [vp, C.POINTER(vp)]
    L.rs_restore.argtypes = [vp, vp]
    L.rs_snapshot_free.argtypes = [vp, vp]
    L.rs_snapshot_free.restype = None
    L.rs_timing.argtypes = [vp, i32]
    L.rs_timing_read.argtypes = [vp, C.POINTER(C.c_float), C.POINTER(i32)]
    L.rs_set_seed.argtypes = [vp, C.c_uint32]
    L.rs_phase_profile.argtypes = [vp, i32, vp]
    L.rs_info.argtypes = [vp, C.POINTER(i32), C.POINTER(i32), C.POINTER(i32), C.POINTER(i32)]
    L.rs_group_step.argtypes = [vp, i32, vp, i32]
    if hasattr(L, 'rs_idqn_create'):
        L.rs_idqn_create.argtypes = [i32, i32, i32] + [vp] * 9 + [C.POINTER(vp)]
        L.rs_idqn_act.argtypes = [vp, vp, i32, i32, i32, f32, u32, u32, vp, vp, vp, vp]
        L.rs_idqn_set_lanes.argtypes = [vp, vp]
        L.rs_idqn_set_device_weights.argtypes = [vp] * 9
        L.rs_idqn_destroy.argtypes = [vp]
        L.rs_idqn_destroy.restype = None
    if hasattr(L, 'rs_mplight_create'):
        L.rs_mplight_create.argtypes = [i32, i32, i32, vp, i32, vp, vp, vp, C.POINTER(vp)]
        L.rs_mplight_act.argtypes = [vp, vp, i32, i32, f32, u32, u32, vp, vp, vp, vp, vp]
        L.rs_mplight_set_device_weights.argtypes = [vp, vp]
        L.rs_mplight_destroy.argtypes = [vp]
        L.rs_mplight_destroy.restype = None
    if hasattr(L, 'rs_group_rollout'):
        L.rs_ippo_act.argtypes = [vp, vp, i32, i32, u32, u32, vp, vp, vp, vp, vp, vp]
        L.rs_group_rollout.argtypes = [vp, i32, vp, vp, i32, i32]
        L.rs_ppo_gae.argtypes = [vp, vp, vp, vp, i32, i32, i32, f32, f32, vp, vp, vp, vp]
    if hasattr(L, 'rs_ppo_create'):
        L.rs_ppo_create.argtypes = [i32, i32, i32, vp, vp, i32, vp, vp, vp, vp, vp, i32, C.POINTER(vp)]
        L.rs_ppo_grad.argtypes = [vp, vp, vp, vp, vp, vp, vp, i32, vp, vp]
        L.rs_ppo_step.argtypes = [vp, vp]
        L.rs_ppo_fit.argtypes = [vp, vp, vp, vp, vp, vp, i32, vp, i32, i32, vp, vp]
        L.rs_ppo_steps.argtypes = [vp]
        L.rs_ppo_steps.restype = C.c_int64
        L.rs_ppo_destroy.argtypes = [vp]
        L.rs_ppo_destroy.restype = None
    if hasattr(L, 'rs_dqn_create'):
        L.rs_dqn_create.argtypes = [i32, i32, i32, vp, vp, i32, vp, vp, vp, vp, vp, vp, i32, C.POINTER(vp)]
        L.rs_dqn_sample.argtypes = [vp, vp, i32, u32, u32, vp, vp]
        L.rs_dqn_grad.argtypes = [vp, vp, vp, i32, vp, vp]
        L.rs_dqn_step.argtypes = [vp, vp]
        L.rs_dqn_update.argtypes = [vp, vp, i32, u32, i32, vp, vp]
        L.rs_dqn_steps.argtypes = [vp]
        L.rs_dqn_steps.restype = C.c_int64
        L.rs_dqn_destroy.argtypes = [vp]
        L.rs_dqn_destroy.restype = None
    if hasattr(L, 'rs_mplight_dqn_create'):
        L.rs_mplight_dqn_create.argtypes = [i32, i32, i32, vp, i32, vp, vp, vp, vp, vp, vp, i32, C.POINTER(vp)]
        L.rs_mplight_dqn_sample.argtypes = [vp, vp, i32, u32, u32, vp, vp]
        L.rs_mplight_dqn_grad.argtypes = [vp, vp, vp, i32, vp, vp]
        L.rs_mplight_dqn_step.argtypes = [vp, vp]
        L.rs_mplight_dqn_update.argtypes = [vp, vp, i32, u32, i32, vp, vp]
        L.rs_mplight_dqn_steps.argtypes = [vp]
        L.rs_mplight_dqn_steps.restype = C.c_int64
        L.rs_mplight_dqn_destroy.argtypes = [vp]
        L.rs_mplight_dqn_destroy.restype = None
    if hasattr(L, 'rs_group_train'):
        L.rs_idqn_pack_weights.argtypes = [vp, vp, vp]
        L.rs_dqn_sync_target.argtypes = [vp, vp]
        L.rs_mplight_dqn_sync_target.argtypes = [vp, vp]
        L.rs_group_train.argtypes = [vp, i32, vp, i32]
    if hasattr(L, 'rs_group_ppo_train'):
        L.rs_ppo_perm.argtypes = [i32, i32, u32, u32, vp, vp]
        L.rs_ippo_pack_weights.argtypes = [vp, vp, vp]
        L.rs_group_ppo_train.argtypes = [vp, i32, vp, i32]
    if hasattr(L, 'rs_fma2c_create'):
        L.rs_fma2c_create.argtypes = [i32, vp, vp, i32, C.POINTER(vp)]
        L.rs_fma2c_act.argtypes = [vp, vp, i32, i32, u32, u32, vp, vp, vp, vp, vp, vp]
        L.rs_fma2c_value.argtypes = [vp, vp, i32, i32, vp, vp]
        L.rs_fma2c_reset.argtypes = [vp, i32, i32, i32, vp]
        L.rs_fma2c_set_device_weights.argtypes = [vp, vp]
        L.rs_fma2c_buffer.argtypes = [vp, i32, C.POINTER(vp)]
        L.rs_fma2c_destroy.argtypes = [vp]
        L.rs_fma2c_destroy.restype = None
    if hasattr(L, 'rs_fma2c_learn_create'):
        L.rs_fma2c_learn_create.argtypes = [vp, vp, i32, i32, C.POINTER(vp)]
        L.rs_fma2c_learn_grad.argtypes = [vp, vp, vp, vp, vp, vp, vp, i32, vp, vp]
        L.rs_fma2c_learn_step.argtypes = [vp, vp]
        L.rs_fma2c_learn_update.argtypes = [vp, vp, vp, vp, vp, vp, vp, i32, vp, vp, vp]
        L.rs_fma2c_learn_reset.argtypes = [vp, vp]
        L.rs_fma2c_learn_buffer.argtypes = [vp, i32, C.POINTER(vp)]
        L.rs_fma2c_learn_destroy.argtypes = [vp]
        L.rs_fma2c_learn_destroy.restype = None
    if hasattr(L, 'rs_default_block'):
        L.rs_default_block.argtypes = [i32, i32, i32]
        L.rs_default_block.restype = i32
    return L


def load_library():
    global _lib
    if _lib is not None:
        return _lib
# ... 148 lines not shown
    mean, dev = np.float32(vt_row[7]), np.float32(vt_row[8])
    f = mean
    if speed_dev:
        s = np.float32(0.0)
        for i in range(4):
            s = np.float32(s + np.float32(_murmur(seed, (env, trip, 0xFFFFFFFF, i)) >> 8) * np.float32(1.0 / 16777216.0))
        z = np.float32((s - np.float32(2.0)) * np.float32(1.7320508))
        f = np.float32(mean + np.float32(dev * z))
    f = min(max(np.float32(f), np.float32(0.2)), np.float32(2.0))
    return float(np.float32(int(np.float32(f * np.float32(4096.0)) + np.float32(0.5))) * np.float32(1.0 / 4096.0))


def torch_stream(device=None):
    import torch
    p = torch.cuda.current_stream(device).cuda_stream
    return p if p else 1


class _DevArray:

    def __init__(self, ptr, shape, dtype_code, owner):
        self.__cuda_array_interface__ = dict(shape=tuple(shape), typestr=_TYPESTR[dtype_code],
                                             data=(int(ptr), False), version=2, strides=None)
        self._owner = owner


class BatchedSim:

    def __init__(self, scenario, n_envs, device=0, seed=0, max_distance=200.0, sigma=-1.0, speed_dev=1,
                 fixed_program=0, env_base=0, step_length=10, yellow_length=None, block_threads=0, trip_log=0, step_ratio=1,
                 tls_expiry=1, device_envs=None):
        self.sc = scenario
        self.n_envs = int(n_envs)
        self.device = int(device)
        self._lib = self._load()
        if yellow_length is not None and int(yellow_length) != int(scenario.yellow_length):
            raise ValueError('scenario %s was compiled with yellow_length=%d (asked %d)' % (scenario.name, scenario.yellow_length, yellow_length))
        self._st, self._keep = pack_scenario(scenario, step_length, yellow_length)
        self._p = ParamsStruct(int(seed) & 0xFFFFFFFF, float(max_distance), float(sigma), int(speed_dev),
                               int(fixed_program), int(trip_log), int(step_ratio), 0 if tls_expiry else 1)
        self.step_ratio = max(1, int(step_ratio))
        self._h = C.c_void_p()
        if not block_threads and device_envs and int(device_envs) != self.n_envs and hasattr(self._lib, 'rs_default_block'):
            block_threads = self._lib.rs_default_block(int(scenario.capacity), int(device_envs), self.device)
        rc = self._lib.rs_create(C.byref(self._st), C.byref(self._p), self.n_envs, int(env_base), self.device,
                                 int(block_threads), C.byref(self._h))
        if rc != 0:
            msg = self._lib.rs_last_error(None)
            self._h = None
            raise RuntimeError('rs_create failed (%d): %s' % (rc, msg.decode() if msg else '?'))
        self.S, self.O, self.C = scenario.n_signals, scenario.n_obs, scenario.capacity
        self.seed, self.env_base, self.speed_dev = int(seed) & 0xFFFFFFFF, int(env_base), int(speed_dev)
        self._maxwave_ready = False
        self._masked_off = frozenset()
        self._dep_cache = None
        self._meta = {}
        for name, bid in BUF_ID.items():
            ptr, shape, nd, dt = C.c_void_p(), (C.c_int64 * 4)(), C.c_int32(), C.c_int32()
            self._check(self._lib.rs_get_buffer(self._h, bid, C.byref(ptr), shape, C.byref(nd), C.byref(dt)))
            self._meta[name] = (ptr.value, tuple(shape[:nd.value]), dt.value)

    def _load(self):
        return load_library()

    def _check(self, rc):
        if rc != 0:
            msg = self._lib.rs_last_error(self._h)
            raise RuntimeError('resco_sim error %d: %s' % (rc, msg.decode() if msg else '?'))

    def close(self):
        if getattr(self, '_h', None):
            self._lib.rs_destroy(self._h)
            self._h = None

    def __del__(self):
        try:
            self.close()
        except Exception:
            pass

    def info(self):
        a, b, c, d = C.c_int32(), C.c_int32(), C.c_int32(), C.c_int32()
        self._check(self._lib.rs_info(self._h, C.byref(a), C.byref(b), C.byref(c), C.byref(d)))
        return dict(n_envs=a.value, block_threads=b.value, lds_bytes=c.value, max_lanes_per_signal=d.value)

    def reset(self, stream=None):
        self._check(self._lib.rs_reset(self._h, stream))

    def step(self, actions=None, stream=None):
        if actions is None:
            self._check(self._lib.rs_step(self._h, None, 0, stream))
            return
        if hasattr(actions, 'data_ptr'):
            assert tuple(actions.shape) == (self.n_envs, self.S) and actions.is_contiguous()
            assert str(actions.dtype) == 'torch.int32'
            self._check(self._lib.rs_step(self._h, actions.data_ptr(), 1 if actions.is_cuda else 0, stream))
            return
        a = np.ascontiguousarray(actions, dtype=np.int32)
        assert a.shape == (self.n_envs, self.S), a.shape
        self._check(self._lib.rs_step(self._h, a.ctypes.data, 0, stream))

    def ticks(self, n, stream=None):
        self._check(self._lib.rs_ticks(self._h, int(n), stream))

    def step_sim(self, n=1, stream=None):
        self._check(self._lib.rs_step_sim(self._h, int(n), stream))

    def set_outputs(self, names=None):
        mask = 0
        for n in (OUTPUT_GROUPS if names is None else names):
            if n not in OUTPUT_GROUPS:
                raise ValueError('%r is not a maskable output buffer (%s)' % (n, ', '.join(OUTPUT_GROUPS)))
            mask |= 1 << BUF_ID[n]
        self._check(self._lib.rs_set_outputs(self._h, mask))
        self._masked_off = frozenset(OUTPUT_GROUPS) - frozenset(OUTPUT_GROUPS if names is None else names)

    def require_output(self, name):
        if name in self._masked_off:
            raise RuntimeError('output buffer %r is switched off (BatchedSim.set_outputs): re-enable it before reading it' % name)

    def reinit_signals(self, stream=None):
        self._check(self._lib.rs_reinit_signals(self._h, stream))

    def set_seed(self, seed):
        self.seed = int(seed) & 0xFFFFFFFF
        self._check(self._lib.rs_set_seed(self._h, self.seed))

    def sync(self):
        self._check(self._lib.rs_sync(self._h))

    def act_random(self, step_key, stream=None):
        self._check(self._lib.rs_act_random(self._h, int(step_key) & 0xFFFFFFFF, stream))

    def act_maxwave(self, use_pressure, stream=None):
        if not self._maxwave_ready:
            pairs, valid, order = maxwave_tables(self.sc)
            self._pairs, self._valid, self._order = pairs, valid, order
            self._check(self._lib.rs_act_maxwave(self._h, pairs.ctypes.data, len(pairs), valid.ctypes.data,
                                                 order.ctypes.data, int(use_pressure), stream))
            self._maxwave_ready = True
            return
        self._check(self._lib.rs_act_maxwave(self._h, None, len(self._pairs), None, None, int(use_pressure), stream))

    def _ensure_maxwave_tables(self, use_pressure):
        if not self._maxwave_ready:
            self.act_maxwave(use_pressure)

    def read(self, name):
        ptr, shape, dt = self._meta[name]
        out = np.empty(shape, _NP_DTYPES[dt])
        if out.nbytes == 0:
            return out
        self._check(self._lib.rs_read_buffer(self._h, BUF_ID[name], out.ctypes.data, out.nbytes))
        return out

    def tensor(self, name, allow_masked=False):
        import torch
        if not allow_masked:
            self.require_output(name)
        ptr, shape, dt = self._meta[name]
        return torch.as_tensor(_DevArray(ptr, shape, dt, self), device='cuda:%d' % self.device)

    def device_pointer(self, name):
        return self._meta[name]

    def outputs(self, names=('lane_agg', 'drq_norm', 'phase', 'mplight', 'wave', 'wait', 'wait_norm', 'pressure',
                             'queue_sum', 'queue_max')):
# ... 136 lines not shown
```

Measured before the change: 3.994 million env-steps/s.

## Specialise step kernel per shipped map with compile-time scenario constants

Generates a header of per-map constexpr scenario constants (table sizes, LDS layout offsets, capacity, register budget) at build time and instantiates a dedicated step kernel per shipped map. At create time the host matches the loaded scenario against these and launches the specialised kernel, falling back to the generic one. The goal is to remove kernarg loads and runtime address arithmetic and let the compiler fold LDS offsets and loop bounds. It also switches record loads to 32-bit byte offsets, with a new cap on n_envs*capacity. The cost is a more complex build, longer compile time and more kernel instances.

```diff
diff --git a/include/resco_sim.h b/include/resco_sim.h
--- a/include/resco_sim.h
+++ b/include/resco_sim.h
@@ -309,6 +309,7 @@
 void rs_fma2c_learn_destroy(rs_fma2c_learn_handle l);
 
 int rs_info(rs_handle h, int32_t *n_envs, int32_t *block_threads, int32_t *lds_bytes, int32_t *max_lanes_per_signal);
+const char *rs_info_kernel(rs_handle h);
 
 #ifdef __cplusplus
 }
diff --git a/resco_amd/build.py b/resco_amd/build.py
--- a/resco_amd/build.py
+++ b/resco_amd/build.py
@@ -1,4 +1,7 @@
+import ctypes
+import glob
 import os
+import re
 import subprocess
 
 HERE = os.path.dirname(os.path.abspath(__file__))
@@ -6,15 +9,118 @@
 SRC = os.path.join(HERE, 'csrc', 'resco_sim.hip')
 LIB = os.path.join(HERE, 'csrc', 'libresco_sim.so')
 HIPCC = os.environ.get('HIPCC', '/opt/rocm/bin/hipcc')
+GEN_DIR = os.path.join(HERE, 'csrc', '_gen')
+SCN_SRC = os.path.join(HERE, 'csrc', 'resco_scn_consts.cpp')
+SCN_LIB = os.path.join(GEN_DIR, 'libresco_scn_consts.so')
+SCN_HEADER = os.path.join(GEN_DIR, 'resco_scn_fix.h')
+SCENARIO_DIR = os.path.join(HERE, 'scenarios')
+CXX = os.environ.get('CXX', 'g++')
 FLAGS = ['--offload-arch=gfx950', '-O3', '-std=c++17', '-ffp-contract=off', '-fno-honor-nans', '-mllvm', '-disable-machine-licm', '-fPIC', '-shared',
-         '-I' + os.path.join(ROOT, 'include'), '-I' + os.path.join(HERE, 'csrc')]
-_DEPS = [SRC] + [os.path.join(HERE, 'csrc', f) for f in ('resco_host.h', 'resco_step.h', 'resco_tables.h', 'resco_policy.h', 'resco_frap.h', 'resco_fma2c.h', 'resco_fma2c_train.h', 'resco_ppo.h', 'resco_train.h', 'resco_ppo_train.h', 'resco_dqn_train.h', 'resco_frap_train.h', 'resco_group_train.h', 'resco_ppo_loop.h')] + \
+         '-I' + os.path.join(ROOT, 'include'), '-I' + os.path.join(HERE, 'csrc'), '-I' + GEN_DIR]
+_HDRS = [os.path.join(HERE, 'csrc', f) for f in ('resco_host.h', 'resco_step.h', 'resco_tables.h')] + \
         [os.path.join(ROOT, 'include', f) for f in ('resco_sim.h', 'resco_model.h')]
+_DEPS = [SRC] + _HDRS + [os.path.join(HERE, 'csrc', f) for f in ('resco_policy.h', 'resco_frap.h', 'resco_fma2c.h', 'resco_fma2c_train.h', 'resco_ppo.h', 'resco_train.h', 'resco_ppo_train.h', 'resco_dqn_train.h', 'resco_frap_train.h', 'resco_group_train.h', 'resco_ppo_loop.h')]
+
+
+def _newer(target, deps):
+    return os.path.exists(target) and all(os.path.getmtime(target) >= os.path.getmtime(d) for d in deps)
+
+
+def _replace(path, write):
+    tmp = '%s.%d.tmp' % (path, os.getpid())
+    write(tmp)
+    os.replace(tmp, path)
+
+
+def build_scn_consts_library(force=False):
+    if not force and _newer(SCN_LIB, [SCN_SRC] + _HDRS):
+        return SCN_LIB
+    os.makedirs(GEN_DIR, exist_ok=True)
+    _replace(SCN_LIB, lambda tmp: subprocess.check_call(
+        [CXX, '-O1', '-std=c++17', '-fPIC', '-shared', '-ffp-contract=off', '-I' + os.path.join(ROOT, 'include'), '-I' + os.path.join(HERE, 'csrc'),
+         SCN_SRC, '-o', tmp, '-lm']))
+    return SCN_LIB
+
+
+def scn_consts(scenario, lib=None, **pack):
+    from ._abi import pack_scenario
+    L = ctypes.CDLL(lib or build_scn_consts_library())
+    L.rs_scn_const_names.restype = ctypes.c_char_p
+    names = L.rs_scn_const_names().decode().split(',')
+    st, keep = pack_scenario(scenario, **pack)
+    out = (ctypes.c_uint32 * len(names))()
+    L.rs_scn_consts.argtypes = [ctypes.c_void_p, ctypes.c_void_p]
+    rc = L.rs_scn_consts(ctypes.byref(st), out)
+    del keep
+    if rc != 0:
+        raise RuntimeError('rs_scn_consts failed (%d)' % rc)
+    signed = lambda n, v: v - (1 << 32) if v >= (1 << 31) and not (n.startswith('o_') or n.endswith('_bits')) else v
+    return {n: signed(n, int(v)) for n, v in zip(names, out)}
+
+
+def shipped_maps():
+    out = []
+    for path in sorted(glob.glob(os.path.join(SCENARIO_DIR, '*.npz'))):
+        name = os.path.splitext(os.path.basename(path))[0]
+        if re.fullmatch(r'[A-Za-z][A-Za-z0-9_]*', name):
+            out.append((name, path))
+    return out
+
+
+def scn_fix_text(consts_by_map):
+    lines = ['// GENERATED by resco_amd/build.py from resco_amd/scenarios/*.npz (rs_scn_consts of every shipped map) -- not in git, do not edit.',
+             '// One struct per map: the members of ScnConsts (resco_step.h) as literals; RS_SCN_MAPS lists the maps.', '#pragma once', '#include <stdint.h>']
+    for name, consts in consts_by_map.items():
+        lines.append('struct ScnFix_%s {' % name)
+        for k, v in consts.items():
+            if k.startswith('o_') or k.endswith('_bits') or v < 0:
+                lines.append('    static constexpr %s %s = %s;' % ('int32_t' if v < 0 else 'uint32_t', k, v if v < 0 else '0x%08xu' % v))
+            else:
+                lines.append('    static constexpr int32_t %s = %d;' % (k, v))
+        lines.append('};')
+    lines.append('#define RS_SCN_MAPS(X)' + ''.join(' X(%s)' % name for name in consts_by_map))
+    return '\n'.join(lines) + '\n'
+
+
+def generate_scn_header(verbose=False):
+    from .scenario import Scenario
+    maps = shipped_maps()
+    inputs = [SCN_SRC] + _HDRS + [path for _, path in maps] + [os.path.join(HERE, f) for f in ('build.py', '_abi.py', 'scenario.py')]
+    if _newer(SCN_HEADER, inputs) and _newer(SCN_LIB, [SCN_SRC] + _HDRS):
+        return SCN_HEADER
+    consts = {}
+    try:
+        lib = build_scn_consts_library()
+    except (OSError, subprocess.CalledProcessError) as e:
+        print('resco_amd.build: no specialised step kernels, the host-only constants library did not build: %s' % e)
+        lib, maps = None, []
+    for name, path in maps:
+        try:
+            consts[name] = scn_consts(Scenario.load(path), lib)
+        except Exception as e:
+            print('resco_amd.build: no specialised step kernel for %s: %s' % (name, e))
+    text = scn_fix_text(consts)
+    old = None
+    if os.path.exists(SCN_HEADER):
+        with open(SCN_HEADER) as f:
+            old = f.read()
+    if text != old:
+        def write(tmp):
+            with open(tmp, 'w') as f:
+                f.write(text)
+        os.makedirs(GEN_DIR, exist_ok=True)
+        _replace(SCN_HEADER, write)
+    elif not _newer(LIB, [SCN_HEADER]):
+        os.utime(SCN_HEADER)
+    if verbose:
+        print('%s: %s' % (SCN_HEADER, ' '.join(consts) or '(no map)'))
+    return SCN_HEADER
 
 
 def build_library(force=False, verbose=False):
     force = force or os.environ.get('GRAFT_FORCE_BUILD') == '1'
-    if not force and os.path.exists(LIB) and all(os.path.getmtime(LIB) >= os.path.getmtime(d) for d in _DEPS):
+    header = generate_scn_header(verbose)
+    if not force and _newer(LIB, _DEPS + [header]):
         return LIB
     cmd = [HIPCC] + FLAGS + [SRC, '-o', LIB]
     if verbose:
diff --git a/resco_amd/csrc/resco_host.h b/resco_amd/csrc/resco_host.h
--- a/resco_amd/csrc/resco_host.h
+++ b/resco_amd/csrc/resco_host.h
@@ -163,6 +163,28 @@
     K.horizon = sc->horizon; K.capacity = sc->capacity; K.step_length = sc->step_length; K.yellow_length = sc->yellow_length * ratio; K.lmax = PT.lmax;
     K.n_arr = PT.n_arr; K.n_dep = PT.n_dep;
 }
+static inline void rs_scn_consts_from(const PackedTables &PT, const rs_scenario *sc, int ratio, ScnConsts *c, Lds *L = nullptr) {
+    KTab K{};
+    rs_ktab_scalars(K, PT, sc, ratio);
+    Lds l{};
+    const size_t bytes = lds_carve(&l, sc->capacity, K.n_cells, K.n_arr, K.n_dep, sc->n_obs, sc->n_signals, sc->n_vtypes, K.tls_maxl);
+    l.cell_inv = PT.cell_inv;
+#define X(n) c->n = K.n;
+    RS_SCN_KTAB(X)
+#undef X
+#define X(n) memcpy(&c->n##_bits, &K.n, 4);
+    RS_SCN_KTAB_F(X)
+#undef X
+    scn_consts_layout(c, l, bytes);
+    c->budget = rs_default_budget(sc->capacity, bytes);
+    if (L) *L = l;
+}
+static inline bool rs_scn_consts_of(const rs_scenario *sc, int ratio, ScnConsts *c) {
+    PackedTables PT;
+    if (rs_pack_tables(PT, sc)) return false;
+    rs_scn_consts_from(PT, sc, ratio, c);
+    return true;
+}
 static inline KParams rs_kparams(const rs_params *p, int32_t env_base, int32_t n_envs) {
     KParams P{};
     P.seed = p->seed; P.env_base = env_base; P.max_distance = p->max_distance; P.sigma = p->sigma;
diff --git a/resco_amd/csrc/resco_scn_consts.cpp b/resco_amd/csrc/resco_scn_consts.cpp
--- /dev/null
+++ b/resco_amd/csrc/resco_scn_consts.cpp
@@ -0,0 +1,49 @@
+#include <math.h>
+#include <stdint.h>
+#include <stddef.h>
+#include <string.h>
+#include <string>
+
+#include "resco_sim.h"
+
+#define RS_DEV static inline
+#define RS_HD
+#define RS_MEM inline
+#define RS_CARVE static inline
+#define RS_SMEM ((char *)0)
+#define RS_LAYOUT_ONLY
+#include "resco_host.h"
+
+extern "C" {
+int rs_scn_consts(const rs_scenario *sc, ScnConsts *out) {
+    if (!sc || !out) return RS_EINVAL;
+    return rs_scn_consts_of(sc, 1, out) ? RS_OK : RS_ELIMIT;
+}
+const char *rs_scn_const_names(void) { return RS_SCN_NAMES; }
+const char *rs_step_args_layout(void) {
+    static std::string s;
+    if (!s.empty()) return s.c_str();
+    auto add = [&](const char *name, const char *cls, size_t off, size_t bytes) {
+        s += std::string(name) + ":" + cls + ":" + std::to_string(off) + ":" + std::to_string(bytes) + ",";
+    };
+    const size_t T = offsetof(StepArgs, T), G = offsetof(StepArgs, G), O = offsetof(StepArgs, O), L = offsetof(StepArgs, L), GP = offsetof(StepArgs, GP);
+    add("T.tables", "pointer", T, offsetof(KTab, cold));
+    add("T.cold", "pointer", T + offsetof(KTab, cold), sizeof(KCold));
+#define X(n) add("T." #n, "const", T + offsetof(KTab, n), 4);
+    RS_SCN_KTAB(X) RS_SCN_KTAB_F(X)
+#undef X
+    add("G.base", "pointer", G + offsetof(State, base), 8);
+    add("G.nc", "state", G + offsetof(State, nc), 8);
+    add("G.pointers", "pointer", G + offsetof(State, trip_log), sizeof(State) - offsetof(State, trip_log));
+    add("O.base", "pointer", O + offsetof(Out, base), 8);
+    add("O.dims", "state", O + offsetof(Out, n), 16);
+#define X(n, tp) add("L." #n, "const", L + offsetof(Lds, n), 4);
+    RS_SCN_LDS(X)
+#undef X
+    add("L.gstride", "const", L + offsetof(Lds, gstride), 4);
+    add("L.lcap", "const", L + offsetof(Lds, lcap), 4);
+    add("L.cell_inv", "const", L + offsetof(Lds, cell_inv), 4);
+    add("GP", "pointer", GP, sizeof(StateP));
+    return s.c_str();
+}
+}
diff --git a/resco_amd/csrc/resco_sim.hip b/resco_amd/csrc/resco_sim.hip
--- a/resco_amd/csrc/resco_sim.hip
+++ b/resco_amd/csrc/resco_sim.hip
@@ -89,7 +89,6 @@
 #include "resco_ppo_loop.h"
 #include "resco_fma2c_train.h"
 
-struct StepArgs { KTab T; State G; Out O; Lds L; };
 typedef const __attribute__((address_space(4))) StepArgs *StepArgsPtr;
 
 template <bool PROF> struct DevExec {
@@ -132,7 +131,7 @@
     if (threadIdx.x == 0) g_sec_prof = P.prof;
 #endif
     DevExec<PROF> ex{(int)blockDim.x, __builtin_amdgcn_readfirstlane((int)threadIdx.x >> 6), PROF ? P.prof : nullptr, (PROF && P.prof) ? wall_clock64() : 0ull};
-    rs_step_body<CAP>(ex, A->L, A->T, A->G, A->O, P, actions, (int)blockIdx.x);
+    rs_step_body<CAP>(ex, A->L, A->T, A->GP, A->O, P, actions, (int)blockIdx.x);
 }
 template <int CAP>
 __global__ void __launch_bounds__(1024, 8)
@@ -146,6 +145,28 @@
 __global__ void __launch_bounds__(768, 6)
 rs_step_kernel_prof(StepArgsPtr Ac, KParams P, const int32_t *__restrict__ actions) { rs_step_kernel_body<0, true>(Ac, P, actions); }
 
+#ifndef RS_ONE_CAP
+#include "resco_scn_fix.h"
+#elif defined(RS_ONE_MAP)
+#include "resco_scn_fix.h"
+#undef RS_SCN_MAPS
+#define RS_SCN_MAPS(X) X(RS_ONE_MAP)
+#else
+#define RS_SCN_MAPS(X)
+#endif
+template <class F> __device__ __forceinline__ void rs_step_kernel_fix_body(StepArgsPtr Ac, const KParams &P, const int32_t *__restrict__ actions) {
+    if ((int)blockIdx.x >= P.n_envs) return;
+    const StepArgs *A = (const StepArgs *)Ac;
+    DevExec<false> ex{(int)blockDim.x, __builtin_amdgcn_readfirstlane((int)threadIdx.x >> 6), nullptr, 0ull};
+    rs_step_body_fix<F>(ex, A->T, A->GP, A->O, P, actions, (int)blockIdx.x);
+}
+template <class F>
+__global__ void __launch_bounds__(1024, 8)
+rs_step_kernel_fix_v64(StepArgsPtr Ac, KParams P, const int32_t *__restrict__ actions) { rs_step_kernel_fix_body<F>(Ac, P, actions); }
+template <class F>
+__global__ void __launch_bounds__(768, 6)
+rs_step_kernel_fix_v80(StepArgsPtr Ac, KParams P, const int32_t *__restrict__ actions) { rs_step_kernel_fix_body<F>(Ac, P, actions); }
+
 __global__ void rs_reset_kernel(KTab T, State G, KParams P) { rs_reset_env(T, G, P, (int)blockIdx.x, (int)threadIdx.x, blockDim.x); }
 __global__ void rs_reinit_kernel(KTab T, State G, KParams P) { rs_reinit_env(T, G, P, (int)blockIdx.x, (int)threadIdx.x, blockDim.x); }
 __global__ void rs_act_random_kernel(KTab T, KParams P, uint32_t step_key, int32_t *actions) {
@@ -158,7 +179,7 @@
     if (i < P.n_envs * T.n_signals) actions[i] = rs_maxwave_action(T, pairs, n_pairs, valid, order, use_pressure, mplight, wave, i);
 }
 
-enum RegBudget { V64 = 0, V128 = 1, V80 = 2 };
+struct FixKernel;
 struct rs_sim {
     int device = 0;
     int n_envs = 0, env_base = 0, block = 256;
@@ -167,6 +188,9 @@
     KTab K{};
     StepArgs *args = nullptr;
     RegBudget budget = V64;
+    ScnConsts consts{};
+    const FixKernel *fix = nullptr;
+    std::string kernel;
     State G{};
     Out O{};
     KParams P{};
@@ -240,6 +264,25 @@
 #endif
 }
 
+typedef bool (*scn_match_fn)(const ScnConsts &);
+struct FixKernel { const char *name; step_kernel_fn fn; scn_match_fn matches; };
+template <class F> static step_kernel_fn fix_kernel_fn() {
+    if constexpr (F::budget == V64) return rs_step_kernel_fix_v64<F>;
+    else return rs_step_kernel_fix_v80<F>;
+}
+static const FixKernel kFixKernels[] = {
+#define RS_FIX_ENTRY(m) RS_FIX_ENTRY_(m)
+#define RS_FIX_ENTRY_(m) {ScnFix_##m::budget == V64 ? "rs_step_kernel_fix_v64<" #m ">" : "rs_step_kernel_fix_v80<" #m ">", fix_kernel_fn<ScnFix_##m>(), scn_fix_matches<ScnFix_##m>},
+    RS_SCN_MAPS(RS_FIX_ENTRY)
+#undef RS_FIX_ENTRY
+#undef RS_FIX_ENTRY_
+    {nullptr, nullptr, nullptr}};
+static const FixKernel *fix_kernel_for(const ScnConsts &c) {
+    for (const FixKernel *k = kFixKernels; k->fn; ++k)
+        if (k->matches(c)) return k;
+    return nullptr;
+}
+
 static hipError_t wait_idle(rs_sim *h) {
     hipError_t e = hipStreamSynchronize(h->stream);
     if (e == hipSuccess && h->last && h->last != h->stream) e = hipStreamSynchronize(h->last);
@@ -291,6 +334,7 @@
     }
     const int C = sc->capacity;
     if (C < 64 || (C % 64) || C > 1984) { h->err = "capacity must be a multiple of 64 in [64, 1984]"; return fail(RS_ELIMIT); }
+    if ((size_t)n_envs * (size_t)C >= RS_STATE_MAX_SLOTS) { h->err = "n_envs * capacity must stay below 2^30 slots (the step kernels address a field of the state with 32-bit byte offsets)"; return fail(RS_ELIMIT); }
     if (sc->kmax < 1 || sc->kmax > 16) { h->err = "kmax (lanes per edge) must be in [1, 16]"; return fail(RS_ELIMIT); }
     PackedTables PT;
     if (const char *msg = rs_pack_tables(PT, sc)) { h->err = msg; return fail(RS_ELIMIT); }
@@ -320,7 +364,9 @@
     if (p->trip_log && (rc = dev_alloc(h, &G.trip_log, N * (size_t)sc->n_trips * 4))) return fail(rc);
     rs_fill_bufs(h->bufs, G, O, h->actions, BufDims{n_envs, C, sc->n_signals, sc->n_obs, lmax, h->K.n_dep, p->trip_log ? sc->n_trips : 0});
 
-    h->lds = lds_carve(nullptr, C, h->K.n_cells, h->K.n_arr, h->K.n_dep, sc->n_obs, sc->n_signals, sc->n_vtypes, h->K.tls_maxl);
+    Lds layout{};
+    rs_scn_consts_from(PT, sc, h->ratio, &h->consts, &layout);
+    h->lds = h->consts.lds_bytes;
     if (const char *pad = getenv("RESCO_STUDY_LDS_PAD")) h->lds += (size_t)atoi(pad);
     if (h->lds > 160 * 1024) { h->err = "scenario needs more than 160 KiB of LDS per environment"; return fail(RS_ELIMIT); }
     if (block_threads == 0) block_threads = rs_default_block(C, n_envs, device_id);
@@ -329,6 +375,23 @@
         return fail(RS_EINVAL);
     }
     h->block = block_threads;
+    h->consts.budget = h->budget; h->consts.lds_bytes = (uint32_t)h->lds;
+    {
+        const char *g = getenv("RESCO_STEP_GENERIC");
+        h->fix = (g && atoi(g) != 0) ? nullptr : fix_kernel_for(h->consts);
+        if (h->fix) h->kernel = h->fix->name;
+        else {
+            char nm[64];
+#ifdef RS_ONE_CAP
+            const int kcap = RS_ONE_CAP;
+#else
+            int kcap = 0;
+            for (int cp : kStepCaps) if (cp == C) kcap = cp;
+#endif
+            snprintf(nm, sizeof(nm), "rs_step_kernel_v%d<%d>", h->budget == V64 ? 64 : (h->budget == V80 ? 80 : 128), kcap);
+            h->kernel = nm;
+        }
+    }
     {
         static std::mutex mu;
         static size_t max_lds[64] = {0};
@@ -340,6 +403,10 @@
                     if (hipFuncSetAttribute((const void *)step_kernel_for(v, cp), hipFuncAttributeMaxDynamicSharedMemorySize, (int)h->lds) != hipSuccess) {
                         h->err = "hipFuncSetAttribute(MaxDynamicSharedMemorySize) failed"; return fail(RS_EHIP);
                     }
+            for (const FixKernel *k = kFixKernels; k->fn; ++k)
+                if (hipFuncSetAttribute((const void *)k->fn, hipFuncAttributeMaxDynamicSharedMemorySize, (int)h->lds) != hipSuccess) {
+                    h->err = "hipFuncSetAttribute(MaxDynamicSharedMemorySize) failed"; return fail(RS_EHIP);
+                }
             if (hipFuncSetAttribute((const void *)rs_step_kernel_prof, hipFuncAttributeMaxDynamicSharedMemorySize, (int)h->lds) != hipSuccess) {
                 h->err = "hipFuncSetAttribute(MaxDynamicSharedMemorySize) failed"; return fail(RS_EHIP);
             }
@@ -347,10 +414,8 @@
         }
     }
     {
-        StepArgs sa{h->K, h->G, h->O, Lds{}};
-        lds_carve(&sa.L, C, h->K.n_cells, h->K.n_arr, h->K.n_dep, sc->n_obs, sc->n_signals, sc->n_vtypes, h->K.tls_maxl);
+        StepArgs sa{h->K, h->G, h->O, layout, StateP(h->G)};
         if (!lds_fix_matches(sa.L, C)) { h->err = "the layout of the working memory does not match the kernel's literals (lds_carve / LdsFix)"; return fail(RS_EINVAL); }
-        sa.L.cell_inv = PT.cell_inv;
         if ((rc = dev_alloc(h, &h->args, 1, false))) return fail(rc);
         if (hipMemcpy(h->args, &sa, sizeof(sa), hipMemcpyHostToDevice) != hipSuccess) { h->err = "hipMemcpy(StepArgs) failed"; return fail(RS_EHIP); }
     }
@@ -396,7 +461,7 @@
         h->ev_used += 1;
         HIPCHK(h, hipEventRecord(e0, st));
     }
-    const step_kernel_fn fn = (h->prof && h->block <= 768) ? (step_kernel_fn)rs_step_kernel_prof : step_kernel_for(h->budget, h->K.capacity);
+    const step_kernel_fn fn = (h->prof && h->block <= 768) ? (step_kernel_fn)rs_step_kernel_prof : (h->fix ? h->fix->fn : step_kernel_for(h->budget, h->K.capacity));
     hipLaunchKernelGGL(fn, dim3(h->n_envs), dim3(h->block), h->lds, st, (StepArgsPtr)h->args, P, (const int32_t *)h->actions);
     HIPCHK(h, hipGetLastError());
     if (h->timing) HIPCHK(h, hipEventRecord(e1, st));
@@ -608,6 +673,7 @@
     return RS_OK;
 }
 
+extern "C" const char *rs_info_kernel(rs_handle h) { return h ? h->kernel.c_str() : ""; }
 extern "C" int rs_info(rs_handle h, int32_t *n_envs, int32_t *block_threads, int32_t *lds_bytes, int32_t *max_lanes_per_signal) {
     if (!h) return RS_EINVAL;
     rs_info_describe(h->n_envs, h->block, h->lds, h->K.lmax, n_envs, block_threads, lds_bytes, max_lanes_per_signal);
diff --git a/resco_amd/csrc/resco_step.h b/resco_amd/csrc/resco_step.h
--- a/resco_amd/csrc/resco_step.h
+++ b/resco_amd/csrc/resco_step.h
@@ -26,6 +26,43 @@
     RS_HD uint16_t *wtot() const { return RS_G((uint16_t *)(base + 40 * nc)); }
     RS_HD uint8_t *owner() const { return RS_G((uint8_t *)(base + 42 * nc)); }
     static size_t bytes(size_t nc_) { return 51 * nc_; }
+};
+template <class Tp, class I> RS_MEM const Tp &rs_at(const Tp *p, I i) { return *(const Tp *)((const char *)p + (uint32_t)i * (uint32_t)sizeof(Tp)); }
+template <class Tp> struct GOff {
+    Tp *p;
+    RS_HD Tp &operator[](size_t i) const { return *(Tp *)((char *)p + (uint32_t)i * (uint32_t)sizeof(Tp)); }
+};
+#define RS_STATE_MAX_SLOTS ((size_t)1 << 30)
+struct StateP {
+    float *pos_, *speed_, *accel_, *tloss_, *sf_;
+    uint32_t *coop_[2], *cooplead_[2];
+    uint16_t *lane_, *trip_, *cursor_, *swait_, *rwait_, *depart_, *wtot_;
+    uint8_t *owner_;
+    int32_t *trip_log, *env, *tls;
+    long long *stats;
+    uint16_t *dep_next;
+    uint32_t *mail;
+    StateP() = default;
+    explicit StateP(const State &G)
+        : pos_(G.pos()), speed_(G.speed()), accel_(G.accel()), tloss_(G.tloss()), sf_(G.sf()), coop_{G.coop(0), G.coop(1)},
+          cooplead_{G.cooplead(0), G.cooplead(1)}, lane_(G.lane()), trip_(G.trip()), cursor_(G.cursor()), swait_(G.swait()), rwait_(G.rwait()),
+          depart_(G.depart()), wtot_(G.wtot()), owner_(G.owner()), trip_log(G.trip_log), env(G.env), tls(G.tls), stats(G.stats),
+          dep_next(G.dep_next), mail(G.mail) {}
+    RS_HD GOff<float> pos() const { return GOff<float>{RS_G(pos_)}; }
+    RS_HD GOff<float> speed() const { return GOff<float>{RS_G(speed_)}; }
+    RS_HD GOff<float> accel() const { return GOff<float>{RS_G(accel_)}; }
+    RS_HD GOff<float> tloss() const { return GOff<float>{RS_G(tloss_)}; }
+    RS_HD GOff<float> sf() const { return GOff<float>{RS_G(sf_)}; }
+    RS_HD GOff<uint32_t> coop(int par) const { return GOff<uint32_t>{RS_G(coop_[par])}; }
+    RS_HD GOff<uint32_t> cooplead(int par) const { return GOff<uint32_t>{RS_G(cooplead_[par])}; }
+    RS_HD GOff<uint16_t> lane() const { return GOff<uint16_t>{RS_G(lane_)}; }
+    RS_HD GOff<uint16_t> trip() const { return GOff<uint16_t>{RS_G(trip_)}; }
+    RS_HD GOff<uint16_t> cursor() const { return GOff<uint16_t>{RS_G(cursor_)}; }
+    RS_HD GOff<uint16_t> swait() const { return GOff<uint16_t>{RS_G(swait_)}; }
+    RS_HD GOff<uint16_t> rwait() const { return GOff<uint16_t>{RS_G(rwait_)}; }
+    RS_HD GOff<uint16_t> depart() const { return GOff<uint16_t>{RS_G(depart_)}; }
+    RS_HD GOff<uint16_t> wtot() const { return GOff<uint16_t>{RS_G(wtot_)}; }
+    RS_HD GOff<uint8_t> owner() const { return GOff<uint8_t>{RS_G(owner_)}; }
 };
 
 struct Out {
@@ -301,6 +338,92 @@
     return choices[0];
 }
 
+#define RS_SCN_KTAB(X)                                                                                                                \
+    X(kmax) X(tls_maxl) X(n_signals) X(n_obs) X(n_vtypes) X(n_dep) X(n_arr) X(n_trips) X(n_lanes) X(n_cells) X(capacity) X(lmax)     \
+    X(step_length) X(yellow_length) X(horizon)
+#define RS_SCN_KTAB_F(X) X(maxlen) X(occ_unit)
+#define RS_SCN_LDS(X)                                                                                                                 \
+    X(node, Node) X(aux, Aux) X(vnx, float) X(vtp, float) X(grid, uint16_t) X(arr, int32_t) X(dep, uint16_t) X(dep_t, uint16_t)       \
+    X(alive, uint32_t) X(alive0, uint32_t) X(insm, uint32_t) X(mailw, uint32_t) X(agg_q, int32_t) X(agg_a, int32_t) X(agg_w, int32_t) \
+    X(agg_m, int32_t) X(agg_n, int32_t) X(agg_s, uint32_t) X(sig_arr, int32_t) X(sig_dep, int32_t) X(phase, int32_t) X(left, int32_t) \
+    X(nextp, int32_t) X(tstate, uint8_t) X(sc, int32_t) X(ls_h, uint16_t) X(ls_lc, uint16_t) X(ls_mh, uint16_t)
+enum RegBudget { V64 = 0, V128 = 1, V80 = 2 };
+struct ScnConsts {
+#define X(n) int32_t n;
+    RS_SCN_KTAB(X)
+#undef X
+#define X(n) uint32_t n##_bits;
+    RS_SCN_KTAB_F(X)
+#undef X
+    uint32_t cell_inv_bits;
+#define X(n, tp) uint32_t o_##n;
+    RS_SCN_LDS(X)
+#undef X
+    uint32_t gstride, lcap;
+    uint32_t lds_bytes;
+    int32_t budget;
+};
+#define RS_SCN_STR_(n) #n ","
+#define RS_SCN_STR_F_(n) #n "_bits,"
+#define RS_SCN_STR_O_(n, tp) "o_" #n ","
+#define RS_SCN_NAMES RS_SCN_KTAB(RS_SCN_STR_) RS_SCN_KTAB_F(RS_SCN_STR_F_) "cell_inv_bits," RS_SCN_LDS(RS_SCN_STR_O_) "gstride,lcap,lds_bytes,budget"
+RS_CARVE int rs_default_budget(int C, size_t lds) {
+    const int waves = C >= 768 ? 8 : ((C / 2) + 63) / 64;
+    return (waves * 64 == 512 && lds <= RS_LDS_4WG_LIMIT) ? V64 : V80;
+}
+RS_CARVE void scn_consts_layout(ScnConsts *c, const Lds &L, size_t lds_bytes) {
+#define X(n, tp) c->o_##n = L.n.off;
+    RS_SCN_LDS(X)
+#undef X
+    c->gstride = L.gstride; c->lcap = L.lcap; c->lds_bytes = (uint32_t)lds_bytes;
+    __builtin_memcpy(&c->cell_inv_bits, &L.cell_inv, 4);
+}
+template <class F> RS_CARVE bool scn_fix_matches(const ScnConsts &c) {
+    bool ok = c.cell_inv_bits == F::cell_inv_bits && c.gstride == F::gstride && c.lcap == F::lcap && c.lds_bytes == F::lds_bytes && c.budget == F::budget;
+#define X(n) ok = ok && c.n == F::n;
+    RS_SCN_KTAB(X)
+#undef X
+#define X(n) ok = ok && c.n##_bits == F::n##_bits;
+    RS_SCN_KTAB_F(X)
+#undef X
+#define X(n, tp) ok = ok && c.o_##n == F::o_##n;
+    RS_SCN_LDS(X)
+#undef X
+    return ok;
+}
+
+struct StepArgs { KTab T; State G; Out O; Lds L; StateP GP; };
+
+#ifndef RS_LAYOUT_ONLY
+template <class F> struct KTabFix {
+    const KTab &K;
+    const KCold &cold;
+    RS_MEM explicit KTabFix(const KTab &K_) : K(K_), cold(K_.cold) {}
+#define X(n) static constexpr int32_t n = F::n;
+    RS_SCN_KTAB(X)
+#undef X
+#define X(n) static constexpr float n = __builtin_bit_cast(float, (uint32_t)F::n##_bits);
+    RS_SCN_KTAB_F(X)
+#undef X
+    RS_MEM const LaneRec *lanes() const { return K.lanes(); }
+    RS_MEM const LinkRec *links() const { return K.links(); }
+    RS_MEM const FoeRec *foes() const { return K.foes(); }
+    RS_MEM const RStep *rsteps() const { return K.rsteps(); }
+    RS_MEM const float *route_cont() const { return K.route_cont(); }
+    RS_MEM const uint16_t *next_link() const { return K.next_link(); }
+    RS_MEM const uint16_t *notbest() const { return K.notbest(); }
+    RS_MEM const RouteRec *routes() const { return K.routes(); }
+    RS_MEM const uint16_t *trip_route() const { return K.trip_route(); }
+    RS_MEM const uint8_t *trip_vtype() const { return K.trip_vtype(); }
+};
+template <class F> struct LdsScn {
+#define X(n, tp) CPtr<tp, F::o_##n> n;
+    RS_SCN_LDS(X)
+#undef X
+    static constexpr uint32_t gstride = F::gstride, lcap = F::lcap;
+    static constexpr float cell_inv = __builtin_bit_cast(float, (uint32_t)F::cell_inv_bits);
+};
+
 #ifdef RS_EMU_DEBUG
 #define RS_CHAIN_GUARD if (++rs_dbg_chain > 50000000L) { printf("endless chain walk\n"); fflush(stdout); abort(); }
 #else
@@ -498,16 +621,16 @@
     return f.slot;
 }
 
-template <class LT> RS_DEV int tls_state(const KTab &T, const LT &L, int tls, int pos) {
+template <class TT, class LT> RS_DEV int tls_state(const TT &T, const LT &L, int tls, int pos) {
     if (tls == 0xFF) return TLS_G;
     return L.tstate[tls * T.tls_maxl + pos];
 }
-RS_DEV uint16_t cache_link(const KTab &T, const LaneRec &LR, int lane, int rq, int trip) {
+template <class TT> RS_DEV uint16_t cache_link(const TT &T, const LaneRec &LR, int lane, int rq, int trip) {
     if (LR.link_cnt == 0) return NLINK_NONE;
-    if (LR.flags & LF_INTERNAL) { const int l = LR.link_start; return (uint16_t)(l | (T.links()[l].arr_idx >= 0 ? NLINK_ARR : 0)); }
-    return T.next_link()[((size_t)rq * T.kmax + (lane - (int)LR.edge_lane0)) * 2 + (trip & 1)];
-}
-template <class LT> RS_DEV bool foe_blocked(const KTab &T, const LT &L, const Grid &grid, const LinkRec &K) {
+    if (LR.flags & LF_INTERNAL) { const int l = LR.link_start; return (uint16_t)(l | (rs_at(T.links(), l).arr_idx >= 0 ? NLINK_ARR : 0)); }
+    return rs_at(T.next_link(), ((uint32_t)rq * (uint32_t)T.kmax + (uint32_t)(lane - (int)LR.edge_lane0)) * 2u + (uint32_t)(trip & 1));
+}
+template <class TT, class LT> RS_DEV bool foe_blocked(const TT &T, const LT &L, const Grid &grid, const LinkRec &K) {
     for (int i = K.foe_start; i < K.foe_start + K.foe_cnt; ++i) {
         const FoeRec F = rec_load16(T.foes(), i);
         if (F.tls != 0xFF && tls_state(T, L, F.tls, F.tls_pos) == TLS_R) continue;
@@ -517,7 +640,7 @@
     }
     return false;
 }
-template <class LT> RS_DEV void tls_refresh(const KTab &T, const LT &L, const KParams &P, int s, int ph) {
+template <class TT, class LT> RS_DEV void tls_refresh(const TT &T, const LT &L, const KParams &P, int s, int ph) {
     const int w = T.tls_maxl >> 2;
     const uint32_t *src = (const uint32_t *)((P.fixed_program ? T.cold.fix8 + T.cold.fix_state_off[s] : T.cold.tls8 + T.cold.tls_state_off[s]) + ph * T.tls_maxl);
     uint32_t *dst = (uint32_t *)((uint8_t *)L.tstate + s * T.tls_maxl);
@@ -529,13 +652,13 @@
 #pragma unroll 1
     for (int i = 8; i < w; ++i) dst[i] = src[i];
 }
-template <class LT> RS_DEV void set_phase(const KTab &T, const LT &L, const KParams &P, int s, int ph) {
+template <class TT, class LT> RS_DEV void set_phase(const TT &T, const LT &L, const KParams &P, int s, int ph) {
     if (ph < 0 || ph >= T.cold.tls_nphase[s]) return;
     L.phase[s] = ph;
     L.left[s] = P.tls_expiry ? T.cold.tls_dur[T.cold.tls_dur_off[s] + ph] : RM_TLS_HOLD_TICKS;
     tls_refresh(T, L, P, s, ph);
 }
-template <class LT> RS_DEV void tls_begin_of_tick(const KTab &T, const LT &L, const KParams &P, int s, int tick) {
+template <class TT, class LT> RS_DEV void tls_begin_of_tick(const TT &T, const LT &L, const KParams &P, int s, int tick) {
     if (P.do_fsm && !P.fixed_program && tick == T.yellow_length) set_phase(T, L, P, s, L.nextp[s]);
     int left = L.left[s];
     if (left == 0) {
@@ -549,9 +672,9 @@
     L.left[s] = left - 1;
 }
 struct ContRow { float c[4]; const float *cn; };
-RS_DEV ContRow cont_row(const KTab &T, int rq) {
+template <class TT> RS_DEV ContRow cont_row(const TT &T, int rq) {
     ContRow R;
-    R.cn = T.route_cont() + (size_t)rq * T.kmax;
+    R.cn = (const float *)((const char *)T.route_cont() + (uint32_t)rq * (uint32_t)T.kmax * 4u);
     for (int j = 0; j < 4; ++j) R.c[j] = j < T.kmax ? R.cn[j] : 0.0f;
     return R;
 }
@@ -582,8 +705,8 @@
     if (rem - (float)cnt * occ_unit >= la * (float)off) return 0;
     return dir;
 }
-RS_DEV uint32_t link_reg_word(const KTab &T, int nlk) { return ((const uint32_t *)&T.links()[nlk & 0x7FFF])[2]; }
-template <class LT> RS_DEV void register_approach_w(const KTab &T, const LT &L, uint32_t kw, float v, float pos, float lane_len, int vt) {
+template <class TT> RS_DEV uint32_t link_reg_word(const TT &T, int nlk) { return rs_at((const uint32_t *)T.links(), (uint32_t)(nlk & 0x7FFF) * 8u + 2u); }
+template <class TT, class LT> RS_DEV void register_approach_w(const TT &T, const LT &L, uint32_t kw, float v, float pos, float lane_len, int vt) {
     const int st = tls_state(T, L, (int)((kw >> 16) & 0xFFu), (int)(kw >> 24));
     if (st == TLS_R) return;
     const float dist = lane_len - pos;
@@ -592,12 +715,12 @@
     const int q = ta * 10.0f >= 65000.0f ? 65000 : (int)(ta * 10.0f);
     rs_atomic_min(&L.arr[(int16_t)(kw & 0xFFFFu)], q);
 }
-template <class LT> RS_DEV void register_approach(const KTab &T, const LT &L, int nlk, float v, float pos, float lane_len, int vt) {
+template <class TT, class LT> RS_DEV void register_approach(const TT &T, const LT &L, int nlk, float v, float pos, float lane_len, int vt) {
     if (!(nlk & NLINK_ARR)) return;
     if (v <= RM_HALT_SPEED) return;
     register_approach_w(T, L, link_reg_word(T, nlk), v, pos, lane_len, vt);
 }
-template <class LT> RS_DEV void follow_neighbour(const KTab &T, const LT &L, uint32_t key, bool clamp_gap, const LaneRec &LR, int lane, float x, float v,
+template <class TT, class LT> RS_DEV void follow_neighbour(const TT &T, const LT &L, uint32_t key, bool clamp_gap, const LaneRec &LR, int lane, float x, float v,
                              float b, float tau, float mingap, float &vsafe) {
     const int X = (int)(key & 0xFFFFu), kx = (int)(key >> 16);
     if ((int)L.node[X].trip != kx) return;
@@ -650,7 +773,7 @@
     const int tk = kk + ((t & 1) ? -1 : +1);
     return tk >= 0 && tk < n && strategic_dir(R, tk, n, x, v, RM_SG_EXTRA_LANES, rem, OCC_NONE, 0, 0, 0.0f) == 0;
 }
-RS_DEV bool may_change_lanes(const KTab &T, int rq, uint32_t nb, const LaneRec &LR, int lane, int k, float x, float v, int t) {
+template <class TT> RS_DEV bool may_change_lanes(const TT &T, int rq, uint32_t nb, const LaneRec &LR, int lane, int k, float x, float v, int t) {
     const int n = LR.flags >> 2;
     if ((LR.flags & LF_INTERNAL) || n < 2) return false;
     const int kk = lane - (int)LR.edge_lane0;
@@ -668,14 +791,14 @@
 #endif
     return r;
 }
-template <class LT> RS_DEV int classify(const KTab &T, const LT &L, int s, const float *vt, float v, float x, const LaneRec &LR, int lane, int rq, uint32_t nb, int k, float sf, int t) {
+template <class TT, class LT> RS_DEV int classify(const TT &T, const LT &L, int s, const float *vt, float v, float x, const LaneRec &LR, int lane, int rq, uint32_t nb, int k, float sf, int t) {
     int fl = 0;
     if (looks_beyond(vt, v, x, LR.len, LR.vmax, sf)) { fl |= FL_H; list_push(L, L.ls_h, SC_NH, s); }
     if (may_change_lanes(T, rq, nb, LR, lane, k, x, v, t)) { fl |= FL_LC; list_push(L, L.ls_lc, SC_NLC, s); }
     return fl;
 }
 
-template <bool LONG, class LT> RS_DEV void phase_plan(const KTab &T, const LT &L, const Grid &grid, const State &G, size_t eo, const KParams &P, int genv, int t, int s) {
+template <bool LONG, class TT, class LT, class GT> RS_DEV void phase_plan(const TT &T, const LT &L, const Grid &grid, const GT &G, size_t eo, const KParams &P, int genv, int t, int s) {
     RS_SEC_BEGIN
     const Aux ax = L.aux[s];
     const int lane = ax.lane;
@@ -728,7 +851,7 @@
             bool stop_here = false;
             LinkRec K;
             if (link == NLINK_NONE) {
-                if (!cur_int && T.rsteps()[rq].next_edge == 0xFFFF) break;
+                if (!cur_int && rs_at(T.rsteps(), rq).next_edge == 0xFFFF) break;
                 stop_here = true;
             } else {
                 K = link_load(T.links(), link);
@@ -798,7 +921,7 @@
     (void)LR;
 }
 
-template <bool LONG, class LT> RS_DEV void phase_move(const KTab &T, const LT &L, const Grid &gnew, const State &G, const KParams &P, int env, size_t eo,
+template <bool LONG, class TT, class LT, class GT> RS_DEV void phase_move(const TT &T, const LT &L, const Grid &gnew, const GT &G, const KParams &P, int env, size_t eo,
                        int t, bool last_tick, bool more, int s, int &active, int &halted, int &top) {
     const Aux ax = L.aux[s];
     const Node me = L.node[s];
@@ -814,7 +937,7 @@
 #ifdef RS_FIELD_LOADS
     LaneRec LR = rec_load16(T.lanes(), lane);
 #endif
-    uint32_t nb = T.notbest()[ax.rq];
+    uint32_t nb = rs_at(T.notbest(), ax.rq);
     uint32_t kw = 0;
     if (more && (ax.nlink & NLINK_ARR)) kw = link_reg_word(T, ax.nlink);
     const float sfv = sf_of(me.sfq);
@@ -856,7 +979,7 @@
         if (!(x > LR.len)) break;
         const bool li = (LR.flags & LF_INTERNAL) != 0;
         if (link == NLINK_NONE) {
-            if (!li && T.rsteps()[rq].next_edge == 0xFFFF) arrived = true; else x = LR.len;
+            if (!li && rs_at(T.rsteps(), rq).next_edge == 0xFFFF) arrived = true; else x = LR.len;
             break;
         }
         x -= LR.len;
@@ -900,7 +1023,7 @@
     nn.pos = x; nn.speed = vn; nn.fl = (uint8_t)(me.fl & fl_mh(t));
     nn.nxt = grid_push(gnew, LR.cell0 + cell_of(L, x, lane_cells(L, LR)), s, vn > RM_HALT_SPEED);
     if (more) {
-        if (LONG && relink) { nb = T.notbest()[rq]; if (na.nlink & NLINK_ARR) kw = link_reg_word(T, na.nlink); }
+        if (LONG && relink) { nb = rs_at(T.notbest(), rq); if (na.nlink & NLINK_ARR) kw = link_reg_word(T, na.nlink); }
         nn.fl |= classify(T, L, s, L.vtp + me.vt * VT_COLS, vn, x, LR, lane, rq, nb, k, sfv, t + 1);
         L.node[s] = nn;
         if ((na.nlink & NLINK_ARR) && vn > RM_HALT_SPEED) register_approach_w(T, L, kw, vn, x, LR.len, me.vt);
@@ -916,7 +1039,7 @@
     return NIL;
 }
 
-template <class LT> RS_DEV int phase_lc_decide(const KTab &T, const LT &L, const Grid &grid, const State &G, size_t eo, int t, int s, const Aux &ax, const Node &me) {
+template <class TT, class LT, class GT> RS_DEV int phase_lc_decide(const TT &T, const LT &L, const Grid &grid, const GT &G, size_t eo, int t, int s, const Aux &ax, const Node &me) {
     const int lane = ax.lane;
 #ifdef RS_FIELD_LOADS
     const LaneRec LR = rec_load16(T.lanes(), lane);
@@ -1003,11 +1126,11 @@
         return code;
 }
 
-template <class LT> RS_DEV bool phase_insert_decide(const KTab &T, const LT &L, const Grid &grid, int t, int d) {
+template <class TT, class LT> RS_DEV bool phase_insert_decide(const TT &T, const LT &L, const Grid &grid, int t, int d) {
     if ((int)L.dep_t[d] > t) return false;
     const int k = L.dep[d];
     const DepInfo LR = rec_load8(T.cold.dep_info, d);
-    const float *vt = L.vtp + T.trip_vtype()[k] * VT_COLS;
+    const float *vt = L.vtp + rs_at(T.trip_vtype(), k) * VT_COLS;
     const float mypos = vt[VT_LENGTH] < LR.len ? vt[VT_LENGTH] : LR.len;
     const int nc = (int)(LR.len * L.cell_inv) + 1;
     const int c1 = LR.cell0 + cell_of(L, mypos + vt[VT_MINGAP] + T.maxlen, nc);
@@ -1035,7 +1158,7 @@
     return -1;
 }
 
-template <class LT> RS_DEV void lc_decide_and_flag(const KTab &T, const LT &L, const Grid &grid, const State &G, size_t eo, int t, int s) {
+template <class TT, class LT, class GT> RS_DEV void lc_decide_and_flag(const TT &T, const LT &L, const Grid &grid, const GT &G, size_t eo, int t, int s) {
     const Aux ax = L.aux[s];
     if (ax.lane == LANE_NONE) return;
     const int code = phase_lc_decide(T, L, grid, G, eo, t, s, ax, L.node[s]);
@@ -1043,8 +1166,8 @@
 }
 struct ExecInline {};
 
-template <int CAP, class Exec, class LT>
-RS_DEV void rs_step_body_on(Exec &ex, const LT &L, const KTab &T, const State &G, const Out &O, const KParams &P,
+template <int CAP, class Exec, class LT, class TT, class GT>
+RS_DEV void rs_step_body_on(Exec &ex, const LT &L, const TT &T, const GT &G, const Out &O, const KParams &P,
                             const int32_t *actions, int env) {
     const int B = ex.B;
     const int C = CAP ? CAP : T.capacity, S = T.n_signals, NO = T.n_obs;
@@ -1093,7 +1216,7 @@
             nn.fl = 0; nn.sfq = (uint16_t)speed_factor_q(P, genv, tr, L.vtp + nn.vt * VT_COLS);
             if ((G.mail[(size_t)env * ((C + 31) / 32) + (s >> 5)] >> (s & 31)) & 1u) nn.sfq |= (uint16_t)SFQ_MAIL((L.sc[SC_T] + 1) & 1);
             nn.nxt = grid_push(Grid{grid0, 0u}, LR0.cell0 + cell_of(L, x, lane_cells(L, LR0)), s, sp > RM_HALT_SPEED);
-            if (n_ticks > 0) nn.fl = (uint8_t)classify(T, L, s, L.vtp + nn.vt * VT_COLS, sp, x, LR0, ln, rq, T.notbest()[rq], tr, sf_of(nn.sfq), L.sc[SC_T]);
+            if (n_ticks > 0) nn.fl = (uint8_t)classify(T, L, s, L.vtp + nn.vt * VT_COLS, sp, x, LR0, ln, rq, rs_at(T.notbest(), rq), tr, sf_of(nn.sfq), L.sc[SC_T]);
             L.node[s] = nn;
             rs_atomic_or(&L.alive[s >> 5], 1u << (s & 31));
         }
@@ -1215,7 +1338,7 @@
                         const int s = nth_free_slot(L, C, rank);
                         if (s < 0) continue;
                         const int k = L.dep[d];
-                        const int v = T.trip_vtype()[k];
+                        const int v = rs_at(T.trip_vtype(), k);
                         const float *vt = L.vtp + v * VT_COLS;
                         const RouteRec RR = rec_load16(T.routes(), T.trip_route()[k]);
                         const LaneRec LRd = rec_load16(T.lanes(), RR.depart_lane);
@@ -1284,7 +1407,7 @@
             const int oi = T.cold.lane_obs[lane];
             bool detect = false;
             if (oi >= 0) {
-                const float d = (LR.len - L.node[s].pos) + T.rsteps()[rq].tlsdist;
+                const float d = (LR.len - L.node[s].pos) + rs_at(T.rsteps(), rq).tlsdist;
                 detect = d <= P.max_distance;
             }
             if (!detect) {
@@ -1402,11 +1525,18 @@
     });
 }
 
-template <int CAP, class Exec>
-RS_DEV void rs_step_body(Exec &ex, const Lds &L, const KTab &T, const State &G, const Out &O, const KParams &P,
+template <int CAP, class Exec, class GT>
+RS_DEV void rs_step_body(Exec &ex, const Lds &L, const KTab &T, const GT &G, const Out &O, const KParams &P,
                          const int32_t *actions, int env) {
     if constexpr (CAP != 0) {
         const LdsFix<CAP> Lf(L);
         rs_step_body_on<CAP>(ex, Lf, T, G, O, P, actions, env);
     } else rs_step_body_on<CAP>(ex, L, T, G, O, P, actions, env);
 }
+template <class F, class Exec, class GT>
+RS_DEV void rs_step_body_fix(Exec &ex, const KTab &T, const GT &G, const Out &O, const KParams &P, const int32_t *actions, int env) {
+    const KTabFix<F> Tf(T);
+    const LdsScn<F> Lf{};
+    rs_step_body_on<F::capacity>(ex, Lf, Tf, G, O, P, actions, env);
+}
+#endif
diff --git a/resco_amd/csrc/resco_tables.h b/resco_amd/csrc/resco_tables.h
--- a/resco_amd/csrc/resco_tables.h
+++ b/resco_amd/csrc/resco_tables.h
@@ -112,7 +112,7 @@
 template <class R, class I> RS_MEM R rec_load16(const R *tab, I i) {
     static_assert(sizeof(R) == 16 && alignof(R) == 16, "rec_load16: a 16-byte record");
     RecRaw16 r;
-    __builtin_memcpy(&r, &tab[i], 16);
+    __builtin_memcpy(&r, (const char *)tab + (uint32_t)i * 16u, 16);
     RS_KEEP4(r.a, r.b, r.c, r.d)
     R out;
     __builtin_memcpy(&out, &r, 16);
@@ -121,7 +121,7 @@
 template <class R, class I> RS_MEM R rec_load8(const R *tab, I i) {
     static_assert(sizeof(R) == 8 && alignof(R) == 8, "rec_load8: an 8-byte record");
     struct alignas(8) Raw { uint32_t a, b; } r;
-    __builtin_memcpy(&r, &tab[i], 8);
+    __builtin_memcpy(&r, (const char *)tab + (uint32_t)i * 8u, 8);
     RS_KEEP2(r.a, r.b)
     R out;
     __builtin_memcpy(&out, &r, 8);
@@ -129,7 +129,7 @@
 }
 template <class I> RS_MEM LinkRec link_load(const LinkRec *tab, I i) {
     RecRaw16 r[2];
-    __builtin_memcpy(r, &tab[i], 32);
+    __builtin_memcpy(r, (const char *)tab + (uint32_t)i * 32u, 32);
     RS_KEEP4(r[0].a, r[0].b, r[0].c, r[0].d)
     RS_KEEP4(r[1].a, r[1].b, r[1].c, r[1].d)
     LinkRec out;
diff --git a/resco_amd/sim.py b/resco_amd/sim.py
--- a/resco_amd/sim.py
+++ b/resco_amd/sim.py
@@ -32,7 +32,7 @@
                'rs_mplight_dqn_create', 'rs_mplight_dqn_sample', 'rs_mplight_dqn_grad', 'rs_mplight_dqn_step', 'rs_mplight_dqn_update',
                'rs_mplight_dqn_steps', 'rs_mplight_dqn_destroy',
                'rs_idqn_pack_weights', 'rs_dqn_sync_target', 'rs_mplight_dqn_sync_target', 'rs_group_train',
-               'rs_ppo_perm', 'rs_ippo_pack_weights', 'rs_group_ppo_train']
+               'rs_ppo_perm', 'rs_ippo_pack_weights', 'rs_group_ppo_train', 'rs_info_kernel']
 
 FMA2C_SYMBOLS = ['rs_fma2c_create', 'rs_fma2c_act', 'rs_fma2c_value', 'rs_fma2c_reset', 'rs_fma2c_set_device_weights', 'rs_fma2c_buffer',
                  'rs_fma2c_destroy', 'rs_fma2c_learn_create', 'rs_fma2c_learn_grad', 'rs_fma2c_learn_step', 'rs_fma2c_learn_update',
@@ -70,6 +70,9 @@
     L.rs_phase_profile.argtypes = [vp, i32, vp]
     L.rs_info.argtypes = [vp, C.POINTER(i32), C.POINTER(i32), C.POINTER(i32), C.POINTER(i32)]
     L.rs_group_step.argtypes = [vp, i32, vp, i32]
+    if hasattr(L, 'rs_info_kernel'):
+        L.rs_info_kernel.argtypes = [vp]
+        L.rs_info_kernel.restype = C.c_char_p
     if hasattr(L, 'rs_idqn_create'):
         L.rs_idqn_create.argtypes = [i32, i32, i32] + [vp] * 9 + [C.POINTER(vp)]
         L.rs_idqn_act.argtypes = [vp, vp, i32, i32, i32, f32, u32, u32, vp, vp, vp, vp]
@@ -384,7 +387,10 @@
     def info(self):
         a, b, c, d = C.c_int32(), C.c_int32(), C.c_int32(), C.c_int32()
         self._check(self._lib.rs_info(self._h, C.byref(a), C.byref(b), C.byref(c), C.byref(d)))
-        return dict(n_envs=a.value, block_threads=b.value, lds_bytes=c.value, max_lanes_per_signal=d.value)
+        out = dict(n_envs=a.value, block_threads=b.value, lds_bytes=c.value, max_lanes_per_signal=d.value)
+        if hasattr(self._lib, 'rs_info_kernel'):
+            out['step_kernel'] = self._lib.rs_info_kernel(self._h).decode()
+        return out
 
     def reset(self, stream=None):
         self._check(self._lib.rs_reset(self._h, stream))
```

New measurement: 4.242 million env-steps/s (median of 6 runs). 1.06x the previous value.
